# justinkay/aldi

Hardware: AMD Instinct MI355X
Metric: images/sec (student+teacher ALDI step), R50-FPN 1333x800 (higher is better)
Workload: dtype bf16

## Files before the change

aldi_amd/_lib.py:

```python
from __future__ import annotations

import ctypes as C
import os
import re

_HERE = os.path.dirname(os.path.abspath(__file__))
LIB_PATH = os.path.join(_HERE, "lib", "libaldi_hip.so")
HEADER_PATH = os.path.join(os.path.dirname(_HERE), "include", "aldi_hip.h")


class AldiHipError(RuntimeError):
    pass


if not os.path.exists(LIB_PATH):
    raise ImportError(
        f"{LIB_PATH} not found: build it with `python -c 'import __graft_entry__ as g; g.build()'` "
        "(or `make -C aldi_amd/csrc`). There is no CPU fallback for the ALDI HIP path.")

lib = C.CDLL(LIB_PATH)

F32, BF16 = 0, 1
MAX_IMAGES, MAX_LEVELS = 16, 5
c_void_p, c_int, c_float, c_long = C.c_void_p, C.c_int, C.c_float, C.c_long


def _ctype(decl: str):
    decl = decl.strip()
    if "*" in decl or decl.startswith("aldi_stream_t"):
        return C.c_void_p
    base = decl.rsplit(" ", 1)[0].replace("const", "").strip() if " " in decl else decl
    return {"int": C.c_int, "long": C.c_long, "float": C.c_float, "size_t": C.c_size_t, "unsigned": C.c_uint, "unsigned long long": C.c_ulonglong,
            "double": C.c_double}[base]


def parse_header(path: str = HEADER_PATH):
    src = open(path).read()
    src = re.sub(r"/\*.*?\*/", "", src, flags=re.S)
    protos = {}
    for m in re.finditer(r"\b(int|long|size_t|const char\*)\s+(aldi_\w+)\s*\(([^;{}]*?)\)\s*;", src, flags=re.S):
        ret, name, args = m.group(1), m.group(2), m.group(3)
        args = " ".join(args.split())
        argtypes = [] if args in ("void", "") else [_ctype(a) for a in args.split(",")]
        restype = {"int": C.c_int, "long": C.c_long, "size_t": C.c_size_t, "const char*": C.c_char_p}[ret]
        protos[name] = (restype, argtypes)
    return protos


PROTOS = parse_header()
for _name, (_res, _args) in PROTOS.items():
    _fn = getattr(lib, _name)
    _fn.restype = _res
    _fn.argtypes = _args


def check(status: int, what: str = ""):
    if status != 0:
        raise AldiHipError(f"{what}: status {status}: {lib.aldi_last_error().decode()}")


def call(name: str, *args):
    check(getattr(lib, name)(*args), name)


def set_tuning(name: str, value: int):
    call("aldi_set_tuning", name.encode(), int(value))


def get_tuning(name: str) -> int:
    v = C.c_int(0)
    call("aldi_get_tuning", name.encode(), C.byref(v))
    return v.value


def reset_tuning():
    call("aldi_reset_tuning")


def last_dispatch() -> str:
    return lib.aldi_last_dispatch().decode()


def plan_dispatch(args, n: int = 1) -> str:
    buf = C.create_string_buffer(224)
    call("aldi_conv_igemm_plan", C.byref(args) if isinstance(args, C.Structure) else args, n, buf, len(buf))
    return buf.value.decode()


def plan_wgrad_dispatch(args, n: int = 1, group: bool = False):
    buf = C.create_string_buffer(224)
    ws = C.c_long(0)
    call("aldi_conv_wgrad_plan", C.byref(args) if isinstance(args, C.Structure) else args, n, int(group), buf, len(buf), C.byref(ws))
    return buf.value.decode(), ws.value


class BoxLossChunk(C.Structure):
    _fields_ = [("r0", c_int), ("r1", c_int), ("grad_scale_cls", c_float), ("grad_scale_box", c_float), ("loss_box", c_void_p),
                ("teacher_pred", c_void_p), ("cls_temperature", c_float), ("kl", c_int), ("do_cls", c_int), ("do_reg", c_int),
                ("grad_scale_distill_cls", c_float), ("grad_scale_distill_reg", c_float), ("loss_distill", c_void_p)]


class ConvArgs(C.Structure):
    _fields_ = [
        ("x", c_void_p), ("w", c_void_p), ("y", c_void_p), ("y_f32", c_void_p),
        ("scale", c_void_p), ("shift", c_void_p), ("res", c_void_p), ("mask", c_void_p),
        ("N", c_int), ("H", c_int), ("W", c_int), ("Cin", c_int),
        ("Cout", c_int), ("KH", c_int), ("KW", c_int), ("stride", c_int), ("pad", c_int),
        ("Ho", c_int), ("Wo", c_int),
        ("relu", c_int), ("res_mode", c_int), ("out_scale", c_int), ("OH", c_int), ("OW", c_int),
        ("dtype", c_int), ("ws", c_void_p), ("ksplit", c_int), ("mask_bits", c_void_p), ("bits_out", c_void_p),
    ]


class WgradArgs(C.Structure):
    _fields_ = [
        ("x", c_void_p), ("g", c_void_p), ("dw", c_void_p), ("scale", c_void_p),
        ("N", c_int), ("H", c_int), ("W", c_int), ("Cin", c_int), ("Cout", c_int), ("KH", c_int), ("KW", c_int),
        ("stride", c_int), ("pad", c_int), ("Ho", c_int), ("Wo", c_int), ("dtype", c_int), ("db", c_void_p),
        ("ws", c_void_p), ("ws_bytes", C.c_long),
    ]


class StemArgs(C.Structure):
    _fields_ = [
        ("img", c_void_p), ("w", c_void_p), ("scale", c_void_p), ("shift", c_void_p), ("y", c_void_p),
        ("N", c_int), ("Hs", c_int), ("Ws", c_int), ("Hc", c_int), ("Wc", c_int),
        ("h", c_int * MAX_IMAGES), ("w_img", c_int * MAX_IMAGES),
        ("mean", c_float * 3), ("std", c_float * 3), ("dtype", c_int),
    ]


class RpnGeom(C.Structure):
    _fields_ = [
        ("num_levels", c_int), ("A", c_int), ("C", c_int),
        ("H", c_int * MAX_LEVELS), ("W", c_int * MAX_LEVELS), ("off", c_int * (MAX_LEVELS + 1)),
    ]


class RoiFeats(C.Structure):
    _fields_ = [
        ("feat", c_void_p * 4), ("grad", c_void_p * 4), ("H", c_int * 4), ("W", c_int * 4),
        ("scale", c_float * 4), ("C", c_int),
    ]


class DgwItem(C.Structure):
    _fields_ = [("w_master", c_void_p), ("scale", c_void_p), ("wt", c_void_p),
                ("Cout", c_int), ("KH", c_int), ("KW", c_int), ("Cin", c_int), ("tile_begin", c_int), ("reserved", c_int)]


class FoldItem(C.Structure):
    _fields_ = [("w", c_void_p), ("scale", c_void_p), ("out", c_void_p), ("rows", c_int), ("cols", c_int), ("chunk_begin", c_int), ("reserved", c_int)]


class BottleneckArgs(C.Structure):
    _fields_ = [("x", c_void_p), ("res", c_void_p), ("y", c_void_p), ("w1", c_void_p), ("w2", c_void_p), ("w3", c_void_p),
                ("b1", c_void_p), ("b2", c_void_p), ("b3", c_void_p),
                ("N", c_int), ("H", c_int), ("W", c_int), ("Cin", c_int), ("mid", c_int), ("Cout", c_int)]


class AttnArgs(C.Structure):
    _fields_ = [
        ("qkv", c_void_p), ("rel_h", c_void_p), ("rel_w", c_void_p),
        ("Qp", c_void_p), ("Kp", c_void_p), ("KpT", c_void_p), ("VT", c_void_p), ("QsT", c_void_p),
        ("O", c_void_p), ("lse", c_void_p), ("dO", c_void_p), ("dOT", c_void_p), ("dQp", c_void_p), ("delta", c_void_p),
        ("dqkv", c_void_p), ("drel_h", c_void_p), ("drel_w", c_void_p),
        ("nB", c_int), ("gh", c_int), ("gw", c_int), ("heads", c_int), ("Dq", c_int), ("scale", c_float),
    ]


PtrArray5 = c_void_p * MAX_LEVELS
```

aldi_amd/csrc/host.h:

```cpp
#pragma once
#include "../../include/aldi_hip.h"

int aldi_set_error_msg(int code, const char* msg);

typedef uint16_t bf16_t;

#define ALDI_KNOBS(X) \
    X(igemm_xcd, 1) X(igemm_tile, 0) X(igemm_dbg, 0) X(igemm_bigtile_min, 1024) X(igemm_bigtile, 64) X(igemm_bigtile_k, 768) X(igemm_lintile_min, 768) \
    X(igemm_halo, 1) X(igemm_force, 0) X(igemm_k64_min, 1024) X(igemm_group, 1) X(igemm_narrow_k, 512) X(igemm_splitk_tile, 2) X(igemm_halo_f32, 0) \
    X(igemm_f32_tile64_max, 4096) X(igemm_direct, 15) X(igemm_lean, 1) X(igemm_halo64_mid, 0) X(igemm_ws, 1) X(igemm_ws_wgs, 512) X(igemm_ws_min, 40000) \
    X(wgrad_lean, 1) X(wgrad_big_min, 28) X(wgrad_big_slots, 256) X(wgrad_slots, 384) X(wgrad_xcd, 1) \
    X(igemm_halo_ilv, 1) X(igemm_halo_small, 0) X(igemm_halo96, 0) \
    X(wgrad_dma, 0) X(wgrad_dbg, 0) X(wgrad_group_slots, 0) X(wgrad_group_epi, 24) X(wgrad_db, 0) X(wgrad_ordered, 1) X(wgrad_big_group, 1) X(wgrad_big_epi, 12) \
    X(wgrad_big_group_min, 64) X(wgrad_lds_pad_kb, 0) X(wgrad_f32_tile128, 1) X(wgrad_dma64, 3) X(wgrad_ilv, 0) \
    X(msda_gather, 7) X(msda_gather_list, 1500) X(msda_bin, 1) X(msda_bin_list, 512) X(roialign_sep, 1) X(roialign_bwd_rows, 2) \
    X(colsum_blocks, 256) X(colsum_minrows, 16) X(colsum_nt, 1024) X(colsum_block_kb, 384) \
    X(stem_mfma, 1) X(stem_pool_wgs, 0) X(sab_blocks, 512) X(ln_bwd_blocks, 512) X(ln_bwd_blocks_narrow, 1024) X(rpn_topk_fused, 1) X(ema_blocks, 2048) X(nms_mask_tri, 1) X(match_wave, 1)

struct AldiTuning {
#define ALDI_KNOB_FIELD(name, dflt) int name;
    ALDI_KNOBS(ALDI_KNOB_FIELD)
#undef ALDI_KNOB_FIELD
};
AldiTuning& aldi_tuning();
void aldi_note_dispatch(const char* kernel);

static inline int cdiv(long a, long b) { return (int)((a + b - 1) / b); }
```

aldi_amd/csrc/igemm.hip:

```cpp
#include "common.h"
#include "igemm_select.h"
#include "tile_prims.h"
#include <stdlib.h>

namespace {

template <typename T, int BM, int BN, int WM, int WN, int LDS_BYTES>
__device__ __forceinline__ void igemm_epilogue(const ConvDev& p, f32x4_t (&acc)[BM / WM / 16][BN / WN / 16], const int m0, const int n0, unsigned char* stg) {
    constexpr int NT = WM * WN * 64;
    constexpr int TM = BM / WM / 16, TN = BN / WN / 16;
    const int tid = threadIdx.x, lane = tid & 63, wave = tid >> 6;
    const int wm = wave / WN, wn = wave % WN;
    const int fr = lane & 15, fq = lane >> 4;
    if (p.dbg & 4) return;
    T* __restrict__ Y = static_cast<T*>(p.y);
    const T* __restrict__ R = static_cast<const T*>(p.res);
    const T* __restrict__ Mk = static_cast<const T*>(p.mask);
    if constexpr (sizeof(T) == 2) {
        constexpr int ROWB = BN * 2 + 16;
        constexpr bool kStageFits = BM * ROWB <= LDS_BYTES;
        if (kStageFits && Y && !p.y_f32 && (p.Cout & 7) == 0) {
            __syncthreads();
            {
                unsigned char* wr = stg + (wm * (BM / WM) + fr) * ROWB + (wn * (BN / WN) + fq * 4) * 2;
// ... 590 lines not shown
            if (wbase + it * NT < BN * KC) {
                unsigned off = b_voff[it] == OOB ? OOB : b_voff[it] + k_off;
                if (ktail && s * BK + b_kce[it] >= p.K) off = OOB;
                if (p.dbg & 16) off &= 0xfffu;
                glds16(rw, &lds[buf][BM * KC + wbase + it * NT], off);
            }
        }
        ci0 += BK;
        if (ci0 >= p.Cin) { ci0 = 0; ++tap; if (++kw == p.KW) { kw = 0; ++kh; } }
    };

    static_assert(KC == 4 || !PIPE, "the register-pipelined loop reads one k-step (4 chunks) per slab");
    constexpr int N_DMA = A_IT + (BN * KC) / NT;
    const int S_all = (p.dbg & 8) ? 1 : (p.K + BK - 1) / BK;
    const int s_first = p.ksplit > 1 ? (int)blockIdx.z * p.slabs_per_split : 0;
    const int S = p.ksplit > 1 ? min(S_all - s_first, p.slabs_per_split) : S_all;
    ci0 = s_first * BK;
    if constexpr (PIPE) pre_seen = S > 3;
    issue_slab(s_first, 0);
    if (S > 1) issue_slab(s_first + 1, 1);
    if constexpr (!PIPE) issue_pre();
    constexpr unsigned SLAB_BYTES = (BM + BN) * KC * 16;
    const int xrow = wm * (BM / WM) + fr, wrow = wn * (BN / WN) + fr;
    const unsigned x_rd0 = lds_addr(&lds[0][0]) + (unsigned)(xrow * KC + swz<KC>(xrow, fq)) * 16u;
    const unsigned w_rd0 = lds_addr(&lds[0][0]) + (unsigned)((BM + wrow) * KC + swz<KC>(wrow, fq)) * 16u;
    if constexpr (PIPE) {
    if (S > 2) issue_slab(s_first + 2, 2);
    __builtin_amdgcn_sched_barrier(0);
    issue_pre();
    __builtin_amdgcn_sched_barrier(0);
    u32x4_t xf0[TM], wf0[TN], xf1[TM], wf1[TN];
    if (S > 2) asm volatile("s_waitcnt vmcnt(%0)" ::"n"(2 * N_DMA + N_PRE) : "memory");
    else if (S > 1) asm volatile("s_waitcnt vmcnt(%0)" ::"n"(N_DMA + N_PRE) : "memory");
    else asm volatile("s_waitcnt vmcnt(%0)" ::"n"(N_PRE) : "memory");
    __builtin_amdgcn_s_barrier();
    __builtin_amdgcn_sched_barrier(0);
    frag_read_all<TM, KC * 16>(xf0, x_rd0);
    frag_read_all<TN, KC * 16>(wf0, w_rd0);
    frag_wait<TM, TN>(xf0, wf0);
    int rbuf = 1, ibuf = 0;
    auto step = [&](int s, u32x4_t* xc, u32x4_t* wc, u32x4_t* xn, u32x4_t* wn_) {
        const bool more = s + 1 < S;
        if (more) {
            if (N_PRE > 0 && s < 2) {
                if (s + 2 < S) asm volatile("s_waitcnt vmcnt(%0)" ::"n"(N_DMA + N_PRE) : "memory");
                else asm volatile("s_waitcnt vmcnt(%0)" ::"n"(N_PRE) : "memory");
            } else {
                if (s + 2 < S) asm volatile("s_waitcnt vmcnt(%0)" ::"n"(N_DMA) : "memory");
                else asm volatile("s_waitcnt vmcnt(0)" ::: "memory");
            }
            __builtin_amdgcn_s_barrier();
            __builtin_amdgcn_sched_barrier(0);
        }
        frag_read_all<TM, KC * 16>(xn, x_rd0 + (unsigned)rbuf * SLAB_BYTES);
        frag_read_all<TN, KC * 16>(wn_, w_rd0 + (unsigned)rbuf * SLAB_BYTES);
        if (more && s + 3 < S) issue_slab(s_first + s + 3, ibuf);
#pragma unroll
        for (int i = 0; i < TM; ++i)
#pragma unroll
            for (int j = 0; j < TN; ++j) acc[i][j] = Mma<T>::run(wc[j], xc[i], acc[i][j]);
        frag_wait<TM, TN>(xn, wn_);
        rbuf = rbuf == NBUF - 1 ? 0 : rbuf + 1;
        ibuf = ibuf == NBUF - 1 ? 0 : ibuf + 1;
    };
    for (int s = 0; s < S; s += 2) {
        step(s, xf0, wf0, xf1, wf1);
        if (s + 1 < S) step(s + 1, xf1, wf1, xf0, wf0);
    }
    } else {
    int buf = 0, nbuf = 2;
    for (int s = 0; s < S; ++s) {
        if (N_PRE > 0 && s == 0 && S > 1) asm volatile("s_waitcnt vmcnt(%0)" ::"n"(N_DMA + N_PRE) : "memory");
        else if (s + 1 < S) asm volatile("s_waitcnt vmcnt(%0)" ::"n"(N_DMA) : "memory");
        else asm volatile("s_waitcnt vmcnt(0)" ::: "memory");
        __builtin_amdgcn_s_barrier();
        __builtin_amdgcn_sched_barrier(0);
        if (s + 2 < S) issue_slab(s_first + s + 2, nbuf);
#pragma unroll
        for (int h = 0; h < KC / 4; ++h) {
            u32x4_t xf[TM], wf[TN];
            const unsigned xa = h == 0 ? x_rd0 : lds_addr(&lds[0][0]) + (unsigned)(xrow * KC + swz<KC>(xrow, fq + 4)) * 16u;
            const unsigned wa = h == 0 ? w_rd0 : lds_addr(&lds[0][0]) + (unsigned)((BM + wrow) * KC + swz<KC>(wrow, fq + 4)) * 16u;
            frag_read_all<TM, KC * 16>(xf, xa + (unsigned)buf * SLAB_BYTES);
            frag_read_all<TN, KC * 16>(wf, wa + (unsigned)buf * SLAB_BYTES);
            frag_wait<TM, TN>(xf, wf);
#pragma unroll
            for (int i = 0; i < TM; ++i)
#pragma unroll
                for (int j = 0; j < TN; ++j) acc[i][j] = Mma<T>::run(wf[j], xf[i], acc[i][j]);
        }
        buf = buf == NBUF - 1 ? 0 : buf + 1;
        nbuf = nbuf == NBUF - 1 ? 0 : nbuf + 1;
    }
    }

    }

    if constexpr (DIRECT) {
        if (!pre_seen) {
            asm volatile("s_waitcnt vmcnt(0)" ::: "memory");
            __builtin_amdgcn_s_barrier();
        }
        __builtin_amdgcn_sched_barrier(0);
        igemm_epilogue_direct<BM, BN, WM, WN, RESL>(p, acc, m0, n0, rres, lds_addr(aux_lds));
        return;
    }
    if (p.ksplit > 1) {
        ConvDev q = p;
        q.y_f32 = p.y_f32 + (long)blockIdx.z * p.M * p.Cout;
        igemm_epilogue<T, BM, BN, WM, WN, NSTAGE * SLOTS * 16>(q, acc, m0, n0, reinterpret_cast<unsigned char*>(&lds_all[0]));
        return;
    }
    igemm_epilogue<T, BM, BN, WM, WN, NSTAGE * SLOTS * 16>(p, acc, m0, n0, reinterpret_cast<unsigned char*>(&lds_all[0]));
}


template <typename T, int BN>
__device__ __forceinline__ void igemm_halo_rs_body(const ConvDev& p, int bid, const int nmt, const int nnt) {
    static_assert(sizeof(T) == 2, "bf16 only");
    constexpr int BM = 256, WM = 4, WN = BN / 64, NT = WM * WN * 64, KC = 4, EP = 8, BK = 32;
    static_assert(NT == 512, "eight waves: two halves of four");
    constexpr int TM = BM / WM / 16, TN = BN / WN / 16;
    constexpr int AS = ((BM + 2) * KC + 63) / 64 * 64;
    constexpr int WS = 3 * BN * KC;
    constexpr int STAGE = AS + WS, NS = 3;
    constexpr int AH_IT = (AS + NT - 1) / NT, WH_IT = WS / NT;
    static_assert(AH_IT == 3 && WH_IT == 3 && WS % NT == 0, "six DMA pieces per thread and group: two per phase");
    __shared__ __attribute__((aligned(128))) uint4 lds[NS * STAGE + 4];

    const int tid = threadIdx.x, lane = tid & 63, wave = tid >> 6;
    const int wm = wave / WN, wn = wave % WN;
    if (p.xcd) {
        const int total = nmt * nnt, q = total >> 3, r = total & 7, xcd = bid & 7, idx = bid >> 3;
        bid = (xcd < r ? xcd * (q + 1) : r * (q + 1) + (xcd - r) * q) + idx;
    }
    const int m0 = (bid / nnt) * BM, n0 = (bid % nnt) * BN;
    const T* __restrict__ X = static_cast<const T*>(p.x);
    const T* __restrict__ Wt = static_cast<const T*>(p.w);
    const __amdgpu_buffer_rsrc_t rx = __builtin_amdgcn_make_buffer_rsrc(const_cast<T*>(X), 0, p.x_bytes, 0x00020000);
    const __amdgpu_buffer_rsrc_t rw = __builtin_amdgcn_make_buffer_rsrc(const_cast<T*>(Wt), 0, p.w_bytes, 0x00020000);
    constexpr unsigned OOB = 0x80000000u;
    const int wbase = __builtin_amdgcn_readfirstlane(tid & ~63);
    const bool half_b = __builtin_amdgcn_readfirstlane(wave) >= 4;
    const bool third_pix = wbase + 2 * NT < AS;
    f32x4_t acc[TM][TN];
#pragma unroll
    for (int i = 0; i < TM; ++i)
#pragma unroll
        for (int j = 0; j < TN; ++j) acc[i][j] = f32x4_t{0.f, 0.f, 0.f, 0.f};
    const int fr = lane & 15, fq = lane >> 4;
    if (tid < 4) lds[NS * STAGE + tid] = make_uint4(0u, 0u, 0u, 0u);

    unsigned ha_voff[AH_IT], ha_mask[AH_IT];
#pragma unroll
    for (int it = 0; it < AH_IT; ++it) {
        const int c = tid + it * NT, row = c >> 2, kce = swz_halo(row, c & 3);
        const int q0 = m0 - 1 + row;
        const bool ok = row < BM + 2 && q0 >= 0 && q0 < p.M;
        const int qq = ok ? q0 : 0;
        const int h0 = (qq / p.W) % p.H;
        ha_voff[it] = ((unsigned)qq * (unsigned)p.Cin + (unsigned)(kce * EP)) * (unsigned)sizeof(T);
        ha_mask[it] = ok ? ((h0 >= 1 ? 1u : 0u) | 2u | (h0 <= p.H - 2 ? 4u : 0u)) : 0u;
    }
    unsigned hw_voff[WH_IT];
#pragma unroll
    for (int it = 0; it < WH_IT; ++it) {
        const int c = tid + it * NT, kwi = c / (BN * KC), rem = c - kwi * (BN * KC), row = rem >> 2, kce = swz_halo(row, rem & 3);
        const int co = n0 + row;
        hw_voff[it] = co < p.Cout ? ((unsigned)co * (unsigned)p.K + (unsigned)(kwi * p.Cin + kce * EP)) * (unsigned)sizeof(T) : OOB;
    }
    const int xrow = wm * (BM / WM) + fr, wrow = wn * (BN / WN) + fr;
    const unsigned lbase = lds_addr(&lds[0]);
    const unsigned zrow = lbase + (unsigned)(NS * STAGE) * 16u + (unsigned)fq * 16u;
    bool edge_l[TM], edge_r[TM];
    unsigned zaddr[TM];
#pragma unroll
    for (int i = 0; i < TM; ++i) {
        const int m = m0 + wm * (BM / WM) + i * 16 + fr;
        const int wo = m % p.W;
        edge_l[i] = wo == 0;
        edge_r[i] = wo == p.W - 1;
        zaddr[i] = zrow - (unsigned)(i * 16 * KC * 16);
    }
    unsigned x_rd[3];
#pragma unroll
    for (int kw = 0; kw < 3; ++kw) x_rd[kw] = lbase + (unsigned)((xrow + kw) * KC + swz_halo(xrow + kw, fq)) * 16u;
    const unsigned w_rd = lbase + (unsigned)((AS + wrow * KC) + swz_halo(wrow, fq)) * 16u;
    constexpr unsigned STAGE_BYTES = STAGE * 16;
    const int G = 3 * (p.Cin / BK);

    unsigned a_off = 0, w_off = 0, ikh = 0;
    int gkh = 0, gci = 0;
    auto next_group = [&]() {
        a_off = (unsigned)(((gkh - 1) * p.W * p.Cin + gci) * (int)sizeof(T));
        w_off = (unsigned)((gkh * 3 * p.Cin + gci) * (int)sizeof(T));
        ikh = (unsigned)gkh;
        gci += BK;
        if (gci >= p.Cin) { gci = 0; ++gkh; }
    };
    const unsigned dmask = (p.dbg & 16) ? 0xfffu : 0xffffffffu;
    const bool no_dma = p.dbg & 32, no_mfma = p.dbg & 64;
    auto issue_pair = [&](int pair, int st) {
        uint4* base = &lds[st * STAGE];
        if (no_dma) return;
        if (pair == 0) {
            glds16(rx, base + wbase, ((ha_mask[0] >> ikh) & 1u) ? (ha_voff[0] + a_off) & dmask : OOB);
            glds16(rx, base + wbase + NT, ((ha_mask[1] >> ikh) & 1u) ? (ha_voff[1] + a_off) & dmask : OOB);
        } else if (pair == 1) {
            glds16(rw, base + AS + wbase, hw_voff[0] == OOB ? OOB : (hw_voff[0] + w_off) & dmask);
            glds16(rw, base + AS + wbase + NT, hw_voff[1] == OOB ? OOB : (hw_voff[1] + w_off) & dmask);
        } else {
            glds16(rw, base + AS + wbase + 2 * NT, hw_voff[2] == OOB ? OOB : (hw_voff[2] + w_off) & dmask);
            if (third_pix) glds16(rx, base + wbase + 2 * NT, ((ha_mask[2] >> ikh) & 1u) ? (ha_voff[2] + a_off) & dmask : OOB);
        }
    };
    next_group();
    issue_pair(0, 0); issue_pair(1, 0); issue_pair(2, 0);
    next_group();
    issue_pair(0, 1); issue_pair(1, 1);
    asm volatile("s_waitcnt vmcnt(4)" ::: "memory");
    __builtin_amdgcn_s_barrier();
    __builtin_amdgcn_sched_barrier(0);
    if (half_b) {
        __builtin_amdgcn_s_barrier();
        __builtin_amdgcn_sched_barrier(0);
    }
    int rs = 0, s1 = 1, s2 = 2;
    for (int g = 0; g < G; ++g) {
        const unsigned gb = (unsigned)rs * STAGE_BYTES;
#pragma unroll
        for (int t = 0; t < 3; ++t) {
            u32x4_t xf[TM], wf[TN];
            if (t == 1) {
                frag_read_all<TM, KC * 16>(xf, x_rd[1] + gb);
            } else {
                unsigned xa[TM];
#pragma unroll
                for (int i = 0; i < TM; ++i) xa[i] = (t == 0 ? edge_l[i] : edge_r[i]) ? zaddr[i] : x_rd[t] + gb;
                frag_read_each<TM, KC * 16>(xf, xa);
            }
            frag_read_all<TN, KC * 16>(wf, w_rd + gb + (unsigned)(t * BN * KC * 16));
            if (t == 0) {
                if (g + 1 < G) issue_pair(2, s1);
            } else if (g + 2 < G) {
                if (t == 1) next_group();
                issue_pair(t - 1, s2);
            }
            if (t == 2 && g + 1 < G) {
                if (g + 2 < G && !no_dma) asm volatile("s_waitcnt vmcnt(4)" ::: "memory");
                else asm volatile("s_waitcnt vmcnt(0)" ::: "memory");
            }
            __builtin_amdgcn_sched_barrier(0);
            __builtin_amdgcn_s_barrier();
            __builtin_amdgcn_sched_barrier(0);
            frag_wait<TM, TN>(xf, wf);
            __builtin_amdgcn_sched_barrier(0);
            __builtin_amdgcn_s_setprio(1);
            if (!no_mfma) {
#pragma unroll
                for (int i = 0; i < TM; ++i)
#pragma unroll
                    for (int j = 0; j < TN; ++j) acc[i][j] = Mma<T>::run(wf[j], xf[i], acc[i][j]);
            }
            __builtin_amdgcn_s_setprio(0);
            __builtin_amdgcn_sched_barrier(0);
            __builtin_amdgcn_s_barrier();
            __builtin_amdgcn_sched_barrier(0);
        }
        const int o = rs; rs = s1; s1 = s2; s2 = o;
    }
    if (!half_b) {
        __builtin_amdgcn_s_barrier();
        __builtin_amdgcn_sched_barrier(0);
    }
    igemm_epilogue<T, BM, BN, WM, WN, NS * STAGE * 16>(p, acc, m0, n0, reinterpret_cast<unsigned char*>(&lds[0]));
}

template <typename T, int BN>
__global__ __launch_bounds__(512) void igemm_halo_rs_kernel(ConvDev p) {
    igemm_halo_rs_body<T, BN>(p, (int)(blockIdx.y * gridDim.x + blockIdx.x), (int)gridDim.x, (int)gridDim.y);
}

#include "igemm_halo64.h"
#include "igemm_ws.h"

template <int BM, int NT, bool HALO> constexpr int min_waves_per_simd() { return HALO && BM == 240 ? 2 * NT / 256 : 1; }
template <typename T, int BM, int BN, int WM, int WN, int KC, bool PIPE, bool HALO = false, int EPI = 0, bool LEAN = false>
__global__ __launch_bounds__(WM* WN * 64, (min_waves_per_simd<BM, WM * WN * 64, HALO>())) void igemm_kernel(ConvDev p) {
    igemm_body<T, BM, BN, WM, WN, KC, PIPE, HALO, EPI, LEAN>(p, (int)(blockIdx.y * gridDim.x + blockIdx.x), (int)gridDim.x, (int)gridDim.y);
}

template <typename T, int BM, int BN, int WM, int WN, int KC, bool PIPE, bool HALO = false>
__global__ __launch_bounds__(WM* WN * 64, (min_waves_per_simd<BM, WM * WN * 64, HALO>())) void igemm_group_kernel(ConvGroup G) {
    const int bid = (int)blockIdx.x;
    int i = 0;
    for (int k = 1; k < G.n; ++k)
        if (bid >= G.wg_begin[k]) i = k;
    i = __builtin_amdgcn_readfirstlane(i);
    const int local = bid - G.wg_begin[i];
    if (local >= G.nmt[i] * G.nnt[i]) return;
    igemm_body<T, BM, BN, WM, WN, KC, PIPE, HALO>(G.p[i], local, G.nmt[i], G.nnt[i]);
}

template <int BM, int BN, int WM, int WN, bool DIRECT, bool ILV = false>
__global__ __launch_bounds__(WM* WN * 64) void igemm_halo64_group_kernel(ConvGroup G) {
    const int bid = (int)blockIdx.x;
    int i = 0;
    for (int k = 1; k < G.n; ++k)
        if (bid >= G.wg_begin[k]) i = k;
    i = __builtin_amdgcn_readfirstlane(i);
    const int local = bid - G.wg_begin[i];
    if (local >= G.nmt[i] * G.nnt[i]) return;
    igemm_halo64_body<BM, BN, WM, WN, DIRECT, ILV>(G.p[i], local, G.nmt[i], G.nnt[i]);
}


int group_table(ConvGroup& G, const int BM, const int BN, const ConvDev& d) {
    int wg = 0;
    for (int i = 0; i < G.n; ++i) {
        G.p[i].xcd = d.xcd; G.p[i].dbg = d.dbg;
        G.nmt[i] = cdiv(G.p[i].M, BM); G.nnt[i] = cdiv(G.p[i].Cout, BN);
        G.wg_begin[i] = wg;
        wg += (G.nmt[i] * G.nnt[i] + 7) / 8 * 8;
    }
    for (int i = G.n; i <= kMaxConvGroup; ++i) G.wg_begin[i] = wg;
    return wg;
}

template <typename T, int BM, int BN, int WM, int WN, int KC, bool PIPE, bool HALO, int EPI>
int launch_tile(const Choice& c, const ConvDev& d, const ConvGroup* g, hipStream_t st) {
    constexpr int NT = WM * WN * 64;
    if constexpr (EPI != 0) {
        const dim3 grid(cdiv(d.M, BM), cdiv(d.Cout, BN));
        if constexpr (!HALO) {
            if (c.lean) hipLaunchKernelGGL((igemm_kernel<T, BM, BN, WM, WN, KC, PIPE, HALO, EPI, true>), grid, dim3(NT), 0, st, d);
        }
        if (HALO || !c.lean) hipLaunchKernelGGL((igemm_kernel<T, BM, BN, WM, WN, KC, PIPE, HALO, EPI, false>), grid, dim3(NT), 0, st, d);
    } else if (g) {
        ConvGroup G = *g;
        const int wg = group_table(G, BM, BN, d);
        hipLaunchKernelGGL((igemm_group_kernel<T, BM, BN, WM, WN, KC, PIPE, HALO>), dim3(wg), dim3(NT), 0, st, G);
    } else {
        const dim3 grid(cdiv(d.M, BM), cdiv(d.Cout, BN), d.ksplit > 1 ? d.ksplit : 1);
        hipLaunchKernelGGL((igemm_kernel<T, BM, BN, WM, WN, KC, PIPE, HALO>), grid, dim3(NT), 0, st, d);
    }
    ALDI_CHECK_LAUNCH();
    return ALDI_OK;
}
template <typename T, int BM, int BN, int WM, int WN, int KC, bool PIPE, int EPI>
int launch_TAP(const Choice& c, const ConvDev& d, const ConvGroup* g, hipStream_t st) { return launch_tile<T, BM, BN, WM, WN, KC, PIPE, false, EPI>(c, d, g, st); }
template <typename T, int BM, int BN, int WM, int WN, int KC, bool PIPE, int EPI>
int launch_HALO(const Choice& c, const ConvDev& d, const ConvGroup* g, hipStream_t st) { return launch_tile<T, BM, BN, WM, WN, KC, PIPE, true, EPI>(c, d, g, st); }

template <typename T, int BM, int BN, int WM, int WN, int KC, bool PIPE, int EPI>
int launch_ROLES(const Choice&, const ConvDev& d, const ConvGroup*, hipStream_t st) {
    static_assert(BM == 256 && WM * WN * 64 == 512, "igemm_halo_rs_body: 256 pixels on eight waves");
    const dim3 grid(cdiv(d.M, BM), cdiv(d.Cout, BN));
    hipLaunchKernelGGL((igemm_halo_rs_kernel<T, BN>), grid, dim3(512), 0, st, d);
    ALDI_CHECK_LAUNCH();
    return ALDI_OK;
}

template <typename T, int BM, int BN, int WM, int WN, int KC, bool PIPE, int EPI>
int launch_HALO64(const Choice& c, const ConvDev& d, const ConvGroup* g, hipStream_t st) {
    constexpr int NT = WM * WN * 64;
    constexpr bool HAS_ILV = BM == 256 && BN == 256 && WM == 4 && WN == 2;
    if (g) {
        ConvGroup G = *g;
        const int wg = group_table(G, BM, BN, d);
        if (c.ilv) {
            if (c.direct) hipLaunchKernelGGL((igemm_halo64_group_kernel<BM, BN, WM, WN, true, HAS_ILV>), dim3(wg), dim3(NT), 0, st, G);
            else hipLaunchKernelGGL((igemm_halo64_group_kernel<BM, BN, WM, WN, false, HAS_ILV>), dim3(wg), dim3(NT), 0, st, G);
        } else {
            if (c.direct) hipLaunchKernelGGL((igemm_halo64_group_kernel<BM, BN, WM, WN, true>), dim3(wg), dim3(NT), 0, st, G);
            else hipLaunchKernelGGL((igemm_halo64_group_kernel<BM, BN, WM, WN, false>), dim3(wg), dim3(NT), 0, st, G);
        }
    } else {
        const dim3 grid(cdiv(d.M, BM), cdiv(d.Cout, BN));
        if (c.ilv) {
            if (c.direct) hipLaunchKernelGGL((igemm_halo64_kernel<BM, BN, WM, WN, true, HAS_ILV>), grid, dim3(NT), 0, st, d);
            else hipLaunchKernelGGL((igemm_halo64_kernel<BM, BN, WM, WN, false, HAS_ILV>), grid, dim3(NT), 0, st, d);
        } else {
            if (c.direct) hipLaunchKernelGGL((igemm_halo64_kernel<BM, BN, WM, WN, true>), grid, dim3(NT), 0, st, d);
            else hipLaunchKernelGGL((igemm_halo64_kernel<BM, BN, WM, WN, false>), grid, dim3(NT), 0, st, d);
        }
    }
    ALDI_CHECK_LAUNCH();
    return ALDI_OK;
}

int launch_choice(const Choice& c, const ConvDev& d, const ConvGroup* g, hipStream_t st) {
    switch (c.tile) {
#define IGEMM_TILE_CASE(id, T, form, BM, BN, WM, WN, KC, PIPE, EPI) \
    case id: return launch_##form<T, BM, BN, WM, WN, KC, PIPE != 0, EPI>(c, d, g, st);
        IGEMM_TILES(IGEMM_TILE_CASE)
#undef IGEMM_TILE_CASE
    default: break;
    }
    return aldi_set_error_msg(ALDI_ERR_ARG, "conv_igemm: unknown tile");
}

__global__ __launch_bounds__(256) void splitk_finalize_kernel(const float* __restrict__ ws, int ks, long mc, int C, const float* __restrict__ scale,
                                                              const float* __restrict__ shift, int relu, bf16_t* __restrict__ y) {
    const long e = ((long)blockIdx.x * blockDim.x + threadIdx.x) * 4;
    if (e >= mc) return;
    float4 a = *reinterpret_cast<const float4*>(ws + e);
    for (int z = 1; z < ks; ++z) {
        const float4 b = *reinterpret_cast<const float4*>(ws + z * mc + e);
        a.x += b.x; a.y += b.y; a.z += b.z; a.w += b.w;
    }
    const int c = (int)(e % C);
    if (scale) { const float4 s4 = *reinterpret_cast<const float4*>(scale + c); a.x *= s4.x; a.y *= s4.y; a.z *= s4.z; a.w *= s4.w; }
    if (shift) { const float4 s4 = *reinterpret_cast<const float4*>(shift + c); a.x += s4.x; a.y += s4.y; a.z += s4.z; a.w += s4.w; }
    if (relu) { a.x = fmaxf(a.x, 0.f); a.y = fmaxf(a.y, 0.f); a.z = fmaxf(a.z, 0.f); a.w = fmaxf(a.w, 0.f); }
    uint2 o;
    o.x = pack2_bf16(a.x, a.y); o.y = pack2_bf16(a.z, a.w);
    *reinterpret_cast<uint2*>(y + e) = o;
}

constexpr int kNameCap = 112;

int conv_one(const aldi_conv_args* a, const bool dry, hipStream_t st, char* name) {
    ConvDev d;
    Choice c;
    if (int rc = plan_conv(a, aldi_tuning(), d, c)) return rc;
    dispatch_name(c, name, kNameCap);
    if (dry) return ALDI_OK;
    if (int rc = launch_choice(c, d, nullptr, st)) return rc;
    aldi_note_dispatch(name);
    if (c.ksplit > 1) {
        const long mc = (long)d.M * d.Cout;
        hipLaunchKernelGGL(splitk_finalize_kernel, dim3(cdiv(mc / 4, 256)), dim3(256), 0, st, static_cast<const float*>(a->ws), c.ksplit, mc, d.Cout, a->scale, a->shift,
                           a->relu, static_cast<bf16_t*>(a->y));
        ALDI_CHECK_LAUNCH();
    }
    return ALDI_OK;
}

int conv_many(const aldi_conv_args* args, const int n, const bool dry, hipStream_t st, char* name) {
    if (!args || n < 1) return aldi_set_error_msg(ALDI_ERR_ARG, "conv_igemm_group: no problems");
    if (n == 1 || !conv_group_same(args, n, aldi_tuning())) {
        for (int i = 0; i < n; ++i)
            if (int rc = conv_one(&args[i], dry, st, name)) return rc;
        return ALDI_OK;
    }
    static thread_local ConvGroup G;
    ConvDev d;
    Choice c;
    if (int rc = plan_conv_group(args, n, aldi_tuning(), G, d, c)) return rc;
    dispatch_name(c, name, kNameCap);
    if (dry) return ALDI_OK;
    if (int rc = launch_choice(c, d, &G, st)) return rc;
    aldi_note_dispatch(name);
    return ALDI_OK;
}
}

extern "C" int aldi_conv_igemm(const aldi_conv_args* a, aldi_stream_t stream) {
    char name[kNameCap];
    return conv_one(a, false, static_cast<hipStream_t>(stream), name);
}

extern "C" int aldi_conv_igemm_group(const aldi_conv_args* args, int n, aldi_stream_t stream) {
    char name[kNameCap];
    return conv_many(args, n, false, static_cast<hipStream_t>(stream), name);
}

extern "C" int aldi_conv_igemm_plan(const aldi_conv_args* args, int n, char* name, int cap) {
    char buf[kNameCap] = "";
    const int rc = n == 1 ? conv_one(args, true, nullptr, buf) : conv_many(args, n, true, nullptr, buf);
    if (rc == ALDI_OK && name && cap > 0) snprintf(name, (size_t)cap, "%s", buf);
    return rc;
}
```

aldi_amd/csrc/igemm_halo64.h:

```cpp
#pragma once

template <int N, int STRIDE, int BASE, int I = 0>
__device__ __forceinline__ void frag_read_n(u32x4_t* f, unsigned addr) {
    if constexpr (I < N) {
        f[I] = frag_read<BASE + I * STRIDE>(addr);
        frag_read_n<N, STRIDE, BASE, I + 1>(f, addr);
    }
}
template <int N>
__device__ __forceinline__ void frag_wait1(u32x4_t* a) {
    asm volatile("s_waitcnt lgkmcnt(0)" ::: "memory");
#pragma unroll
    for (int i = 0; i < N; ++i) asm volatile("" : "+v"(a[i]));
}

template <int V> struct KwTag { static constexpr int value = V; };

__device__ __forceinline__ void mma_ip(f32x4_t& c, const u32x4_t& a, const u32x4_t& b) {
    asm volatile("v_mfma_f32_16x16x32_bf16 %0, %1, %2, %0" : "+v"(c) : "v"(a), "v"(b));
}
template <int NM, int I = 0, typename FM, typename FF>
__device__ __forceinline__ void interleave(FM&& mma, FF&& fill) {
    if constexpr (I < NM) {
        mma(KwTag<I>{});
        fill(KwTag<I>{});
        interleave<NM, I + 1>(mma, fill);
    }
}

template <int BM, int BN, int WM, int WN, bool DIRECT, bool ILV = false>
__device__ __forceinline__ void igemm_halo64_body(const ConvDev& p, int bid, const int nmt, const int nnt) {
    typedef bf16_t T;
    constexpr int NT = WM * WN * 64, KC = 8, EP = 8, BK = 64;
    constexpr int TM = BM / WM / 16;
    constexpr int TN = BN / WN / 16;
    constexpr int CS = TN / 4;
    constexpr int TH = 4;
    static_assert((TM == 4 || TM == 8) && (CS == 1 || CS == 2), "64 / 128 pixels x 64 / 128 channels per wave");
    constexpr int XS = ((BM + 2) * KC + 63) / 64 * 64;
    constexpr int WS = BN * KC;
    constexpr int X_IT = (XS + NT - 1) / NT;
    constexpr int W_IT = WS / NT;
    constexpr int XQ = (X_IT - 1) / 4, WQ = W_IT / 4;
    static_assert((X_IT - 1) % 4 == 0 && W_IT % 4 == 0 && WS % NT == 0 && XS - (X_IT - 1) * NT <= 64, "piece schedule below: four quarters + one tail piece (wave 0) per slab, four quarters per tap");
    constexpr int RING = 2 * XS + 2 * WS;
    constexpr int EPI_SLOTS = BM * (BN * 2 + 16) / 16;
    constexpr int LDS_SLOTS = RING + 8 > EPI_SLOTS ? RING + 8 : EPI_SLOTS;
    constexpr int FR = 16 * KC * 16;
    __shared__ __attribute__((aligned(128))) uint4 lds_all[LDS_SLOTS];

    const int tid = threadIdx.x, lane = tid & 63, wave = tid >> 6;
    const int wm = wave / WN, wn = wave % WN;
    if (p.xcd) {
        const int total = nmt * nnt, q = total >> 3, r = total & 7, xcd = bid & 7, idx = bid >> 3;
        bid = (xcd < r ? xcd * (q + 1) : r * (q + 1) + (xcd - r) * q) + idx;
    }
    const int m0 = (bid / nnt) * BM, n0 = (bid % nnt) * BN;
    const __amdgpu_buffer_rsrc_t rx = __builtin_amdgcn_make_buffer_rsrc(const_cast<T*>(static_cast<const T*>(p.x)), 0, p.x_bytes, 0x00020000);
    const __amdgpu_buffer_rsrc_t rw = __builtin_amdgcn_make_buffer_rsrc(const_cast<T*>(static_cast<const T*>(p.w)), 0, p.w_bytes, 0x00020000);
    constexpr unsigned OOB = 0x80000000u;
    const int wbase = __builtin_amdgcn_readfirstlane(tid & ~63);
    const bool tail = wbase + (X_IT - 1) * NT < XS;
    const int fr = lane & 15, fq = lane >> 4;
    const int plev = __builtin_amdgcn_readfirstlane((p.dbg & 128) ? 0 : (p.dbg & 256) ? 1 : ((wave < WM * WN / 2) != ((p.dbg & 512) != 0)) ? 2 : 1);
    const bool prio = plev != 0, prio_hi = plev == 2;
    const bool early_w = ILV && __builtin_amdgcn_readfirstlane(p.dbg & 1024) == 0;
    const bool no_dma = p.dbg & 32, no_mfma = p.dbg & 64;

    f32x4_t acc[TM][TN];
#pragma unroll
    for (int i = 0; i < TM; ++i)
#pragma unroll
        for (int j = 0; j < TN; ++j) acc[i][j] = f32x4_t{0.f, 0.f, 0.f, 0.f};
    if (tid < 8) lds_all[RING + tid] = make_uint4(0u, 0u, 0u, 0u);

    unsigned xa_voff[X_IT], xa_ok = 0;
#pragma unroll
    for (int it = 0; it < X_IT; ++it) {
        const int c = tid + it * NT, row = c >> 3, kce = (c & 7) ^ (row & 6);
        const int q0 = m0 - 1 + row;
        const bool ok = row < BM + 2 && q0 >= 0 && q0 < p.M;
        const int qq = ok ? q0 : 0;
        const int h0 = (qq / p.W) % p.H;
        xa_voff[it] = ((unsigned)qq * (unsigned)p.Cin + (unsigned)(kce * EP)) * 2u;
        if (ok) xa_ok |= ((h0 >= 1 ? 1u : 0u) | 2u | (h0 <= p.H - 2 ? 4u : 0u)) << (3 * it);
    }
    unsigned wa_voff[W_IT];
#pragma unroll
    for (int it = 0; it < W_IT; ++it) {
        const int c = tid + it * NT, row = c >> 3, kce = (c & 7) ^ (row & 6);
        const int co = n0 + (DIRECT ? direct_perm<BN / WN>(row) : row);
        wa_voff[it] = co < p.Cout ? ((unsigned)co * (unsigned)p.K + (unsigned)(kce * EP)) * 2u : OOB;
    }
    int xkh = 0, xci = 0, tkh = 0, tci = 0, tkw = 0;
    auto issue_x = [&](int it, int st) {
        if (no_dma) return;
        const unsigned a_off = (unsigned)(((xkh - 1) * p.W * p.Cin + xci) * 2);
        glds16(rx, &lds_all[st * XS + wbase + it * NT], ((xa_ok >> (3 * it + xkh)) & 1u) ? xa_voff[it] + a_off : OOB);
    };
    auto next_x = [&]() { if (++xkh == 3) { xkh = 0; xci += BK; } };
    auto issue_w = [&](int it, int st, unsigned w_off) {
        if (no_dma) return;
        glds16(rw, &lds_all[2 * XS + st * WS + wbase + it * NT], wa_voff[it] == OOB ? OOB : wa_voff[it] + w_off);
    };
    auto tap_off = [&]() { return (unsigned)(((tkh * 3 + tkw) * p.Cin + tci) * 2); };
    auto next_tap = [&]() { if (++tkw == 3) { tkw = 0; if (++tkh == 3) { tkh = 0; tci += BK; } } };

    const int xrow = wm * (BM / WM) + fr, wrow = wn * (BN / WN) + fr;
    const unsigned lbase = lds_addr(&lds_all[0]);
    unsigned x_rd[3][2], w_rd[2];
#pragma unroll
    for (int kw = 0; kw < 3; ++kw)
#pragma unroll
        for (int h = 0; h < 2; ++h) x_rd[kw][h] = lbase + (unsigned)((xrow + kw) * KC + ((h * 4 + fq) ^ ((xrow + kw) & 6))) * 16u;
#pragma unroll
    for (int h = 0; h < 2; ++h) w_rd[h] = lbase + (unsigned)(2 * XS + wrow * KC + ((h * 4 + fq) ^ (wrow & 6))) * 16u;
    bool edge_l[TM], edge_r[TM];
    unsigned zaddr[TM];
#pragma unroll
    for (int i = 0; i < TM; ++i) {
        const int m = m0 + wm * (BM / WM) + i * 16 + fr;
        const int wo = m % p.W;
        edge_l[i] = wo == 0;
        edge_r[i] = wo == p.W - 1;
        zaddr[i] = lbase + (unsigned)(RING * 16) + (unsigned)fq * 16u - (unsigned)(i * FR);
    }
    auto read_x = [&](u32x4_t* xf, auto KW, auto H, unsigned xoff) {
        constexpr int kw = decltype(KW)::value, h = decltype(H)::value;
        if constexpr (kw == 1) {
            frag_read_n<TM, FR, 0>(xf, x_rd[1][h] + xoff);
        } else {
            const unsigned a = x_rd[kw][h] + xoff;
            unsigned xa[TM];
#pragma unroll
            for (int i = 0; i < TM; ++i) xa[i] = (kw == 0 ? edge_l[i] : edge_r[i]) ? zaddr[i] : a;
            frag_read_each<TM, KC * 16>(xf, xa);
        }
    };

    const int ngroups = 3 * (p.Cin / BK), U = 3 * ngroups;
#pragma unroll
    for (int it = 0; it < X_IT - 1; ++it) issue_x(it, 0);
    if (tail) issue_x(X_IT - 1, 0);
    next_x();
    {
        const unsigned o = tap_off();
#pragma unroll
        for (int it = 0; it < W_IT; ++it) issue_w(it, 0, o);
        next_tap();
    }
    unsigned woff_a = tap_off();
#pragma unroll
    for (int q = 0; q < 2 * WQ; ++q) issue_w(q, 1, woff_a);
    if (early_w) {
#pragma unroll
        for (int q = 2 * WQ; q < 4 * WQ; ++q) issue_w(q, 1, woff_a);
    }
    next_tap();
    __builtin_amdgcn_sched_barrier(0);
    if (early_w) asm volatile("s_waitcnt vmcnt(%0)" ::"n"(4 * WQ) : "memory");
    else asm volatile("s_waitcnt vmcnt(%0)" ::"n"(2 * WQ) : "memory");
    __builtin_amdgcn_s_barrier();
    __builtin_amdgcn_sched_barrier(0);

    u32x4_t x0[TM], x1[TM], wa[TH], wb[TH];
    read_x(x0, KwTag<0>{}, KwTag<0>{}, 0u);
    frag_read_n<TH, FR, 0>(wa, w_rd[0]);
    frag_wait<TM, TH>(x0, wa);
    __builtin_amdgcn_sched_barrier(0);

    unsigned xoff = 0, woff = 0;
    constexpr unsigned XSB = XS * 16, WSB = WS * 16;
    auto tap4 = [&](auto KW, const int g, const int u) {
        constexpr int kw = decltype(KW)::value;
        const bool more1 = u + 1 < U, more2 = u + 2 < U;
        frag_read_n<TH, FR, TH * FR>(wb, w_rd[0] + woff);
        if (more1) {
#pragma unroll
            for (int q = 0; q < WQ; ++q) issue_w(2 * WQ + q, (u + 1) & 1, woff_a);
        }
        __builtin_amdgcn_sched_barrier(0);
        if (!no_mfma) {
            if (prio) { if (prio_hi) __builtin_amdgcn_s_setprio(2); else __builtin_amdgcn_s_setprio(1); }
#pragma unroll
            for (int i = 0; i < TM; ++i)
#pragma unroll
                for (int j = 0; j < TH; ++j) acc[i][j] = Mma<T>::run(wa[j], x0[i], acc[i][j]);
            if (prio) __builtin_amdgcn_s_setprio(0);
        }
        frag_wait1<TH>(wb);
        __builtin_amdgcn_sched_barrier(0);
        read_x(x1, KW, KwTag<1>{}, xoff);
        frag_read_n<TH, FR, 0>(wa, w_rd[1] + woff);
        if (more1) {
#pragma unroll
            for (int q = 0; q < WQ; ++q) issue_w(3 * WQ + q, (u + 1) & 1, woff_a);
        }
        __builtin_amdgcn_sched_barrier(0);
        if (!no_mfma) {
            if (prio) { if (prio_hi) __builtin_amdgcn_s_setprio(2); else __builtin_amdgcn_s_setprio(1); }
#pragma unroll
            for (int i = 0; i < TM; ++i)
#pragma unroll
                for (int j = 0; j < TH; ++j) acc[i][TH + j] = Mma<T>::run(wb[j], x0[i], acc[i][TH + j]);
            if (prio) __builtin_amdgcn_s_setprio(0);
        }
        frag_wait<TM, TH>(x1, wa);
        __builtin_amdgcn_sched_barrier(0);
        frag_read_n<TH, FR, TH * FR>(wb, w_rd[1] + woff);
        int nx = 0;
        if (kw < 2 && g + 1 < ngroups) {
            const int st = (g + 1) & 1;
            if constexpr (kw == 0) {
#pragma unroll
                for (int q = 0; q < 2 * XQ; ++q) issue_x(q, st);
                nx = 2 * XQ;
            }
            if constexpr (kw == 1) {
#pragma unroll
                for (int q = 0; q < 2 * XQ; ++q) issue_x(2 * XQ + q, st);
                nx = 2 * XQ;
                if (tail) { issue_x(X_IT - 1, st); nx = 2 * XQ + 1; }
                next_x();
            }
        }
        __builtin_amdgcn_sched_barrier(0);
        if (!no_mfma) {
            if (prio) { if (prio_hi) __builtin_amdgcn_s_setprio(2); else __builtin_amdgcn_s_setprio(1); }
#pragma unroll
            for (int i = 0; i < TM; ++i)
#pragma unroll
                for (int j = 0; j < TH; ++j) acc[i][j] = Mma<T>::run(wa[j], x1[i], acc[i][j]);
            if (prio) __builtin_amdgcn_s_setprio(0);
        }
        frag_wait1<TH>(wb);
        __builtin_amdgcn_sched_barrier(0);
        if (no_dma || nx == 0) asm volatile("s_waitcnt vmcnt(0)" ::: "memory");
        else if (nx == 2 * XQ) asm volatile("s_waitcnt vmcnt(%0)" ::"n"(2 * XQ) : "memory");
        else asm volatile("s_waitcnt vmcnt(%0)" ::"n"(2 * XQ + 1) : "memory");
        __builtin_amdgcn_s_barrier();
        __builtin_amdgcn_sched_barrier(0);
        constexpr int kw_n = kw == 2 ? 0 : kw + 1;
        const unsigned xoff_n = kw == 2 ? xoff ^ XSB : xoff, woff_n = woff ^ WSB;
        read_x(x0, KwTag<kw_n>{}, KwTag<0>{}, xoff_n);
        frag_read_n<TH, FR, 0>(wa, w_rd[0] + woff_n);
        if (more2) {
            woff_a = tap_off();
#pragma unroll
            for (int q = 0; q < 2 * WQ; ++q) issue_w(q, u & 1, woff_a);
            next_tap();
        }
        __builtin_amdgcn_sched_barrier(0);
        if (!no_mfma) {
            if (prio) { if (prio_hi) __builtin_amdgcn_s_setprio(2); else __builtin_amdgcn_s_setprio(1); }
#pragma unroll
            for (int i = 0; i < TM; ++i)
#pragma unroll
                for (int j = 0; j < TH; ++j) acc[i][TH + j] = Mma<T>::run(wb[j], x1[i], acc[i][TH + j]);
            if (prio) __builtin_amdgcn_s_setprio(0);
        }
        frag_wait<TM, TH>(x0, wa);
        __builtin_amdgcn_sched_barrier(0);
        xoff = xoff_n; woff = woff_n;
    };
    auto x_addr = [&](unsigned* xa, auto KW, auto H, unsigned xo) {
        constexpr int kw = decltype(KW)::value, h = decltype(H)::value;
#pragma unroll
        for (int i = 0; i < TM; ++i) {
            if constexpr (kw == 1) xa[i] = x_rd[1][h] + xo;
            else xa[i] = (kw == 0 ? edge_l[i] : edge_r[i]) ? zaddr[i] : x_rd[kw][h] + xo;
        }
    };
    auto tap4i = [&](auto KW, const int g, const int u) {
        constexpr int kw = decltype(KW)::value;
        constexpr int NM = TM * TH;
        static_assert(TM + TH + 1 + 2 * 2 * WQ <= NM && TH + 1 + 2 * (2 * XQ + 1) <= NM && TM + TH + 2 * 2 * WQ < NM, "the fillers of a sub-phase fit between its MFMAs");
        const bool more1 = u + 1 < U, more2 = u + 2 < U;
        {
            const unsigned wr = w_rd[0] + woff;
            if (prio) { if (prio_hi) __builtin_amdgcn_s_setprio(2); else __builtin_amdgcn_s_setprio(1); }
            interleave<NM>([&](auto M) { constexpr int m = decltype(M)::value; mma_ip(acc[m / TH][m % TH], wa[m % TH], x0[m / TH]); },
                           [&](auto M) {
                               constexpr int m = decltype(M)::value;
                               if constexpr (m < TH) wb[m] = frag_read<(TH + m) * FR>(wr);
                               if constexpr (m == TH + 1) {
                                   if (more1 && !early_w) {
#pragma unroll
                                       for (int q = 0; q < WQ; ++q) issue_w(2 * WQ + q, (u + 1) & 1, woff_a);
                                   }
                               }
                           });
            if (prio) __builtin_amdgcn_s_setprio(0);
            frag_wait1<TH>(wb);
            __builtin_amdgcn_sched_barrier(0);
        }
        {
            unsigned xa[TM];
            x_addr(xa, KW, KwTag<1>{}, xoff);
            const unsigned wr = w_rd[1] + woff;
            if (prio) { if (prio_hi) __builtin_amdgcn_s_setprio(2); else __builtin_amdgcn_s_setprio(1); }
            interleave<NM>([&](auto M) { constexpr int m = decltype(M)::value; mma_ip(acc[m / TH][TH + m % TH], wb[m % TH], x0[m / TH]); },
                           [&](auto M) {
                               constexpr int m = decltype(M)::value;
                               if constexpr (m < TM) x1[m] = frag_read<m * FR>(xa[m]);
                               else if constexpr (m < TM + TH) wa[m - TM] = frag_read<(m - TM) * FR>(wr);
                               if constexpr (m == TM + TH + 1) {
                                   if (more1 && !early_w) {
#pragma unroll
                                       for (int q = 0; q < WQ; ++q) issue_w(3 * WQ + q, (u + 1) & 1, woff_a);
                                   }
                               }
                           });
            if (prio) __builtin_amdgcn_s_setprio(0);
            frag_wait<TM, TH>(x1, wa);
            __builtin_amdgcn_sched_barrier(0);
        }
        const bool slab = kw < 2 && g + 1 < ngroups;
        const int sst = (g + 1) & 1;
        int nx = 0;
        if (slab) nx = (kw == 1 && tail) ? 2 * XQ + 1 : 2 * XQ;
        {
            const unsigned wr = w_rd[1] + woff;
            if (prio) { if (prio_hi) __builtin_amdgcn_s_setprio(2); else __builtin_amdgcn_s_setprio(1); }
            interleave<NM>([&](auto M) { constexpr int m = decltype(M)::value; mma_ip(acc[m / TH][m % TH], wa[m % TH], x1[m / TH]); },
                           [&](auto M) {
                               constexpr int m = decltype(M)::value;
                               if constexpr (m < TH) wb[m] = frag_read<(TH + m) * FR>(wr);
                               if constexpr (kw < 2 && m > TH && (m - TH) % 2 == 1 && (m - TH) / 2 <= 2 * XQ) {
                                   constexpr int q = (m - TH) / 2;
                                   if (slab) {
                                       if constexpr (q < 2 * XQ) issue_x(kw * 2 * XQ + q, sst);
                                       else if constexpr (kw == 1) { if (tail) issue_x(X_IT - 1, sst); }
                                   }
                               }
                           });
            if (prio) __builtin_amdgcn_s_setprio(0);
            if constexpr (kw == 1) { if (slab) next_x(); }
            frag_wait1<TH>(wb);
            __builtin_amdgcn_sched_barrier(0);
        }
        if (no_dma || nx == 0) asm volatile("s_waitcnt vmcnt(0)" ::: "memory");
        else if (nx == 2 * XQ) asm volatile("s_waitcnt vmcnt(%0)" ::"n"(2 * XQ) : "memory");
        else asm volatile("s_waitcnt vmcnt(%0)" ::"n"(2 * XQ + 1) : "memory");
        __builtin_amdgcn_s_barrier();
        __builtin_amdgcn_sched_barrier(0);
        {
            constexpr int kw_n = kw == 2 ? 0 : kw + 1;
            const unsigned xoff_n = kw == 2 ? xoff ^ XSB : xoff, woff_n = woff ^ WSB;
            unsigned xa[TM];
            x_addr(xa, KwTag<kw_n>{}, KwTag<0>{}, xoff_n);
            const unsigned wr = w_rd[0] + woff_n;
            if (more2) woff_a = tap_off();
            if (prio) { if (prio_hi) __builtin_amdgcn_s_setprio(2); else __builtin_amdgcn_s_setprio(1); }
            interleave<NM>([&](auto M) { constexpr int m = decltype(M)::value; mma_ip(acc[m / TH][TH + m % TH], wb[m % TH], x1[m / TH]); },
                           [&](auto M) {
                               constexpr int m = decltype(M)::value;
                               if constexpr (m < TM) x0[m] = frag_read<m * FR>(xa[m]);
                               else if constexpr (m < TM + TH) wa[m - TM] = frag_read<(m - TM) * FR>(wr);
                               if constexpr (m > TM + TH && (m - TM - TH) % 2 == 1 && (m - TM - TH) / 2 < 2 * WQ) {
                                   if (more2) issue_w((m - TM - TH) / 2, u & 1, woff_a);
                               }
                               if constexpr (m > TM + TH && (m - TM - TH) % 2 == 0 && (m - TM - TH) / 2 - 1 < 2 * WQ) {
                                   if (more2 && early_w) issue_w(2 * WQ + (m - TM - TH) / 2 - 1, u & 1, woff_a);
                               }
                           });
            if (prio) __builtin_amdgcn_s_setprio(0);
            if (more2) next_tap();
            frag_wait<TM, TH>(x0, wa);
            __builtin_amdgcn_sched_barrier(0);
            xoff = xoff_n; woff = woff_n;
        }
    };
    auto tap2 = [&](auto KW, const int g, const int u) {
        constexpr int kw = decltype(KW)::value;
        const bool more1 = u + 1 < U, more2 = u + 2 < U;
        read_x(x1, KW, KwTag<1>{}, xoff);
        frag_read_n<TH, FR, 0>(wb, w_rd[1] + woff);
        if (more1) {
#pragma unroll
            for (int q = 0; q < 2 * WQ; ++q) issue_w(2 * WQ + q, (u + 1) & 1, woff_a);
        }
        int nx = 0;
        if (kw < 2 && g + 1 < ngroups) {
            const int st = (g + 1) & 1;
            if constexpr (kw == 0) {
#pragma unroll
                for (int q = 0; q < 2 * XQ; ++q) issue_x(q, st);
                nx = 2 * XQ;
            }
            if constexpr (kw == 1) {
#pragma unroll
                for (int q = 0; q < 2 * XQ; ++q) issue_x(2 * XQ + q, st);
                nx = 2 * XQ;
                if (tail) { issue_x(X_IT - 1, st); nx = 2 * XQ + 1; }
                next_x();
            }
        }
        __builtin_amdgcn_sched_barrier(0);
        if (!no_mfma) {
            if (prio) { if (prio_hi) __builtin_amdgcn_s_setprio(2); else __builtin_amdgcn_s_setprio(1); }
#pragma unroll
            for (int i = 0; i < TM; ++i)
#pragma unroll
                for (int j = 0; j < TH; ++j) acc[i][j] = Mma<T>::run(wa[j], x0[i], acc[i][j]);
            if (prio) __builtin_amdgcn_s_setprio(0);
        }
        frag_wait<TM, TH>(x1, wb);
        __builtin_amdgcn_sched_barrier(0);
        if (no_dma || nx == 0) asm volatile("s_waitcnt vmcnt(0)" ::: "memory");
        else if (nx == 2 * XQ) asm volatile("s_waitcnt vmcnt(%0)" ::"n"(2 * XQ) : "memory");
        else asm volatile("s_waitcnt vmcnt(%0)" ::"n"(2 * XQ + 1) : "memory");
        __builtin_amdgcn_s_barrier();
        __builtin_amdgcn_sched_barrier(0);
        constexpr int kw_n = kw == 2 ? 0 : kw + 1;
        const unsigned xoff_n = kw == 2 ? xoff ^ XSB : xoff, woff_n = woff ^ WSB;
        read_x(x0, KwTag<kw_n>{}, KwTag<0>{}, xoff_n);
        frag_read_n<TH, FR, 0>(wa, w_rd[0] + woff_n);
        if (more2) {
            woff_a = tap_off();
#pragma unroll
            for (int q = 0; q < 2 * WQ; ++q) issue_w(q, u & 1, woff_a);
            next_tap();
        }
        __builtin_amdgcn_sched_barrier(0);
        if (!no_mfma) {
            if (prio) { if (prio_hi) __builtin_amdgcn_s_setprio(2); else __builtin_amdgcn_s_setprio(1); }
#pragma unroll
            for (int i = 0; i < TM; ++i)
#pragma unroll
                for (int j = 0; j < TH; ++j) acc[i][j] = Mma<T>::run(wb[j], x1[i], acc[i][j]);
            if (prio) __builtin_amdgcn_s_setprio(0);
        }
        frag_wait<TM, TH>(x0, wa);
        __builtin_amdgcn_sched_barrier(0);
        xoff = xoff_n; woff = woff_n;
    };
    auto tap = [&](auto KW, const int g, const int u) {
        if constexpr (CS == 2 && ILV) tap4i(KW, g, u);
        else if constexpr (CS == 2) tap4(KW, g, u);
        else tap2(KW, g, u);
    };
    for (int g = 0; g < ngroups; ++g) {
        tap(KwTag<0>{}, g, 3 * g);
        tap(KwTag<1>{}, g, 3 * g + 1);
        tap(KwTag<2>{}, g, 3 * g + 2);
    }
    if constexpr (ILV) asm volatile("s_nop 15\n\ts_nop 15" ::: "memory");
    if constexpr (DIRECT) {
        if (p.dbg & 4) return;
        constexpr int H = TN / 2;
        float4 sc[H][2], sh[H][2];
        const bool has_sc = p.scale != nullptr, has_sh = p.shift != nullptr;
#pragma unroll
        for (int h = 0; h < H; ++h) {
            const int c = n0 + wn * (BN / WN) + h * 32 + fq * 8;
            const bool okc = c < p.Cout;
            sc[h][0] = sc[h][1] = make_float4(1.f, 1.f, 1.f, 1.f);
            sh[h][0] = sh[h][1] = make_float4(0.f, 0.f, 0.f, 0.f);
            if (has_sc && okc) { sc[h][0] = *reinterpret_cast<const float4*>(p.scale + c); sc[h][1] = *reinterpret_cast<const float4*>(p.scale + c + 4); }
            if (has_sh && okc) { sh[h][0] = *reinterpret_cast<const float4*>(p.shift + c); sh[h][1] = *reinterpret_cast<const float4*>(p.shift + c + 4); }
        }
        const __amdgpu_buffer_rsrc_t ry = make_rsrc_uniform(p.y, 0x7fffffffu);
        typedef short s16x2_t __attribute__((ext_vector_type(2)));
#pragma unroll
        for (int i = 0; i < TM; ++i) {
            const int m = m0 + wm * (BM / WM) + i * 16 + fr;
#pragma unroll
            for (int h = 0; h < H; ++h) {
                const int c = n0 + wn * (BN / WN) + h * 32 + fq * 8;
                const bool ok = m < p.M && c < p.Cout;
                float v[8];
#pragma unroll
                for (int e = 0; e < 4; ++e) { v[e] = acc[i][2 * h][e]; v[4 + e] = acc[i][2 * h + 1][e]; }
                if (has_sc) {
                    v[0] *= sc[h][0].x; v[1] *= sc[h][0].y; v[2] *= sc[h][0].z; v[3] *= sc[h][0].w;
                    v[4] *= sc[h][1].x; v[5] *= sc[h][1].y; v[6] *= sc[h][1].z; v[7] *= sc[h][1].w;
                }
                if (has_sh) {
                    v[0] += sh[h][0].x; v[1] += sh[h][0].y; v[2] += sh[h][0].z; v[3] += sh[h][0].w;
                    v[4] += sh[h][1].x; v[5] += sh[h][1].y; v[6] += sh[h][1].z; v[7] += sh[h][1].w;
                }
                uint32_t d[4];
#pragma unroll
                for (int q = 0; q < 4; ++q) d[q] = pack2_bf16(v[2 * q], v[2 * q + 1]);
                if (p.relu) {
#pragma unroll
                    for (int q = 0; q < 4; ++q) {
                        s16x2_t t = *reinterpret_cast<s16x2_t*>(&d[q]);
                        t = __builtin_elementwise_max(t, s16x2_t{0, 0});
                        d[q] = *reinterpret_cast<uint32_t*>(&t);
                    }
                }
                const u32x4_t ov = {d[0], d[1], d[2], d[3]};
                __builtin_amdgcn_raw_buffer_store_b128(ov, ry, ok ? ((unsigned)m * (unsigned)p.Cout + (unsigned)c) * 2u : 0x80000000u, 0, 0);
            }
        }
        return;
    }
    igemm_epilogue<T, BM, BN, WM, WN, LDS_SLOTS * 16>(p, acc, m0, n0, reinterpret_cast<unsigned char*>(&lds_all[0]));
}

template <int BM, int BN, int WM, int WN, bool DIRECT, bool ILV = false>
__global__ __launch_bounds__(WM* WN * 64) void igemm_halo64_kernel(ConvDev p) {
    igemm_halo64_body<BM, BN, WM, WN, DIRECT, ILV>(p, (int)(blockIdx.y * gridDim.x + blockIdx.x), (int)gridDim.x, (int)gridDim.y);
}
```

aldi_amd/csrc/igemm_select.h:

```cpp
#pragma once
#include "host.h"
#include <stdio.h>

namespace {

struct ConvDev {
    const void* x; const void* w; void* y; float* y_f32;
    const float* scale; const float* shift; const void* res; const void* mask;
    int N, H, W, Cin, Cout, KH, KW, stride, pad, Ho, Wo;
    int relu, res_mode, out_scale, OH, OW;
    int M, K, xcd, dbg;
    unsigned x_bytes, w_bytes;
    int ksplit, slabs_per_split;
    int lean;
    const unsigned char* mask_bits; unsigned char* bits_out;
};

constexpr int kMaxConvGroup = 12;
struct ConvGroup {
    int n;
    int wg_begin[kMaxConvGroup + 1];
    int nmt[kMaxConvGroup], nnt[kMaxConvGroup];
    ConvDev p[kMaxConvGroup];
};

#define IGEMM_TILES(X) \
    X(BF16_TAP_128x16,       bf16_t, TAP,    128, 16,  4, 1, 4, 1, 0) X(F32_TAP_128x16,   float, TAP,  128, 16,  4, 1, 4, 1, 0) \
    X(BF16_TAP_128x128,      bf16_t, TAP,    128, 128, 2, 2, 4, 1, 0) X(F32_TAP_128x128,  float, TAP,  128, 128, 2, 2, 4, 1, 0) \
    X(BF16_TAP_128x64,       bf16_t, TAP,    128, 64,  4, 1, 4, 1, 0) X(F32_TAP_128x64,   float, TAP,  128, 64,  4, 1, 4, 1, 0) \
    X(BF16_TAP_64x64,        bf16_t, TAP,    64,  64,  2, 2, 4, 1, 0) X(F32_TAP_64x64,    float, TAP,  64,  64,  2, 2, 4, 1, 0) \
    X(BF16_TAP_256x128,      bf16_t, TAP,    256, 128, 4, 2, 4, 0, 0) X(F32_TAP_256x128,  float, TAP,  256, 128, 4, 2, 4, 0, 0) \
    X(BF16_HALO_128x128,     bf16_t, HALO,   128, 128, 2, 2, 4, 0, 0) X(F32_HALO_128x128, float, HALO, 128, 128, 2, 2, 4, 0, 0) \
    X(BF16_HALO_128x64,      bf16_t, HALO,   128, 64,  4, 1, 4, 0, 0) X(F32_HALO_128x64,  float, HALO, 128, 64,  4, 1, 4, 0, 0) \
    X(BF16_HALO_256x128,     bf16_t, HALO,   256, 128, 4, 2, 4, 0, 0) X(F32_HALO_256x128, float, HALO, 256, 128, 4, 2, 4, 0, 0) \
    X(BF16_HALO_128x64_D,    bf16_t, HALO,   128, 64,  4, 1, 4, 0, 1) \
    X(BF16_HALO_96x64,       bf16_t, HALO,   96,  64,  3, 1, 4, 0, 0) X(BF16_HALO_96x64_D, bf16_t, HALO, 96, 64, 3, 1, 4, 0, 1) \
    X(BF16_HALO_64x64,       bf16_t, HALO,   64,  64,  2, 2, 4, 0, 0) X(BF16_HALO_64x64_D, bf16_t, HALO, 64, 64, 2, 2, 4, 0, 1) \
    X(BF16_HALO_240x128,     bf16_t, HALO,   240, 128, 3, 2, 4, 0, 0) \
    X(BF16_ROLES_256x128,    bf16_t, ROLES,  256, 128, 4, 2, 4, 0, 0) \
    X(BF16_HALO64_256x256,   bf16_t, HALO64, 256, 256, 4, 2, 8, 0, 0) \
    X(BF16_HALO64_128x128,   bf16_t, HALO64, 128, 128, 2, 2, 8, 0, 0) \
    X(BF16_HALO64_256x256_W4, bf16_t, HALO64, 256, 256, 2, 2, 8, 0, 0) \
    X(BF16_TAP_128x64_D,     bf16_t, TAP,    128, 64,  4, 1, 4, 1, 1) X(BF16_TAP_128x64_DR, bf16_t, TAP, 128, 64, 4, 1, 4, 1, 2) \
    X(BF16_TAP_128x128_K64,  bf16_t, TAP,    128, 128, 2, 2, 8, 0, 0) \
    X(BF16_TAP_128x64_K64,   bf16_t, TAP,    128, 64,  4, 1, 8, 0, 0) X(BF16_TAP_128x64_K64_D, bf16_t, TAP, 128, 64, 4, 1, 8, 0, 1) \
    X(BF16_TAP_64x64_K64,    bf16_t, TAP,    64,  64,  2, 2, 8, 0, 0) X(BF16_TAP_64x64_K64_D, bf16_t, TAP, 64, 64, 2, 2, 8, 0, 1) \
    X(BF16_TAP_256x128_K64,  bf16_t, TAP,    256, 128, 4, 2, 8, 0, 0) \
    X(BF16_WS_K64,           bf16_t, WS,     32,  256, 1, 4, 8, 0, 1) X(BF16_WS_K128,     bf16_t, WS,  32,  256, 1, 4, 16, 0, 1) \
    X(BF16_WS_K256,          bf16_t, WS,     32,  128, 1, 4, 32, 0, 1) X(BF16_WS_K512,    bf16_t, WS,  16,  128, 1, 4, 64, 0, 1)

enum TileForm { TAP, HALO, ROLES, HALO64, WS };
enum TileId {
#define IGEMM_TILE_ID(id, T, form, BM, BN, WM, WN, KC, PIPE, EPI) id,
    IGEMM_TILES(IGEMM_TILE_ID)
#undef IGEMM_TILE_ID
    kNumTiles
};
struct TileRow { const char* id; bool f32; TileForm form; int BM, BN, WM, WN, KC; bool pipe; int epi; };
constexpr TileRow kTiles[kNumTiles] = {
#define IGEMM_TILE_ROW(id, T, form, BM, BN, WM, WN, KC, PIPE, EPI) {#id, sizeof(T) == 4, form, BM, BN, WM, WN, KC, PIPE != 0, EPI},
    IGEMM_TILES(IGEMM_TILE_ROW)
#undef IGEMM_TILE_ROW
};

struct Choice {
    TileId tile;
    bool lean;
    bool direct, ilv;
    int ksplit;
    int ws_wgs;
    int group_n;
};

inline int ws_channels(int K) { return K == 64 || K == 128 ? 256 : K == 256 || K == 512 ? 128 : 0; }
inline bool ws_ok(const ConvDev& d) {
    const int bn = ws_channels(d.K);
    return d.KH * d.KW == 1 && d.stride == 1 && d.pad == 0 && d.K == d.Cin && bn && d.Cout % bn == 0 && d.y && !d.y_f32 && !d.mask && d.out_scale == 1 &&
           d.ksplit <= 1 && (long)d.M * d.Cout * 2 < (1L << 31);
}
inline bool halo64_direct_ok(const ConvDev& d) {
    return d.y && !d.y_f32 && d.out_scale == 1 && (d.Cout & 7) == 0 && !d.mask && !d.mask_bits && !d.bits_out && !d.res_mode;
}
inline bool plain_1x1(const ConvDev& d) { return d.KH * d.KW == 1 && d.stride == 1 && d.pad == 0; }

inline Choice select_tile(const ConvDev& d, const AldiTuning& tn, const bool f32, const int group_n, const ConvDev* group = nullptr) {
    Choice c = {BF16_TAP_128x128, false, false, false, d.ksplit > 1 ? d.ksplit : 0, tn.igemm_ws_wgs, group_n};
    const auto pick = [&](TileId bf16_id, TileId f32_id) {
        c.tile = f32 ? f32_id : bf16_id;
        const TileRow& r = kTiles[c.tile];
        c.lean = r.form == TAP && r.epi != 0 && tn.igemm_lean && plain_1x1(d) && d.K % 64 == 0 && !(tn.igemm_dbg & (8 | 16));
        if (r.form == HALO64) {
            c.direct = (tn.igemm_direct & 8) != 0;
            for (int i = 0; i < (group_n ? group_n : 1); ++i) c.direct = c.direct && halo64_direct_ok(group_n ? group[i] : d);
            c.ilv = c.tile == BF16_HALO64_256x256 && tn.igemm_halo_ilv != 0;
        }
        return c;
    };
#define BOTH(name) pick(BF16_##name, F32_##name)
#define BF16(name) pick(BF16_##name, BF16_##name)
    const bool bf16 = !f32;
    if (d.ksplit > 1) {
        const int tile_knob = tn.igemm_splitk_tile;
        const bool big_ok = (long)cdiv(d.M, 256) * cdiv(d.Cout, 128) * d.ksplit >= 200;
        if (tile_knob == 3 || (tile_knob == 2 && big_ok)) return BF16(TAP_256x128_K64);
        if (tile_knob == 1 || (tile_knob == 4 && big_ok)) return BF16(TAP_256x128);
        return BF16(TAP_128x128_K64);
    }
    const long big = (long)cdiv(d.M, 128) * cdiv(d.Cout, 128);
    const int force = tn.igemm_force;
    const bool direct_ok = bf16 && !group_n && d.y && !d.y_f32 && d.out_scale == 1 && (d.Cout & 7) == 0 && !d.mask && d.ksplit <= 1 &&
                           !(d.mask_bits && (d.scale || d.shift)) && d.Cout >= 64 &&
                           !(d.mask_bits && (d.Cout & 31));
    const int direct = direct_ok ? tn.igemm_direct : 0;
    {
        const bool same3 = d.KH == 3 && d.KW == 3 && d.stride == 1 && d.pad == 1 && d.Ho == d.H && d.Wo == d.W && d.Cin % 32 == 0 && d.out_scale == 1;
        const bool f32_halo = f32 && tn.igemm_halo_f32 > 0 && (long)cdiv(d.M, 128) * cdiv(d.Cout, 64) >= tn.igemm_halo_f32;
        if (tn.igemm_halo && (bf16 || f32_halo) && same3) {
            if (force == 1) return BOTH(HALO_128x128);
            if (bf16 && force == 2 && (direct & 4) && !d.res_mode) return BF16(HALO_128x64_D);
            if (force == 2) return BOTH(HALO_128x64);
            if (force == 4) return BOTH(HALO_256x128);
            if (bf16) {
                if (force == 17 && (direct & 4) && !d.res_mode) return BF16(HALO_96x64_D);
                if (force == 17) return BF16(HALO_96x64);
                if (force == 16 && (direct & 4) && !d.res_mode) return BF16(HALO_64x64_D);
                if (force == 16) return BF16(HALO_64x64);
                if (force == 9) return BF16(HALO_240x128);
                if (force == 10 && !group_n) return BF16(ROLES_256x128);
                if (force == 11 && d.Cin % 64 == 0) return BF16(HALO64_256x256);
                if (force == 13 && d.Cin % 64 == 0) return BF16(HALO64_128x128);
                if (force == 15 && d.Cin % 64 == 0) return BF16(HALO64_256x256_W4);
            }
            if (force == 0 || force == 3) {
                if (d.Cout <= 64) return BOTH(HALO_128x64);
                if (big >= tn.igemm_bigtile_min) {
                    if (bf16 && tn.igemm_bigtile == 64 && d.Cin % 64 == 0 && d.Cout % 256 == 0) return BF16(HALO64_256x256);
                    if (bf16 && tn.igemm_bigtile == 65 && d.Cin % 64 == 0 && d.Cout % 256 == 0) return BF16(HALO64_256x256_W4);
                    if (tn.igemm_bigtile == 1) return BOTH(HALO_128x128);
                    if (bf16 && tn.igemm_bigtile == 10 && !group_n) return BF16(ROLES_256x128);
                    return BOTH(HALO_256x128);
                }
                if (bf16 && tn.igemm_halo64_mid > 0 && big >= tn.igemm_halo64_mid && d.Cin % 64 == 0 && d.Cout % 128 == 0) return BF16(HALO64_128x128);
                const long t64 = (long)cdiv(d.M, 128) * cdiv(d.Cout, 64);
                if (bf16 && tn.igemm_halo96 > 0 && t64 >= 200 && t64 <= 600) {
                    if ((direct & 4) && !d.res_mode) return BF16(HALO_96x64_D);
                    return BF16(HALO_96x64);
                }
                if (bf16 && tn.igemm_halo_small > 0 && t64 <= tn.igemm_halo_small && d.Cin >= 512) {
                    if ((direct & 4) && !d.res_mode) return BF16(HALO_64x64_D);
                    return BF16(HALO_64x64);
                }
                if (bf16 && (direct & 4) && !d.res_mode) return BF16(HALO_128x64_D);
                return BOTH(HALO_128x64);
            }
        }
    }
    if (bf16 && !group_n && ws_ok(d) && (force == 14 || (force == 0 && tn.igemm_ws && (tn.igemm_direct & 1) && d.M >= (d.res_mode == 2 ? 4L : 1L) * tn.igemm_ws_min)))
        return d.K == 64 ? BF16(WS_K64) : d.K == 128 ? BF16(WS_K128) : d.K == 256 ? BF16(WS_K256) : BF16(WS_K512);
    if (force == 5 || (force == 0 && d.Cout <= 16)) return BOTH(TAP_128x16);
    if (force == 1) return BOTH(TAP_128x128);
    if (bf16 && force == 2 && (direct & 1)) return d.res_mode ? BF16(TAP_128x64_DR) : BF16(TAP_128x64_D);
    if (force == 2) return BOTH(TAP_128x64);
    if (force == 3) return BOTH(TAP_64x64);
    if (force == 4) return BOTH(TAP_256x128);
    if (bf16) {
        const bool plain = plain_1x1(d);
        if (plain && force == 6) return BF16(TAP_128x128_K64);
        if (plain && force == 7) return BF16(TAP_128x64_K64);
        if (plain && force == 12 && (direct & 1) && !d.res_mode && d.K % 64 == 0) return BF16(TAP_128x64_K64_D);
        const bool lin256 = tn.igemm_tile != 9 && big >= tn.igemm_lintile_min && d.K >= tn.igemm_bigtile_k;
        if (plain && (force == 8 || (force == 0 && !lin256 && d.Cout > 64 && d.K % 64 == 0 && d.K >= tn.igemm_k64_min))) {
            if ((direct & 2) && !d.res_mode) return BF16(TAP_64x64_K64_D);
            return BF16(TAP_64x64_K64);
        }
    }
    if (f32 && force == 0 && big < tn.igemm_f32_tile64_max) return BOTH(TAP_64x64);
    if (d.Cout <= 64) return BOTH(TAP_128x64);
    if (tn.igemm_tile != 9 && big >= tn.igemm_lintile_min && d.K >= tn.igemm_bigtile_k) {
        if (bf16 && tn.igemm_tile != 7 && plain_1x1(d) && d.K % 64 == 0) return BF16(TAP_256x128_K64);
        return BOTH(TAP_256x128);
    }
    if (big < 200) return BOTH(TAP_64x64);
    if (bf16 && d.K <= tn.igemm_narrow_k && (direct & 1)) return d.res_mode ? BF16(TAP_128x64_DR) : BF16(TAP_128x64_D);
    if (bf16 && d.K <= tn.igemm_narrow_k) return BOTH(TAP_128x64);
    return BOTH(TAP_128x128);
#undef BOTH
#undef BF16
}

inline int dispatch_name(const Choice& c, char* name, int cap) {
    const TileRow& r = kTiles[c.tile];
    const char* elem = r.f32 ? "f32" : "bf16";
    const char* grp = c.group_n ? "_group" : "";
    switch (r.form) {
    case WS: return snprintf(name, cap, "igemm_ws<%s,%d,%d,k%d>", elem, r.BM, r.BN, r.KC * 8);
    case HALO64:
        return snprintf(name, cap, "igemm%s%.0d<%s,%d,%d,%d,%d,halo64%s%s>", grp, c.group_n, elem, r.BM, r.BN, r.WM, r.WN, c.direct ? ",direct" : "",
                        (c.tile == BF16_HALO64_256x256 && !c.ilv) ? ",lockstep" : "");
    case ROLES: return snprintf(name, cap, "igemm<%s,%d,%d,%d,%d,roles,halo>", elem, r.BM, r.BN, r.WM, r.WN);
    default:
        return snprintf(name, cap, "igemm%s%.0d<%s,%d,%d,%d,%d,%s,%s%s%s>%s", grp, c.group_n, elem, r.BM, r.BN, r.WM, r.WN, r.pipe ? "pipe" : "flat", r.form == HALO ? "halo" : "tap",
                        r.KC == 8 ? ",k64" : "", r.epi == 2 ? ",direct+res" : r.epi == 1 ? ",direct" : "", c.ksplit > 1 ? " splitk" : "");
    }
}

inline int fill_convdev(const aldi_conv_args* a, ConvDev& d) {
    if (!a || !a->x || !a->w || (!a->y && !a->y_f32)) return aldi_set_error_msg(ALDI_ERR_ARG, "conv_igemm: null pointer");
    const int bk = a->dtype == ALDI_BF16 ? 32 : 16;
    const int ep = a->dtype == ALDI_BF16 ? 8 : 4;
    if (a->dtype != ALDI_BF16 && a->dtype != ALDI_F32) return aldi_set_error_msg(ALDI_ERR_ARG, "conv_igemm: bad dtype");
    if (a->KH * a->KW == 1 ? (a->Cin % ep != 0) : (a->Cin % bk != 0))
        return aldi_set_error_msg(ALDI_ERR_ARG, "conv_igemm: Cin must be a multiple of 32 (bf16) / 16 (f32) for KxK convs; of a 16-B chunk for 1x1");
    if (a->Cout % 4 != 0) return aldi_set_error_msg(ALDI_ERR_ARG, "conv_igemm: Cout must be a multiple of 4");
    if (a->res_mode == 2 && ((a->Ho & 1) || (a->Wo & 1))) return aldi_set_error_msg(ALDI_ERR_ARG, "conv_igemm: upsample residual needs even Ho,Wo");
    if (a->res_mode && !a->res) return aldi_set_error_msg(ALDI_ERR_ARG, "conv_igemm: res_mode set without res");
    d.x = a->x; d.w = a->w; d.y = a->y; d.y_f32 = a->y_f32; d.scale = a->scale; d.shift = a->shift;
    d.res = a->res; d.mask = a->mask;
    d.N = a->N; d.H = a->H; d.W = a->W; d.Cin = a->Cin; d.Cout = a->Cout; d.KH = a->KH; d.KW = a->KW;
    d.stride = a->stride; d.pad = a->pad; d.Ho = a->Ho; d.Wo = a->Wo;
    d.relu = a->relu; d.res_mode = a->res_mode; d.out_scale = a->out_scale < 1 ? 1 : a->out_scale;
    d.OH = a->OH; d.OW = a->OW;
    long M = (long)a->N * a->Ho * a->Wo;
    if (M <= 0 || M > 0x7fffffffL) return aldi_set_error_msg(ALDI_ERR_ARG, "conv_igemm: bad M");
    d.M = (int)M;
    d.K = a->KH * a->KW * a->Cin;
    const size_t esz = a->dtype == ALDI_BF16 ? 2 : 4;
    const size_t xb = (size_t)a->N * a->H * a->W * a->Cin * esz, wb = (size_t)a->Cout * d.K * esz;
    const size_t yb = (size_t)a->N * (d.out_scale > 1 ? (size_t)a->OH * a->OW : (size_t)a->Ho * a->Wo) * a->Cout * esz;
    if (xb >= 0x80000000ull || wb >= 0x80000000ull || yb >= 0x80000000ull)
        return aldi_set_error_msg(ALDI_ERR_ARG, "conv_igemm: operand larger than 2 GiB (32-bit buffer offsets)");
    if (a->KH * a->KW > 16) return aldi_set_error_msg(ALDI_ERR_ARG, "conv_igemm: at most 16 taps");
    d.x_bytes = (unsigned)xb;
    d.w_bytes = (unsigned)wb;
    d.xcd = 0; d.dbg = 0;
    d.ksplit = 0; d.slabs_per_split = 0; d.lean = 0;
    d.mask_bits = static_cast<const unsigned char*>(a->mask_bits);
    d.bits_out = static_cast<unsigned char*>(a->bits_out);
    if ((a->mask_bits || a->bits_out) && (a->dtype != ALDI_BF16 || (a->Cout & 7) || d.out_scale != 1 || a->res_mode == 2 || !a->y || a->y_f32 || a->ksplit > 1))
        return aldi_set_error_msg(ALDI_ERR_ARG, "conv_igemm: bit masks take bf16 outputs with Cout % 8 == 0 in the plain layout (no fp32 output, scatter, upsampled residual or split-K)");
    if (a->mask_bits && a->mask) return aldi_set_error_msg(ALDI_ERR_ARG, "conv_igemm: mask and mask_bits are alternatives");
    return ALDI_OK;
}

inline int plan_conv(const aldi_conv_args* a, const AldiTuning& tn, ConvDev& d, Choice& c) {
    if (int rc = fill_convdev(a, d)) return rc;
    if (a->ksplit > 1) {
        const int ks = a->ksplit;
        if (a->dtype != ALDI_BF16 || a->KH * a->KW != 1 || a->stride != 1 || a->pad != 0 || a->res_mode || a->mask || a->y_f32 || !a->y || !a->ws ||
            (a->out_scale > 1) || d.K % (64 * ks) != 0 || ks > 64)
            return aldi_set_error_msg(ALDI_ERR_ARG, "conv_igemm: split-K takes bf16 plain 1x1 / linear layers with K % (64 * ksplit) == 0, a workspace, no res / mask / fp32 output");
        d.y = nullptr; d.y_f32 = static_cast<float*>(a->ws); d.scale = nullptr; d.shift = nullptr; d.relu = 0;
        d.ksplit = ks;
    }
    c = select_tile(d, tn, a->dtype != ALDI_BF16, 0);
    d.xcd = tn.igemm_xcd; d.dbg = tn.igemm_dbg;
    if (c.ksplit > 1) d.slabs_per_split = d.K / (kTiles[c.tile].KC * 8) / c.ksplit;
    return ALDI_OK;
}

inline bool conv_group_same(const aldi_conv_args* args, int n, const AldiTuning& tn) {
    bool same = n <= kMaxConvGroup && tn.igemm_group;
    for (int i = 1; i < n && same; ++i) {
        const aldi_conv_args &a = args[0], &b = args[i];
        same = a.dtype == b.dtype && a.Cin == b.Cin && a.Cout == b.Cout && a.KH == b.KH && a.KW == b.KW &&
               a.stride == b.stride && a.pad == b.pad && (a.Ho == a.H) == (b.Ho == b.H) && (a.Wo == a.W) == (b.Wo == b.W) && a.out_scale == b.out_scale &&
               (a.y != nullptr) == (b.y != nullptr) && (a.y_f32 != nullptr) == (b.y_f32 != nullptr);
    }
    return same;
}

inline int plan_conv_group(const aldi_conv_args* args, int n, const AldiTuning& tn, ConvGroup& G, ConvDev& d, Choice& c) {
    G.n = n;
    long Msum = 0;
    for (int i = 0; i < n; ++i) {
        if (int rc = fill_convdev(&args[i], G.p[i])) return rc;
        Msum += G.p[i].M;
    }
    for (int i = 1; i < n; ++i)
        for (int j = i; j > 0 && G.p[j].M > G.p[j - 1].M; --j) { const ConvDev t_ = G.p[j]; G.p[j] = G.p[j - 1]; G.p[j - 1] = t_; }
    d = G.p[0];
    d.M = (int)(Msum > 0x7fffffffL ? 0x7fffffffL : Msum);
    c = select_tile(d, tn, args[0].dtype != ALDI_BF16, n, G.p);
    d.xcd = tn.igemm_xcd; d.dbg = tn.igemm_dbg;
    return ALDI_OK;
}

}
```

aldi_amd/engine.py:

```python
from __future__ import annotations

import contextlib
import dataclasses
import inspect
import math
import os
from collections import OrderedDict
from typing import Dict, List, Optional, Sequence, Tuple

import torch

from . import ops
from .arch import FC_DIM, FPN_C, NUM_ANCHORS, POOL, STAGE_BLOCKS, Packed, ParamLayout, pad_to

PIXEL_MEAN = (103.530, 116.280, 123.675)
PIXEL_STD = (1.0, 1.0, 1.0)
ANCHOR_SIZES = (32, 64, 128, 256, 512)
ANCHOR_RATIOS = (0.5, 1.0, 2.0)
STRIDES = (4, 8, 16, 32, 64)
GMAX = 128
RPN_BATCH, RPN_POS_FRAC = 256, 0.5
ROI_BATCH, ROI_POS_FRAC = 512, 0.25
RPN_PRE = (2000, 1000)
RPN_POST = (1000, 1000)
# ... 116 lines not shown
    def folded(self, names: Sequence[str]) -> List[torch.Tensor]:
        if self._fold_plan is None:
            self._fold_names = list(names) if not self._fold_names else self._fold_names
            self._fold_plan = ops.FoldWeightsPlan([(self.w_master(n), self.scale(n)) for n in self._fold_names])
            self._fold_plan.run()
        idx = [self._fold_names.index(n) for n in names]
        return [self._fold_plan.out[i] for i in idx]

    def stem_packed(self, name: str) -> torch.Tensor:
        if self._stem_pk is None:
            self._stem_pk = ops.stem_pack_weights(self.w_master(name))
            self._stem_name = name
        return self._stem_pk

    def _wt_source(self, key: str):
        neg = key.endswith("-")
        key = key[:-1] if neg else key
        flat = key.endswith("@flat")
        name = key[:-len("@flat")] if flat else key
        w = self.w_master(name)
        if flat:
            w = w.view(w.shape[0], 1, 1, -1)
        return w, self._wt_scale(name, neg)

    def _wt_scale(self, name: str, negate: bool):
        if not negate:
            return self.scale(name)
        rows = self.layout.t[name].rows
        if rows not in self._neg1:
            self._neg1[rows] = torch.full((rows,), -1.0, dtype=torch.float32, device=self.device)
        return self._neg1[rows]

    def _refresh_wt(self):
        self._wt_dirty = False
        self._wt.clear()
        if not self._wt_keys:
            return
        if self._wt_plan is None:
            self._wt_plan = ops.DgradWeightsPlan([self._wt_source(key) for key in self._wt_keys], self.dtype)
        self._wt_plan.run()
        for key, o in zip(self._wt_keys, self._wt_plan.out):
            self._wt[key] = o

    def load_state_dict(self, sd: Dict[str, torch.Tensor]):
        missing = [k for k in self.layout.state_dict_keys() if k not in sd]
        if missing:
            raise KeyError(f"missing keys in state_dict: {missing[:5]}{'...' if len(missing) > 5 else ''}")
        self.master.copy_(self.layout.pack(sd).to(self.device))
        self.refresh()

    def state_dict(self) -> "OrderedDict[str, torch.Tensor]":
        return self.layout.unpack(self.master)

    def refresh(self, cast: bool = True):
        L = self.layout
        if L.bn_channels:
            b = L.bn_base
            c = L.bn_channels
            ops.bn_fold(self.master[b:b + c], self.master[b + c:b + 2 * c], self.master[b + 2 * c:b + 3 * c],
                        self.master[b + 3 * c:b + 4 * c], self.bn_scale, self.bn_shift, c)
        if self.dtype != torch.float32 and cast:
            ops.cast_from_f32(self.master[:L.n_weights], self.dtype, out=self.compute)
        if self._stem_pk is not None:
            ops.stem_pack_weights(self.w_master(self._stem_name), out=self._stem_pk)
        if self._fold_plan is not None:
            self._fold_plan.run()
        self._refresh_wt()

    def zero_grad(self):
        self.grad.zero_()
        self._gscale = 1.0

    def scale_grad(self, f: float):
        self._gscale = getattr(self, "_gscale", 1.0) * f

    def sgd_step(self, lr: float, momentum: float = 0.9, weight_decay: float = 1e-4, grad_scale: float = 1.0):
        n = self.layout.n_train
        ops.sgd_step(self.master, self.grad, self.mom, self.compute if self.dtype != torch.float32 else None, n, lr, momentum,
                     weight_decay, grad_scale * getattr(self, "_gscale", 1.0), self.first_step, self.dtype)
        self._after_sgd()

    def _after_sgd(self):
        self.first_step = False
        if self.lazy_wt:
            self._wt_dirty = True
        else:
            self._refresh_wt()

    def sgd_range_dev(self, lo: int, hi: int, hyper: torch.Tensor):
        hi = min(hi, self.layout.n_train)
        if hi > lo:
            ops.sgd_step_dev(self.master, self.grad, self.mom, self.compute if self.dtype != torch.float32 else None, lo, hi, hyper, self.dtype)

    def ema_from(self, student: "Weights", alpha: float, copy_only: bool):
        n = self.layout.n_total
        if self.dtype == torch.bfloat16:
            ops.ema_update(self.master, student.master, self.compute, n, alpha, copy_only, self.dtype, n_compute=self.layout.n_weights)
            self.refresh(cast=False)
        else:
            ops.ema_update(self.master, student.master, None, n, alpha, copy_only, torch.float32)
            self.refresh()


def make_anchors(shapes: Sequence[Tuple[int, int]], device, sizes: Sequence[float] = ANCHOR_SIZES) -> torch.Tensor:
    out = []
    for (h, w), size, stride in zip(shapes, sizes, STRIDES):
        cell = []
        for r in ANCHOR_RATIOS:
            area = size ** 2.0
            aw = math.sqrt(area / r)
            ah = r * aw
            cell.append([-aw / 2.0, -ah / 2.0, aw / 2.0, ah / 2.0])
        cell = torch.tensor(cell, dtype=torch.float32)
        sx = torch.arange(0, w * stride, step=stride, dtype=torch.float32)
        sy = torch.arange(0, h * stride, step=stride, dtype=torch.float32)
        yy, xx = torch.meshgrid(sy, sx, indexing="ij")
        shifts = torch.stack((xx.reshape(-1), yy.reshape(-1), xx.reshape(-1), yy.reshape(-1)), dim=1)
        out.append((shifts.view(-1, 1, 4) + cell.view(1, -1, 4)).reshape(-1, 4))
    return torch.cat(out).contiguous().to(device)


@dataclasses.dataclass(frozen=True)
class D2Params:
    pixel_mean: Tuple[float, ...] = PIXEL_MEAN
    pixel_std: Tuple[float, ...] = PIXEL_STD
    anchor_sizes: Tuple[float, ...] = ANCHOR_SIZES
    rpn_batch: int = RPN_BATCH
    rpn_pos_frac: float = RPN_POS_FRAC
    rpn_iou: Tuple[float, float] = (0.3, 0.7)
    rpn_pre: Tuple[int, int] = RPN_PRE
    rpn_post: Tuple[int, int] = RPN_POST
    rpn_nms: float = RPN_NMS
    roi_batch: int = ROI_BATCH
    roi_pos_frac: float = ROI_POS_FRAC
    roi_iou: float = 0.5
    roi_weights: Tuple[float, float, float, float] = ROI_WEIGHTS
    score_thresh: float = SCORE_THRESH
    nms_test: float = NMS_TEST
    dets: int = DETS

    @classmethod
    def from_cfg(cls, cfg) -> "D2Params":
        M = cfg.MODEL

        def get(node, key, default):
            return node.get(key, default) if hasattr(node, "get") else getattr(node, key, default)

        def need(cond, what):
            if not cond:
                raise ValueError(f"aldi_amd R50-FPN engine: unsupported config value: {what}")
        rpn, roi, box, ag = M.RPN, M.ROI_HEADS, get(M, "ROI_BOX_HEAD", {}), M.ANCHOR_GENERATOR
        sizes = [list(s_) for s_ in ag.SIZES]
        need(len(sizes) == 5 and all(len(s_) == 1 for s_ in sizes), f"ANCHOR_GENERATOR.SIZES {sizes} (one size per level p2..p6)")
        ratios = [list(r_) for r_ in ag.ASPECT_RATIOS]
        need(all(tuple(float(v) for v in r_) == ANCHOR_RATIOS for r_ in ratios), f"ANCHOR_GENERATOR.ASPECT_RATIOS {ratios} (kernels: {ANCHOR_RATIOS})")
        need(len(M.PIXEL_MEAN) == 3 and len(M.PIXEL_STD) == 3, "PIXEL_MEAN / PIXEL_STD must have 3 entries")
        need(list(get(rpn, "IN_FEATURES", ["p2", "p3", "p4", "p5", "p6"])) == ["p2", "p3", "p4", "p5", "p6"], "RPN.IN_FEATURES")
        need(list(get(roi, "IN_FEATURES", ["p2", "p3", "p4", "p5"])) == ["p2", "p3", "p4", "p5"], "ROI_HEADS.IN_FEATURES")
        need(tuple(get(rpn, "BBOX_REG_WEIGHTS", (1.0, 1.0, 1.0, 1.0))) == (1.0, 1.0, 1.0, 1.0), "RPN.BBOX_REG_WEIGHTS != (1, 1, 1, 1)")
        need(float(get(rpn, "SMOOTH_L1_BETA", 0.0)) == 0.0 and float(get(box, "SMOOTH_L1_BETA", 0.0)) == 0.0, "SMOOTH_L1_BETA != 0 (the losses are pure L1)")
        need(get(rpn, "BBOX_REG_LOSS_TYPE", "smooth_l1") == "smooth_l1" and get(box, "BBOX_REG_LOSS_TYPE", "smooth_l1") == "smooth_l1", "BBOX_REG_LOSS_TYPE")
        need(float(get(rpn, "LOSS_WEIGHT", 1.0)) == 1.0 and float(get(rpn, "BBOX_REG_LOSS_WEIGHT", 1.0)) == 1.0, "RPN loss weights != 1")
        need(int(get(box, "POOLER_RESOLUTION", POOL)) == POOL and int(get(box, "POOLER_SAMPLING_RATIO", 0)) == 0 and
             get(box, "POOLER_TYPE", "ROIAlignV2") == "ROIAlignV2", "ROI_BOX_HEAD pooler (kernels: ROIAlignV2, 7x7, adaptive sampling)")
        need(not get(box, "CLS_AGNOSTIC_BBOX_REG", False), "CLS_AGNOSTIC_BBOX_REG")
        need(get(roi, "PROPOSAL_APPEND_GT", True), "ROI_HEADS.PROPOSAL_APPEND_GT False")
        need(len(rpn.IOU_THRESHOLDS) == 2 and len(roi.IOU_THRESHOLDS) == 1, "IOU_THRESHOLDS (RPN: two, ROI heads: one)")
        pre = (int(rpn.PRE_NMS_TOPK_TRAIN), int(rpn.PRE_NMS_TOPK_TEST))
        post = (int(rpn.POST_NMS_TOPK_TRAIN), int(rpn.POST_NMS_TOPK_TEST))
        need(max(pre) <= 2048 and min(pre + post) >= 1, f"RPN.PRE_NMS_TOPK {pre} (the NMS workspace holds 2048 boxes per level and image)")
        dets = int(get(get(cfg, "TEST", {}), "DETECTIONS_PER_IMAGE", DETS))
        need(1 <= dets <= GMAX, f"TEST.DETECTIONS_PER_IMAGE {dets} (<= {GMAX}: pseudo-label rows)")
        need(int(rpn.BATCH_SIZE_PER_IMAGE) >= 1 and int(roi.BATCH_SIZE_PER_IMAGE) >= 1, "BATCH_SIZE_PER_IMAGE")
        return cls(pixel_mean=tuple(float(v) for v in M.PIXEL_MEAN), pixel_std=tuple(float(v) for v in M.PIXEL_STD),
                   anchor_sizes=tuple(float(s_[0]) for s_ in sizes), rpn_batch=int(rpn.BATCH_SIZE_PER_IMAGE), rpn_pos_frac=float(rpn.POSITIVE_FRACTION),
                   rpn_iou=(float(rpn.IOU_THRESHOLDS[0]), float(rpn.IOU_THRESHOLDS[1])), rpn_pre=pre, rpn_post=post, rpn_nms=float(rpn.NMS_THRESH),
                   roi_batch=int(roi.BATCH_SIZE_PER_IMAGE), roi_pos_frac=float(roi.POSITIVE_FRACTION), roi_iou=float(roi.IOU_THRESHOLDS[0]),
                   roi_weights=tuple(float(v) for v in get(box, "BBOX_REG_WEIGHTS", ROI_WEIGHTS)), score_thresh=float(roi.SCORE_THRESH_TEST),
                   nms_test=float(roi.NMS_THRESH_TEST), dets=dets)


def raise_on_error(code: int, who: str = "engine"):
    if code & 1:
        raise FloatingPointError(f"{who}: predicted boxes or scores contain Inf/NaN. Training has diverged.")
    if code & 2:
        raise RuntimeError(f"{who}: sparse RPN-head backward: more active pixels than (2 * BATCH_SIZE_PER_IMAGE + 4 * positives) per image; "
                           "the excess was dropped, gradients of this step are wrong -- or, from the detection post-processing: a row of class "
                           "scores contains Inf/NaN; the row was dropped")
    if code & 4:
        raise RuntimeError(f"{who}: detection post-processing: more than 8192 candidates above SCORE_THRESH_TEST in one image; the excess was dropped")
    if code & 8:
        raise RuntimeError(f"{who}: RPN top-k: the group barrier of `topk_fused_kernel` timed out (its workgroups were not co-resident); the candidates "
                           "of this step are wrong.  Set ALDI_RPN_TOPK_FUSED=0 for the five-launch path")
    if code:
        raise RuntimeError(f"{who}: device error word {code}")


class Ctx(dict):
    __getattr__ = dict.__getitem__
    __setattr__ = dict.__setitem__


class RCNN:
    p = D2Params()

    def __init__(self, weights: Weights, num_classes: int, params: Optional[D2Params] = None):
        self.wts = weights
        if params is not None:
            self.p = params
        self.K = num_classes
        self.device, self.dtype = weights.device, weights.dtype
        self.Cp = weights.layout.t["box_pred"].rows
        self.Ch = weights.layout.t["rpn_head_out"].rows
        self._anchor_cache: Dict[tuple, tuple] = {}
        self._ws: Dict[str, torch.Tensor] = {}
        self.err = torch.zeros(1, dtype=torch.int32, device=self.device)
        torch.set_num_threads(1)
        idx = lambda n: int(n.rsplit(".", 1)[1])
        names = list(getattr(weights.layout, "t", {}))
        self.img_da_layers = sorted((n for n in names if n.startswith("img_align.model.")), key=idx)
        self.ins_da_layers = sorted((n for n in names if n.startswith("ins_align.model.")), key=idx)
        self.has_img_da, self.has_ins_da = bool(self.img_da_layers), bool(self.ins_da_layers)
        self.fused_stem = os.environ.get("ALDI_FUSED_STEM", "1") == "1"
        self.wgrad_tail_split = int(os.environ.get("ALDI_WGRAD_TAIL_SPLIT", "2"))
        self.group_wgrad = os.environ.get("ALDI_WGRAD_GROUP", "1") == "1"
        self.mask_bits = os.environ.get("ALDI_MASK_BITS", "1") == "1"
        self.mask_bits_inner = os.environ.get("ALDI_MASK_BITS_INNER", "1") == "1"
        self.level_groups = os.environ.get("ALDI_LEVEL_GROUPS", "1") == "1"
        self.fused_res2 = os.environ.get("ALDI_FUSED_RES2", "1") == "1"
        self.fused_res2_shortcut = os.environ.get("ALDI_FUSED_RES2_SHORTCUT", "1") == "1"
        self._wg_queue: list = []
        self.sparse_rpn_backward = os.environ.get("ALDI_RPN_SPARSE_BWD", "1") == "1"
        spec = getattr(weights.layout, "img_da", None)
        self.img_da_level = ("p2", "p3", "p4", "p5", "p6").index(spec["layer"]) if spec else 0

    def stage_images(self, images: Sequence[torch.Tensor]):
        sizes = [(int(im.shape[1]), int(im.shape[2])) for im in images]
        Hs = pad_to(max(s[0] for s in sizes), 32)
        Ws = pad_to(max(s[1] for s in sizes), 32)
        N = len(images)
        if all(im.is_cuda for im in images):
            st = torch.zeros((N, 3, Hs, Ws), dtype=torch.uint8, device=self.device)
            for i, im in enumerate(images):
                st[i, :, : sizes[i][0], : sizes[i][1]] = im
        else:
            host = torch.zeros((N, 3, Hs, Ws), dtype=torch.uint8).pin_memory()
            for i, im in enumerate(images):
                host[i, :, : sizes[i][0], : sizes[i][1]] = im
            st = host.to(self.device, non_blocking=True)
        hw = torch.tensor(sizes, dtype=torch.int32).to(self.device)
        return st, sizes, hw

    def stage_gt(self, instances: Sequence[dict]):
        N = len(instances)
        gb = torch.zeros((N, GMAX, 4), dtype=torch.float32)
        gc = torch.zeros((N, GMAX), dtype=torch.int32)
        cnt = torch.zeros((N,), dtype=torch.int32)
        on_dev = []
        for i, inst in enumerate(instances):
            b = inst["gt_boxes"]
            b = b.tensor if hasattr(b, "tensor") else b
            g = int(b.shape[0])
            if g > GMAX:
                raise ValueError(f"more than {GMAX} GT boxes in one image")
            if g:
                if b.is_cuda:
                    on_dev.append((i, g, b, inst["gt_classes"]))
                else:
                    gb[i, :g] = b.reshape(-1, 4).to(torch.float32)
                    gc[i, :g] = inst["gt_classes"].to(torch.int32)
            cnt[i] = g
        gbd, gcd, cntd = ops.upload_packed([gb, gc, cnt], self.device)
        for i, g, b, cl in on_dev:
            gbd[i, :g] = b.reshape(-1, 4).to(torch.float32)
            gcd[i, :g] = cl.to(torch.int32)
        return {"boxes": gbd, "classes": gcd, "count": cntd, "host_count": cnt.tolist()}

    def geometry(self, Hs: int, Ws: int):
        key = (Hs, Ws)
        if key not in self._anchor_cache:
            shapes = []
            h, w = Hs // 4, Ws // 4
            for l in range(4):
                shapes.append((h, w))
                if l < 3:
                    h, w = h // 2, w // 2
            shapes.append(((shapes[3][0] - 1) // 2 + 1, (shapes[3][1] - 1) // 2 + 1))
            geom = ops.make_geom(shapes, NUM_ANCHORS, self.Ch)
            anchors = make_anchors(shapes, self.device, getattr(self, "anchor_sizes", self.p.anchor_sizes))
            self._anchor_cache[key] = (shapes, geom, anchors)
            while len(self._anchor_cache) > 16:
                self._anchor_cache.pop(next(iter(self._anchor_cache)))
        else:
            self._anchor_cache[key] = self._anchor_cache.pop(key)
        return self._anchor_cache[key]

    def workspace(self, name: str, nbytes: int) -> torch.Tensor:
        t = self._ws.get(name)
        if t is None or t.numel() < nbytes:
            t = torch.empty(nbytes, dtype=torch.uint8, device=self.device)
            self._ws[name] = t
        return t

    def _conv_call(self, x, name, *, relu=False, res=None, res_mode=0, want_f32=False, out=None, bits_out=None):
        W = self.wts
        p = W.layout.t[name]
        return x, W.w(name), dict(stride=p.stride, pad=p.pad, scale=W.scale(name), shift=W.shift(name), res=res, res_mode=res_mode, relu=relu,
                                  want_f32=want_f32, out=out, bits_out=bits_out)

    def conv(self, x, name, **kw):
        x, w, kw = self._conv_call(x, name, **kw)
        return ops.conv2d(x, w, **kw)

    def _serve(self, req):
        if isinstance(req, list):
            return ops.conv2d_group([self._conv_call(r[0], r[1], **r[2]) for r in req])
        return self.conv(req[0], req[1], **req[2])

    def _drive(self, gen):
        try:
            req = next(gen)
            while True:
                req = gen.send(self._serve(req))
        except StopIteration as e:
            return e.value

    @staticmethod
    def drive_pair(eng_a, gen_a, eng_b, gen_b, streams=None):
        res = [None, None]
        ctx_a = torch.cuda.stream(streams[0]) if streams else contextlib.nullcontext()
        ctx_b = torch.cuda.stream(streams[1]) if streams else contextlib.nullcontext()
        try:
            with ctx_a:
                ra = next(gen_a)
        except StopIteration as e:
            ra, res[0] = None, e.value
        try:
            with ctx_b:
                rb = next(gen_b)
        except StopIteration as e:
            rb, res[1] = None, e.value
        while ra is not None or rb is not None:
            if streams:
                if ra is not None:
                    with ctx_a:
                        ya = eng_a._serve(ra)
                        try:
                            ra = gen_a.send(ya)
                        except StopIteration as e:
                            ra, res[0] = None, e.value
                if rb is not None:
                    with ctx_b:
                        yb = eng_b._serve(rb)
                        try:
                            rb = gen_b.send(yb)
                        except StopIteration as e:
                            rb, res[1] = None, e.value
                continue
            if ra is not None and rb is not None:
                la, lb = (ra if isinstance(ra, list) else [ra]), (rb if isinstance(rb, list) else [rb])
                ys = ops.conv2d_group([eng_a._conv_call(r[0], r[1], **r[2]) for r in la] + [eng_b._conv_call(r[0], r[1], **r[2]) for r in lb])
                ya = ys[:len(la)] if isinstance(ra, list) else ys[0]
                yb = ys[len(la):] if isinstance(rb, list) else ys[len(la)]
            elif ra is not None:
                ya = eng_a._serve(ra)
            else:
                yb = eng_b._serve(rb)
            if ra is not None:
                try:
                    ra = gen_a.send(ya)
                except StopIteration as e:
                    ra, res[0] = None, e.value
            if rb is not None:
                try:
                    rb = gen_b.send(yb)
                except StopIteration as e:
                    rb, res[1] = None, e.value
        return res[0], res[1]

    def trunk(self, st_u8: torch.Tensor, sizes, save: bool) -> Ctx:
        return self._drive(self.trunk_steps(st_u8, sizes, save))

    def prefix_pipelinable(self) -> bool:
        return type(self) is RCNN and self.dtype == torch.bfloat16 and self.fused_stem and self.fused_res2

    def trunk_steps(self, st_u8: torch.Tensor, sizes, save: bool, fpn: bool = True, pre: Optional[torch.Tensor] = None,
                    prefix_out: Optional[torch.Tensor] = None):
        W = self.wts
        c = Ctx()
        bu = "backbone.bottom_up."
        if pre is not None:
            x = pre
        elif self.dtype == torch.bfloat16 and self.fused_stem:
            x = ops.stem_pool_forward(st_u8, sizes, W.stem_packed(bu + "stem.conv1"), W.scale(bu + "stem.conv1"), W.shift(bu + "stem.conv1"),
                                      self.p.pixel_mean, self.p.pixel_std)
        else:
            stem = ops.stem_forward(st_u8, sizes, W.w_master(bu + "stem.conv1"), W.scale(bu + "stem.conv1"), W.shift(bu + "stem.conv1"),
                                    self.p.pixel_mean, self.p.pixel_std, self.dtype)
            x = ops.maxpool3s2(stem)
            del stem
        blocks = []
        cs = []
        out_bits = {}
        fuse2 = self.dtype == torch.bfloat16 and self.fused_res2
        if fuse2:
            res2 = [f"{bu}res2.{b}.conv{k}" for b in range(STAGE_BLOCKS[0]) for k in (1, 2, 3)]
            fw = dict(zip(res2, W.folded(res2)))
        assert prefix_out is None or (fuse2 and pre is None)
        for si, nb in enumerate(STAGE_BLOCKS):
            if si == 0 and pre is not None:
                cs.append(x)
                continue
            for b in range(nb):
                p = f"{bu}res{si + 2}.{b}."
                if si == 0 and fuse2:
                    fold_sc = b == 0 and self.fused_res2_shortcut
                    sc = (yield x, p + "shortcut", {}) if b == 0 and not fold_sc else x
                    x = ops.bottleneck_fused(x, sc, fw[p + "conv1"], fw[p + "conv2"], fw[p + "conv3"], W.shift(p + "conv1"), W.shift(p + "conv2"),
                                             W.shift(p + "conv3"), out=prefix_out if (prefix_out is not None and b == nb - 1) else None,
                                             shortcut=(W.w(p + "shortcut"), W.scale(p + "shortcut"), W.shift(p + "shortcut")) if fold_sc else None)
                    continue
                sc = (yield x, p + "shortcut", {}) if b == 0 else x
                want_bits = save and si > 0 and self.mask_bits and self.dtype == torch.bfloat16

                def bits_for(inp, name):
                    if not want_bits:
                        return None
                    lt = W.layout.t[name]
                    ho = (inp.shape[1] + 2 * lt.pad - lt.kk) // lt.stride + 1
                    wo = (inp.shape[2] + 2 * lt.pad - lt.kk) // lt.stride + 1
                    return torch.empty(inp.shape[0] * ho * wo * (lt.wshape[0] // 8), dtype=torch.uint8, device=self.device)
                b1 = bits_for(x, p + "conv1") if self.mask_bits_inner else None
                h1 = yield x, p + "conv1", dict(relu=True, bits_out=b1)
                b2 = bits_for(h1, p + "conv2") if self.mask_bits_inner else None
                h2 = yield h1, p + "conv2", dict(relu=True, bits_out=b2)
                bits = bits_for(h2, p + "conv3")
                out = yield h2, p + "conv3", dict(relu=True, res=sc, res_mode=1, bits_out=bits)
                if save and si > 0:
                    blocks.append((p, x, h1, h2, out, b == 0))
                    if bits is not None:
                        out_bits[out.data_ptr()] = bits
                        if b1 is not None:
                            out_bits[h1.data_ptr()], out_bits[h2.data_ptr()] = b1, b2
                x = out
            cs.append(x)
            if prefix_out is not None:
                return x
        if not fpn:
            if save:
                c.blocks, c.cs, c.out_bits = blocks, cs, out_bits
            else:
                c.cs = cs
            return c
        prev = {}
        P = {}
        prev[5] = yield cs[3], "backbone.fpn_lateral5", {}
        if self.level_groups:
            for lvl in (4, 3, 2):
                prev[lvl] = yield cs[lvl - 2], f"backbone.fpn_lateral{lvl}", dict(res=prev[lvl + 1], res_mode=2)
            outs = yield [(prev[lvl], f"backbone.fpn_output{lvl}", {}) for lvl in (2, 3, 4, 5)]
            P.update(zip((2, 3, 4, 5), outs))
        else:
            P[5] = yield prev[5], "backbone.fpn_output5", {}
            for lvl in (4, 3, 2):
                prev[lvl] = yield cs[lvl - 2], f"backbone.fpn_lateral{lvl}", dict(res=prev[lvl + 1], res_mode=2)
                P[lvl] = yield prev[lvl], f"backbone.fpn_output{lvl}", {}
        P[6] = ops.subsample2(P[5])
        c.P = [P[2], P[3], P[4], P[5], P[6]]
        if save:
            c.blocks, c.cs, c.prev, c.out_bits = blocks, cs, prev, out_bits
        return c

    def rpn_head(self, c: Ctx, save: bool):
        self._drive(self.rpn_head_steps(c, save))

    def rpn_head_steps(self, c: Ctx, save: bool):
        px = [f.shape[0] * f.shape[1] * f.shape[2] for f in c.P]
        flat = torch.empty((1, sum(px), 1, FPN_C), dtype=self.dtype, device=self.device)
        ts, o, reqs = [], 0, []
        for f, n in zip(c.P, px):
            view = flat[0, o:o + n, 0].view(f.shape[0], f.shape[1], f.shape[2], FPN_C)
            reqs.append((f, "proposal_generator.rpn_head.conv", dict(relu=True, out=view)))
            o += n
        if self.level_groups:
            ts = yield reqs
        else:
            for r in reqs:
                ts.append((yield r))
        hf = yield flat, "rpn_head_out", dict(want_f32=True)
        heads, o = [], 0
        for f, n in zip(c.P, px):
            heads.append(hf[0, o:o + n, 0].view(f.shape[0], f.shape[1], f.shape[2], hf.shape[3]))
            o += n
        c.head, c.head_flat = heads, hf
        if save:
            c.rpn_t = ts

    def box_head(self, pooled: torch.Tensor, c: Optional[Ctx] = None):
        R = pooled.shape[0]
        x = pooled.view(R, 1, 1, POOL * POOL * FPN_C)
        fc1 = self.conv(x, "roi_heads.box_head.fc1", relu=True)
        bits2 = None
        if c is not None and self.mask_bits and self.dtype == torch.bfloat16 and R > 0 and os.environ.get("ALDI_MASK_BITS_FC", "1") == "1":
            bits2 = torch.empty(R * (FC_DIM // 8), dtype=torch.uint8, device=self.device)
        fc2 = self.conv(fc1, "roi_heads.box_head.fc2", relu=True, bits_out=bits2)
        pred = self.conv(fc2, "box_pred", want_f32=True).view(R, self.Cp)
        if c is not None:
            c.pooled, c.fc1, c.fc2 = pooled, fc1, fc2
            if bits2 is not None:
                if c.get("out_bits") is None:
                    c.out_bits = {}
                c.out_bits[fc2.data_ptr()] = bits2
        return pred, fc2

    def roi_feats(self, c: Ctx, grads=None):
        return ops.make_roi_feats(c.P[:4], grads, [1.0 / s for s in STRIDES[:4]])

    def _sample_host(self, counts: List[List[int]], batch: int, frac: float):
        N = len(counts)
        S = batch
        sel = torch.zeros((N, 2, S), dtype=torch.int32)
        nsel = torch.zeros((N, 2), dtype=torch.int32)
        for n, (npos, nneg) in enumerate(counts):
            num_pos = min(npos, int(batch * frac))
            num_neg = min(nneg, batch - num_pos)
            perm1 = randperm_prefix(npos, num_pos)
            perm2 = randperm_prefix(nneg, num_neg)
            sel[n, 0, :num_pos] = perm1.to(torch.int32)
            sel[n, 1, :num_neg] = perm2.to(torch.int32)
            nsel[n, 0], nsel[n, 1] = num_pos, num_neg
        return sel, nsel, nsel.tolist()

    def _sample(self, counts: List[List[int]], batch: int, frac: float):
        sel, nsel, h = self._sample_host(counts, batch, frac)
        sel_d, nsel_d = ops.upload_packed([sel, nsel], self.device)
        return sel_d, nsel_d, h

    def rpn_match(self, geom, anchors, gt, N):
        sumA = anchors.shape[0]
        dev = self.device
        best_iou = torch.empty((N, sumA), dtype=torch.float32, device=dev)
        best_idx = torch.empty((N, sumA), dtype=torch.int32, device=dev)
        labels = torch.empty((N, sumA), dtype=torch.int32, device=dev)
        scratch = ops.box_match_scratch(N, GMAX, dev)
        ops.box_match(anchors, 0, None, sumA, gt["boxes"], gt["count"], GMAX, N, self.p.rpn_iou[0], self.p.rpn_iou[1], True, best_iou, best_idx, scratch, labels)
        lists = torch.empty((N, 2, sumA), dtype=torch.int32, device=dev)
        counts = torch.empty((N, 2), dtype=torch.int32, device=dev)
        ops.compact_labels(labels, sumA, N, 0, lists, counts)
        return labels, best_idx, lists, counts

    def rpn_sample(self, lists, counts, N, host_counts=None):
        if host_counts is None:
            both = torch.cat([counts.view(-1), self.err.view(-1)]).cpu().tolist()
            raise_on_error(both[-1])
            host_counts = [both[2 * i: 2 * i + 2] for i in range(N)]
        lists = lists.contiguous()
        sel, nsel, nsel_h = self._sample(host_counts, self.p.rpn_batch, self.p.rpn_pos_frac)
        L_ = lists.shape[2]
        labels = torch.empty((N, L_), dtype=torch.int32, device=self.device)
        ops.rpn_apply_sample(labels, L_, N, lists, sel, nsel, self.p.rpn_batch)
        n_fg = sum(a for a, _ in nsel_h)
        n_valid = sum(a + b for a, b in nsel_h)
        return labels, n_valid, n_fg, host_counts

    def proposals(self, c: Ctx, geom, anchors, hw, N, training: bool):
        nl = 5
        ws = self.workspace("rpn", ops.rpn_proposals_workspace(N, nl))
        post = self.p.rpn_post[0 if training else 1]
        boxes = torch.empty((N, post, 4), dtype=torch.float32, device=self.device)
        scores = torch.empty((N, post), dtype=torch.float32, device=self.device)
        count = torch.empty((N,), dtype=torch.int32, device=self.device)
        ops.rpn_proposals(geom, c.head, anchors, hw, N, self.p.rpn_pre[0 if training else 1], post, self.p.rpn_nms, ws, boxes, scores, count, self.err)
        return boxes, scores, count

    def forward_train(self, images, instances, *, roi_seed: Optional[int] = None, pre_roi_hook=None,
                      gt_dev: Optional[dict] = None, do_align: bool = False, labeled: bool = True,
                      da_weights: Tuple[float, float] = (0.0, 0.0)) -> Ctx:
        N = len(images)
        st, sizes, hw = self.stage_images(images)
        shapes, geom, anchors = self.geometry(st.shape[2], st.shape[3])
        gt = gt_dev if gt_dev is not None else self.stage_gt(instances)
        c = self.trunk(st, sizes, save=True)
        c.N, c.sizes, c.hw, c.geom, c.anchors, c.gt, c.shapes = N, sizes, hw, geom, anchors, gt, shapes
        self.rpn_head(c, save=True)
        dev = self.device
        _, matched, lists, counts = self.rpn_match(geom, anchors, gt, N)
        labels, _, _, c.rpn_host_counts = self.rpn_sample(lists, counts, N)
        c.rpn_labels, c.rpn_matched, c.rpn_lists, c.rpn_counts = labels, matched, lists, counts
        c.loss_rpn = torch.zeros(2, dtype=torch.float32, device=dev)
        ops.rpn_loss(geom, c.head, None, anchors, labels, matched, gt["boxes"], gt["count"], GMAX, N, 1.0 / (self.p.rpn_batch * N), 0.0, 0.0, c.loss_rpn)
        c.props, c.prop_scores, c.prop_count = self.proposals(c, geom, anchors, hw, N, training=True)
        if pre_roi_hook is not None:
            pre_roi_hook()
        if roi_seed is not None:
            torch.manual_seed(roi_seed)
        self.roi_sample(c, c.props, c.prop_count, gt, N)
        self.roi_forward(c)
        c.loss_box = torch.zeros(2, dtype=torch.float32, device=dev)
        ops.box_loss(c.pred, self.Cp, self.K, c.R, c.rois, c.r_cls, c.r_gt, self.p.roi_weights, 0.0, 0.0, None, c.loss_box)
        c.align = {}
        c.distill = None
        c.labeled, c.da_weights = labeled, da_weights
        if do_align:
            self.align_forward(c, labeled, da_weights)
        return c

    def forward_train_fused(self, specs: List[dict]) -> Ctx:
        dev = self.device
        images = [im for sp in specs for im in sp["images"]]
        N = len(images)
        st, sizes, hw = self.stage_images(images)
        shapes, geom, anchors = self.geometry(st.shape[2], st.shape[3])
        c = self.trunk(st, sizes, save=True)
        c.N, c.sizes, c.hw, c.geom, c.anchors, c.shapes = N, sizes, hw, geom, anchors, shapes
        self.rpn_head(c, save=True)
        side = self._wgrad_stream()
        if side is not None:
            side.wait_stream(torch.cuda.current_stream())
            with torch.cuda.stream(side):
                c.props, c.prop_scores, c.prop_count = self.proposals(c, geom, anchors, hw, N, training=True)
        else:
            c.props, c.prop_scores, c.prop_count = self.proposals(c, geom, anchors, hw, N, training=True)
        for sp in specs:
            if sp.get("gt_lazy") is not None:
                sp["gt_dev"] = sp["gt_lazy"]()
        for sp in specs:
            if sp.get("gt_wait") is not None:
                sp["gt_wait"]()
        gts = [sp["gt_dev"] if sp.get("gt_dev") is not None else self.stage_gt(sp["instances"]) for sp in specs]
        gt = {k: torch.cat([g[k] for g in gts]) for k in ("boxes", "classes", "count")}
        c.gt = gt
        _, matched, lists, counts = self.rpn_match(geom, anchors, gt, N)
        if side is not None:
            torch.cuda.current_stream().wait_stream(side)
        prep = self._roi_prepare(c.props, c.prop_count, gt, N)
        both = torch.cat([counts.view(-1), prep["counts"].view(-1), self.err.view(-1)]).cpu().tolist()
        raise_on_error(both[-1], "student")
        rpn_counts = [both[2 * i: 2 * i + 2] for i in range(N)]
        roi_counts = [both[2 * N + 2 * i: 2 * N + 2 * i + 2] for i in range(N)]
        rsel, rnsel, rh, osel, onsel, oh = [], [], [], [], [], []
        n0 = 0
        chunks = []
        for sp in specs:
            n1 = n0 + len(sp["images"])
            if sp.get("pre_rpn"):
                sp["pre_rpn"]()
            a, b, h_ = self._sample_host(rpn_counts[n0:n1], self.p.rpn_batch, self.p.rpn_pos_frac)
            rsel.append(a); rnsel.append(b); rh += h_
            if sp.get("pre_roi"):
                sp["pre_roi"]()
            a, b, h2 = self._sample_host(roi_counts[n0:n1], self.p.roi_batch, self.p.roi_pos_frac)
            osel.append(a); onsel.append(b); oh += h2
            chunks.append(dict(n0=n0, n1=n1, labeled=sp.get("labeled", True), do_align=sp.get("do_align", False),
                               da_weights=sp.get("da_weights", (0.0, 0.0)), rpn_counts=rpn_counts[n0:n1], roi_counts=roi_counts[n0:n1]))
            n0 = n1
        labels = torch.empty((N, anchors.shape[0]), dtype=torch.int32, device=dev)
        rsel_d, rnsel_d, osel_d, onsel_d = ops.upload_packed([torch.cat(rsel), torch.cat(rnsel), torch.cat(osel), torch.cat(onsel)], dev)
        ops.rpn_apply_sample(labels, anchors.shape[0], N, lists, rsel_d, rnsel_d, self.p.rpn_batch)
        c.rpn_labels, c.rpn_matched, c.rpn_lists, c.rpn_counts = labels, matched, lists, counts
        self._roi_gather(c, prep, osel_d, onsel_d, oh, gt, N)
        r0 = 0
        for ch, sp in zip(chunks, specs):
            r1 = r0 + sum(c.rows[ch["n0"]:ch["n1"]])
            if sp.get("post_rois") is not None:
                sp["post_rois"](c, ch["n0"], r0, r1)
            r0 = r1
        self.roi_forward(c)
        r0 = 0
        for ch in chunks:
            n0, n1 = ch["n0"], ch["n1"]
            r1 = r0 + sum(c.rows[n0:n1])
            ch["r0"], ch["r1"] = r0, r1
            ch["loss_rpn"] = torch.zeros(2, dtype=torch.float32, device=dev)
            ch["loss_box"] = torch.zeros(2, dtype=torch.float32, device=dev)
            nc = n1 - n0
            ops.rpn_loss(geom, [h[n0:n1] for h in c.head], None, anchors, labels[n0:n1], matched[n0:n1], gt["boxes"][n0:n1], gt["count"][n0:n1],
                         GMAX, nc, 1.0 / (self.p.rpn_batch * nc), 0.0, 0.0, ch["loss_rpn"])
            ops.box_loss(c.pred[r0:r1], self.Cp, self.K, r1 - r0, c.rois[r0:r1], c.r_cls[r0:r1], c.r_gt[r0:r1], self.p.roi_weights, 0.0, 0.0, None, ch["loss_box"])
            ch["align"] = {}
            ch["distill"] = None
            if ch["do_align"]:
                self._align_forward_chunk(c, ch)
            r0 = r1
        c.chunks = chunks
        c.align = {}
        c.distill = None
        return c

    def _align_forward_chunk(self, c: Ctx, ch: dict):
        dev = self.device
        label = 1.0 if ch["labeled"] else 0.0
        n0, n1, r0, r1 = ch["n0"], ch["n1"], ch["r0"], ch["r1"]
        if self.has_img_da:
            acts, pooled, logit = self._img_disc_forward(c.P[self.img_da_level][n0:n1])
            ch["loss_da_img"] = torch.zeros(1, dtype=torch.float32, device=dev)
            ops.domain_bce(logit, logit.shape[-1], n1 - n0, label, ch["da_weights"][0], 0.0, None, ch["loss_da_img"])
            ch["align"]["img"] = (acts, pooled, logit)
        if self.has_ins_da and r1 > r0:
            acts, logit = self._ins_disc_forward(c.fc2[r0:r1])
            ch["loss_da_ins"] = torch.zeros(1, dtype=torch.float32, device=dev)
            ops.domain_bce(logit, logit.shape[-1], r1 - r0, label, ch["da_weights"][1], 0.0, None, ch["loss_da_ins"])
            ch["align"]["ins"] = (acts, logit)

    def _img_disc_forward(self, feat: torch.Tensor):
        acts = [feat]
        for name in self.img_da_layers[:-1]:
            acts.append(self.conv(acts[-1], name, relu=True))
        pooled = ops.avgpool(acts[-1])
        return acts, pooled, self.conv(pooled, self.img_da_layers[-1], want_f32=True)

    def _ins_disc_forward(self, feat: torch.Tensor):
        acts = [feat]
        for name in self.ins_da_layers[:-1]:
            acts.append(self.conv(acts[-1], name, relu=True))
        return acts, self.conv(acts[-1], self.ins_da_layers[-1], want_f32=True)

    def distill_forward_chunk(self, c: Ctx, ch: dict, teacher_head, teacher_pred, labels, n_valid, n_fg, values=True, **kw):
        dev = self.device
        n0, n1, r0, r1 = ch["n0"], ch["n1"], ch["r0"], ch["r1"]
        ch["distill"] = dict(t_head=teacher_head, t_pred=teacher_pred, labels=labels, n_valid=n_valid, n_fg=n_fg, **kw)
        if not values:
            return
        ch["loss_dist_rpn"] = torch.zeros(2, dtype=torch.float32, device=dev)
        ch["loss_dist_roi"] = torch.zeros(2, dtype=torch.float32, device=dev)
        ops.rpn_distill_loss(c.geom, [h[n0:n1] for h in c.head], teacher_head, None, labels, n1 - n0, kw["obj_T"], n_valid, n_fg,
                             kw["do_obj"], kw["do_rpn_reg"], 0.0, ch["loss_dist_rpn"], counts_dev=kw.get("counts_dev"))
        ops.roih_distill_loss(c.pred[r0:r1], teacher_pred, self.Cp, self.K, r1 - r0, kw["cls_T"], kw["kl"], kw["do_cls"], kw["do_roih_reg"],
                              0.0, None, ch["loss_dist_roi"])

    def chunk_loss_dict(self, ch: dict) -> "OrderedDict[str, torch.Tensor]":
        d = OrderedDict()
        d["loss_cls"], d["loss_box_reg"] = ch["loss_box"][0], ch["loss_box"][1]
        d["loss_rpn_cls"], d["loss_rpn_loc"] = ch["loss_rpn"][0], ch["loss_rpn"][1]
        if "img" in ch["align"]:
            d["loss_da_img"] = ch["loss_da_img"][0]
        if "ins" in ch["align"]:
            d["loss_da_ins"] = ch["loss_da_ins"][0]
        return d

    def chunk_distill_loss_dict(self, ch: dict) -> "OrderedDict[str, torch.Tensor]":
        d = OrderedDict()
        k = ch["distill"]
        if k["do_obj"]:
            d["loss_obj_bce"] = ch["loss_dist_rpn"][0]
        if k["do_rpn_reg"]:
            d["loss_rpn_l1"] = ch["loss_dist_rpn"][1]
        if k["do_cls"]:
            d["loss_cls_ce"] = ch["loss_dist_roi"][0]
        if k["do_roih_reg"]:
            d["loss_roih_l1"] = ch["loss_dist_roi"][1]
        return d

    def backward_fused(self, c: Ctx, scales: List[Dict[str, float]], after_losses=None):
        T, dev = self.dtype, self.device
        early = c.get("rpn_early")
        if early is not None and early.get("arena_box") is not None and self._aux_stream() is not None:
            arena, c.gpred = early["arena_box"], early["gpred"]
            torch.cuda.current_stream().wait_event(early["ev_zero"])
        else:
            arena = torch.zeros(2 + 8 * len(c.chunks), dtype=torch.float32, device=dev)
            c.gpred = torch.zeros((max(c.R, 1), self.Cp), dtype=torch.float32, device=dev)
        scratch = arena[:2]
        aux0 = self._aux_stream() if early is not None else None
        if aux0 is None:
            early = None
        rpn_ctx = (lambda: torch.cuda.stream(aux0)) if early is not None else contextlib.nullcontext
        if early is not None and early.get("ev") is not None:
            aux0.wait_event(early["ev"])
        hf = c.get("head_flat")
        with rpn_ctx():
            rpn_arena = arena
            if early is not None:
                rpn_arena = early["arena"]
                rpn_arena.zero_()
            if hf is not None:
                gf, o = (early["gf"].zero_() if early is not None else torch.zeros_like(hf)), 0
                c.ghead = []
                for h in c.head:
                    n = h.shape[0] * h.shape[1] * h.shape[2]
                    c.ghead.append(gf[0, o:o + n, 0].view(h.shape))
                    o += n
            else:
                c.ghead = [torch.zeros_like(h) for h in c.head]
        gt = c.gt
        align_list = []
        box_fused = [] if (c.R > 0 and len(c.chunks) <= 8 and self.Cp % 2 == 0 and os.environ.get("ALDI_BOX_LOSS_FUSED", "1") == "1") else None
        c.gpred_lo = None
        for ci, (ch, sc_) in enumerate(zip(c.chunks, scales)):
            sc = lambda k: float(sc_.get(k, 0.0))
            n0, n1, r0, r1 = ch["n0"], ch["n1"], ch["r0"], ch["r1"]
            nc = n1 - n0
            heads = [h[n0:n1] for h in c.head]
# ... 609 lines not shown
```

aldi_amd/ops.py:

```python
from __future__ import annotations

import ctypes as C
import os
from typing import List, Optional, Sequence

import torch

from . import _lib as L


def dtype_code(t: torch.dtype) -> int:
    if t == torch.float32:
        return L.F32
    if t == torch.bfloat16:
        return L.BF16
    raise TypeError(f"unsupported dtype {t}")


def _p(t: Optional[torch.Tensor]):
    return None if t is None else t.data_ptr()


_RAW_STREAM = getattr(torch._C, "_cuda_getCurrentRawStream", None)


def stream_ptr() -> int:
    if _RAW_STREAM is not None:
        return _RAW_STREAM(torch.cuda.current_device())
    return torch.cuda.current_stream().cuda_stream


def upload_packed(tensors, device):
    metas, off = [], 0
    for t in tensors:
        nb = t.numel() * t.element_size()
        metas.append((off, nb))
        off += (nb + 15) // 16 * 16
    host = torch.empty(max(off, 16), dtype=torch.uint8).pin_memory()
    for t, (o, nb) in zip(tensors, metas):
        if nb:
            host[o:o + nb] = t.contiguous().view(-1).view(torch.uint8)
    dev = host.to(device, non_blocking=True)
    return [dev[o:o + nb].view(t.dtype).view(t.shape) for t, (o, nb) in zip(tensors, metas)]


def conv2d(x: torch.Tensor, w: torch.Tensor, *, stride: int = 1, pad: int = 0,
           scale: Optional[torch.Tensor] = None, shift: Optional[torch.Tensor] = None,
           res: Optional[torch.Tensor] = None, res_mode: int = 0, relu: bool = False,
           mask: Optional[torch.Tensor] = None, out: Optional[torch.Tensor] = None,
           out_f32: Optional[torch.Tensor] = None, want_f32: bool = False,
           out_scale: int = 1, out_hw=None, ksplit: Optional[int] = None, mask_bits: Optional[torch.Tensor] = None,
           bits_out: Optional[torch.Tensor] = None) -> torch.Tensor:
    N, H, W_, Cin = x.shape
    Cout, KH, KW, Cin2 = w.shape
    assert Cin == Cin2 and x.is_contiguous() and w.is_contiguous() and x.dtype == w.dtype, (x.shape, w.shape, x.dtype, w.dtype)
    Ho = (H + 2 * pad - KH) // stride + 1
    Wo = (W_ + 2 * pad - KW) // stride + 1
    if out_scale > 1:
        OH, OW = out_hw
        shape = (N, OH, OW, Cout)
    else:
        OH = OW = 0
        shape = (N, Ho, Wo, Cout)
    if out is None and not want_f32:
        out = torch.empty(shape, dtype=x.dtype, device=x.device)
    if want_f32 and out_f32 is None:
        out_f32 = torch.empty(shape, dtype=torch.float32, device=x.device)
    ws = None
    if ksplit is None:
        ksplit = _auto_ksplit(x, N * Ho * Wo, Cout, KH * KW * Cin, KH * KW == 1 and stride == 1 and pad == 0 and res is None and mask is None
                              and not want_f32 and out_f32 is None and out_scale == 1 and mask_bits is None and bits_out is None)
    if ksplit and ksplit > 1:
        ws = torch.empty(ksplit * N * Ho * Wo * Cout, dtype=torch.float32, device=x.device)
    a = L.ConvArgs(_p(x), _p(w), _p(out), _p(out_f32), _p(scale), _p(shift), _p(res), _p(mask),
                   N, H, W_, Cin, Cout, KH, KW, stride, pad, Ho, Wo,
                   int(relu), res_mode, out_scale, OH, OW, dtype_code(x.dtype), _p(ws), int(ksplit or 0), _p(mask_bits), _p(bits_out))
    L.call("aldi_conv_igemm", C.byref(a), stream_ptr())
    return out_f32 if want_f32 and out is None else out


def _auto_ksplit(x, M, Cout, K, plain: bool) -> int:
    if not plain or x.dtype != torch.bfloat16 or K < 4096 or K % 256 or os.environ.get("ALDI_SPLITK", "1") != "1":
        return 0
    tiles = ((M + 127) // 128) * ((Cout + 127) // 128)
    if not (16 <= tiles <= 160) or Cout % 4:
        return 0
    tiles256 = ((M + 255) // 256) * ((Cout + 127) // 128)
    for ks in (2, 4, 7, 8, 14, 16):
        if K % (64 * ks) == 0 and tiles256 * ks >= 216:
            return ks
    return 4 if K % 256 == 0 else 0


def _conv_args(x, w, *, stride=1, pad=0, scale=None, shift=None, res=None, res_mode=0, relu=False, mask=None, out=None, out_f32=None,
               want_f32=False, out_scale=1, out_hw=None, mask_bits=None, bits_out=None):
    N, H, W_, Cin = x.shape
    Cout, KH, KW, Cin2 = w.shape
    assert Cin == Cin2 and x.is_contiguous() and w.is_contiguous() and x.dtype == w.dtype, (x.shape, w.shape, x.dtype, w.dtype)
    Ho = (H + 2 * pad - KH) // stride + 1
    Wo = (W_ + 2 * pad - KW) // stride + 1
    if out_scale > 1:
        OH, OW = out_hw
        shape = (N, OH, OW, Cout)
    else:
        OH = OW = 0
        shape = (N, Ho, Wo, Cout)
    if out is None and not want_f32:
        out = torch.empty(shape, dtype=x.dtype, device=x.device)
    if want_f32 and out_f32 is None:
        out_f32 = torch.empty(shape, dtype=torch.float32, device=x.device)
    a = L.ConvArgs(_p(x), _p(w), _p(out), _p(out_f32), _p(scale), _p(shift), _p(res), _p(mask),
                   N, H, W_, Cin, Cout, KH, KW, stride, pad, Ho, Wo,
                   int(relu), res_mode, out_scale, OH, OW, dtype_code(x.dtype), None, 0, _p(mask_bits), _p(bits_out))
    return a, (out_f32 if want_f32 and out is None else out)


def conv2d_group(calls) -> List[torch.Tensor]:
    arr = (L.ConvArgs * len(calls))()
    outs = []
    for i, (x, w, kw) in enumerate(calls):
        arr[i], y = _conv_args(x, w, **kw)
        outs.append(y)
    L.call("aldi_conv_igemm_group", arr, len(calls), stream_ptr())
    return outs


_WGRAD_WS = {}
WGRAD_WS_EPOCH = 0
WGRAD_ORDERED = os.environ.get("ALDI_WGRAD_ORDERED", "1") != "0"


def _wgrad_workspace(arr, n: int, device) -> None:
    if not WGRAD_ORDERED:
        return
    need = L.lib.aldi_conv_wgrad_group_workspace(arr, n)
    if need < 0:
        raise RuntimeError("aldi_conv_wgrad_group_workspace: " + L.lib.aldi_last_error().decode())
    if need == 0:
        need = 256
    key = (device, stream_ptr())
    buf = _WGRAD_WS.get(key)
    if buf is None or buf.numel() * 4 < need:
        global WGRAD_WS_EPOCH
        if buf is not None:
            WGRAD_WS_EPOCH += 1
            if torch.cuda.is_current_stream_capturing():
                raise RuntimeError("the weight-gradient workspace has to grow during a hipGraph capture: run the new shapes eagerly once first")
        else:
            need = max([need] + [b.numel() * 4 for (d_, _), b in _WGRAD_WS.items() if d_ == device])
        buf = torch.empty((need + (need >> 2) + 3) // 4, dtype=torch.float32, device=device)
        _WGRAD_WS[key] = buf
    arr[0].ws = buf.data_ptr()
    arr[0].ws_bytes = buf.numel() * 4


def conv_wgrad(x: torch.Tensor, g: torch.Tensor, dw: torch.Tensor, *, KH: int, KW: int, stride: int = 1, pad: int = 0,
               scale: Optional[torch.Tensor] = None, db: Optional[torch.Tensor] = None) -> None:
    N, H, W_, Cin = x.shape
    _, Ho, Wo, Cout = g.shape
    assert dw.dtype == torch.float32 and dw.numel() == Cout * KH * KW * Cin and x.dtype == g.dtype, (dw.shape, x.shape, g.shape)
    arr = (L.WgradArgs * 1)()
    arr[0] = L.WgradArgs(_p(x), _p(g), _p(dw), _p(scale), N, H, W_, Cin, Cout, KH, KW, stride, pad, Ho, Wo, dtype_code(x.dtype), _p(db), None, 0)
    if x.dtype == torch.bfloat16:
        _wgrad_workspace(arr, 1, x.device)
    L.call("aldi_conv_wgrad", arr, stream_ptr())


def conv_wgrad_group(problems) -> None:
    arr = (L.WgradArgs * len(problems))()
    for i, (x, g, dw, kw) in enumerate(problems):
        N, H, W_, Cin = x.shape
        _, Ho, Wo, Cout = g.shape
        KH, KW = kw["KH"], kw["KW"]
        assert dw.dtype == torch.float32 and dw.numel() == Cout * KH * KW * Cin and x.dtype == g.dtype, (dw.shape, x.shape, g.shape)
        arr[i] = L.WgradArgs(_p(x), _p(g), _p(dw), _p(kw.get("scale")), N, H, W_, Cin, Cout, KH, KW, kw.get("stride", 1), kw.get("pad", 0), Ho, Wo,
                             dtype_code(x.dtype), _p(kw.get("db")), None, 0)
    _wgrad_workspace(arr, len(problems), problems[0][0].device)
    L.call("aldi_conv_wgrad_group", arr, len(problems), stream_ptr())


def noop() -> None:
    L.call("aldi_noop", stream_ptr())


def bias_grad(g: torch.Tensor, db: torch.Tensor) -> None:
    Cc = g.shape[-1]
    L.call("aldi_bias_grad", _p(g), _p(db), g.numel() // Cc, Cc, dtype_code(g.dtype), stream_ptr())


def dgrad_weights(w_master: torch.Tensor, scale: Optional[torch.Tensor], dtype: torch.dtype,
                  out: Optional[torch.Tensor] = None) -> torch.Tensor:
    Cout, KH, KW, Cin = w_master.shape
    if out is None:
        out = torch.empty((Cin, KH, KW, Cout), dtype=dtype, device=w_master.device)
    L.call("aldi_dgrad_weights", _p(w_master), _p(scale), _p(out), Cout, KH, KW, Cin, dtype_code(dtype), stream_ptr())
    return out


class DgradWeightsPlan:

    def __init__(self, entries, dtype: torch.dtype):
        dev = entries[0][0].device
        self.dtype = dtype
        self.keep = list(entries)
        sizes = [w.numel() for w, _ in entries]
        offs, tot = [], 0
        for n in sizes:
            offs.append(tot)
            tot += (n + 63) // 64 * 64
        self.buf = torch.empty(tot, dtype=dtype, device=dev)
        self.out = []
        items = (L.DgwItem * len(entries))()
        tile = 0
        for i, (w, sc) in enumerate(entries):
            Cout, KH, KW, Cin = w.shape
            o = self.buf[offs[i]:offs[i] + sizes[i]].view(Cin, KH, KW, Cout)
            self.out.append(o)
            it = items[i]
            it.w_master, it.scale, it.wt = w.data_ptr(), (sc.data_ptr() if sc is not None else None), o.data_ptr()
            it.Cout, it.KH, it.KW, it.Cin, it.tile_begin, it.reserved = Cout, KH, KW, Cin, tile, 0
            tile += KH * KW * ((Cout + 31) // 32) * ((Cin + 31) // 32)
        self.total_tiles = tile
        self.n = len(entries)
        raw = torch.frombuffer(bytearray(bytes(items)), dtype=torch.uint8)
        self.items = raw.to(dev)

    def run(self):
        L.call("aldi_dgrad_weights_batch", _p(self.items), self.n, self.total_tiles, dtype_code(self.dtype), stream_ptr())


class FoldWeightsPlan:

    def __init__(self, entries):
        dev = entries[0][0].device
        self.keep = list(entries)
        sizes = [w.numel() for w, _ in entries]
        offs, tot = [], 0
        for n in sizes:
            assert n % 8 == 0
            offs.append(tot)
            tot += (n + 63) // 64 * 64
        self.buf = torch.empty(tot, dtype=torch.bfloat16, device=dev)
        self.out = []
        items = (L.FoldItem * len(entries))()
        chunk = 0
        for i, (w, sc) in enumerate(entries):
            assert w.dtype == torch.float32 and w.is_contiguous() and w.data_ptr() % 16 == 0, "fold_weights: fp32, contiguous, 16-byte aligned"
            o = self.buf[offs[i]:offs[i] + sizes[i]].view(w.shape)
            self.out.append(o)
            it = items[i]
            it.w, it.scale, it.out = w.data_ptr(), (sc.data_ptr() if sc is not None else None), o.data_ptr()
            it.rows, it.cols, it.chunk_begin, it.reserved = w.shape[0], sizes[i] // w.shape[0], chunk, 0
            chunk += sizes[i] // 8
        self.total_chunks, self.n = chunk, len(entries)
        self.items = torch.frombuffer(bytearray(bytes(items)), dtype=torch.uint8).to(dev)

    def run(self):
        L.call("aldi_fold_weights_batch", _p(self.items), self.n, self.total_chunks, stream_ptr())


def bottleneck_fused(x: torch.Tensor, res: torch.Tensor, w1, w2, w3, b1, b2, b3, out: Optional[torch.Tensor] = None, *,
                     shortcut=None) -> torch.Tensor:
    N, H, W_, Cin = x.shape
    mid, Cout = w1.shape[0], w3.shape[0]
    assert x.dtype == torch.bfloat16 and x.is_contiguous()
    assert w1.numel() == mid * Cin and w2.numel() == mid * 9 * mid and w3.numel() == Cout * mid and w1.dtype == torch.bfloat16
    if out is None:
        out = torch.empty((N, H, W_, Cout), dtype=x.dtype, device=x.device)
    if shortcut is not None:
        wsc, ssc, bsc = shortcut
        assert wsc.dtype == torch.bfloat16 and wsc.is_contiguous() and wsc.numel() == Cout * Cin, wsc.shape
        assert ssc.dtype == bsc.dtype == torch.float32 and ssc.numel() == bsc.numel() == Cout
        a = L.BottleneckArgs(_p(x), None, _p(out), _p(w1), _p(w2), _p(w3), _p(b1), _p(b2), _p(b3), N, H, W_, Cin, mid, Cout)
        L.call("aldi_bottleneck_fused_sc", C.byref(a), _p(wsc), _p(ssc), _p(bsc), stream_ptr())
        return out
    assert res.is_contiguous() and res.shape == (N, H, W_, Cout), (x.shape, res.shape)
    a = L.BottleneckArgs(_p(x), _p(res), _p(out), _p(w1), _p(w2), _p(w3), _p(b1), _p(b2), _p(b3), N, H, W_, Cin, mid, Cout)
    L.call("aldi_bottleneck_fused", C.byref(a), stream_ptr())
    return out


def stem_forward(img_u8: torch.Tensor, sizes: Sequence[Sequence[int]], w: torch.Tensor, scale: torch.Tensor, shift: torch.Tensor,
                 mean: Sequence[float], std: Sequence[float], dtype: torch.dtype) -> torch.Tensor:
    N, _, Hs, Ws = img_u8.shape
    Hc, Wc = Hs // 2, Ws // 2
    y = torch.empty((N, Hc, Wc, 64), dtype=dtype, device=img_u8.device)
    a = L.StemArgs()
    a.img, a.w, a.scale, a.shift, a.y = _p(img_u8), _p(w), _p(scale), _p(shift), _p(y)
    a.N, a.Hs, a.Ws, a.Hc, a.Wc = N, Hs, Ws, Hc, Wc
    for i, (h, w_) in enumerate(sizes):
        a.h[i], a.w_img[i] = int(h), int(w_)
    for c in range(3):
        a.mean[c], a.std[c] = float(mean[c]), float(std[c])
    a.dtype = dtype_code(dtype)
    L.call("aldi_stem_forward", C.byref(a), stream_ptr())
    return y


def stem_pack_weights(w: torch.Tensor, out: Optional[torch.Tensor] = None) -> torch.Tensor:
    if out is None:
        out = torch.empty((64, 200), dtype=torch.bfloat16, device=w.device)
    L.call("aldi_stem_pack_weights", _p(w), _p(out), stream_ptr())
    return out


def stem_pool_forward(img_u8: torch.Tensor, sizes: Sequence[Sequence[int]], w_packed: torch.Tensor, scale: torch.Tensor, shift: torch.Tensor,
                      mean: Sequence[float], std: Sequence[float]) -> torch.Tensor:
    N, _, Hs, Ws = img_u8.shape
    Hc, Wc = Hs // 2, Ws // 2
    y = torch.empty((N, (Hc - 1) // 2 + 1, (Wc - 1) // 2 + 1, 64), dtype=torch.bfloat16, device=img_u8.device)
    a = L.StemArgs()
    a.img, a.w, a.scale, a.shift, a.y = _p(img_u8), None, _p(scale), _p(shift), None
    a.N, a.Hs, a.Ws, a.Hc, a.Wc = N, Hs, Ws, Hc, Wc
    for i, (h, w_) in enumerate(sizes):
        a.h[i], a.w_img[i] = int(h), int(w_)
    for c in range(3):
        a.mean[c], a.std[c] = float(mean[c]), float(std[c])
    a.dtype = L.BF16
    L.call("aldi_stem_pool_forward", C.byref(a), _p(w_packed), _p(y), stream_ptr())
    return y


def maxpool3s2(x: torch.Tensor) -> torch.Tensor:
    N, H, W_, Cc = x.shape
    y = torch.empty((N, (H - 1) // 2 + 1, (W_ - 1) // 2 + 1, Cc), dtype=x.dtype, device=x.device)
    L.call("aldi_maxpool3s2", _p(x), _p(y), N, H, W_, Cc, dtype_code(x.dtype), stream_ptr())
    return y


def subsample2(x: torch.Tensor) -> torch.Tensor:
    N, H, W_, Cc = x.shape
    y = torch.empty((N, (H - 1) // 2 + 1, (W_ - 1) // 2 + 1, Cc), dtype=x.dtype, device=x.device)
    L.call("aldi_subsample2", _p(x), _p(y), N, H, W_, Cc, 0, dtype_code(x.dtype), stream_ptr())
    return y


def subsample2_bwd(g_small: torch.Tensor, g_big: torch.Tensor) -> None:
    N, H, W_, Cc = g_big.shape
    L.call("aldi_subsample2", _p(g_small), _p(g_big), N, H, W_, Cc, 1, dtype_code(g_big.dtype), stream_ptr())


def upsample2_bwd(g: torch.Tensor, out: torch.Tensor, accumulate: bool) -> None:
    N, Hc, Wc, Cc = out.shape
    assert g.shape == (N, Hc * 2, Wc * 2, Cc)
    L.call("aldi_upsample2_bwd", _p(g), _p(out), N, Hc, Wc, Cc, int(accumulate), dtype_code(g.dtype), stream_ptr())


def upsample2_bwd_chain(g2: torch.Tensor, o3: torch.Tensor, o4: torch.Tensor, o5: torch.Tensor) -> None:
    N, H5, W5, Cc = o5.shape
    assert o4.shape == (N, H5 * 2, W5 * 2, Cc) and o3.shape == (N, H5 * 4, W5 * 4, Cc) and g2.shape == (N, H5 * 8, W5 * 8, Cc)
    L.call("aldi_upsample2_bwd_chain", _p(g2), _p(o3), _p(o4), _p(o5), N, H5, W5, Cc, dtype_code(g2.dtype), stream_ptr())


def add_f32(a: Optional[torch.Tensor], b: Optional[torch.Tensor], out: torch.Tensor, relu_src: Optional[torch.Tensor] = None) -> torch.Tensor:
    L.call("aldi_add_f32", _p(a), _p(b), _p(relu_src), _p(out), out.numel(), dtype_code(out.dtype), stream_ptr())
    return out


def cast_from_f32(src: torch.Tensor, dtype: torch.dtype, out: Optional[torch.Tensor] = None) -> torch.Tensor:
    if out is None:
        out = torch.empty(src.shape, dtype=dtype, device=src.device)
    L.call("aldi_cast_from_f32", _p(src), _p(out), src.numel(), dtype_code(dtype), stream_ptr())
    return out


def sgd_step(p, g, buf, p_compute, n, lr, momentum, weight_decay, grad_scale, first_step, dtype) -> None:
    L.call("aldi_sgd_step", _p(p), _p(g), _p(buf), _p(p_compute), n, lr, momentum, weight_decay, grad_scale, int(first_step),
           dtype_code(dtype), stream_ptr())


def sgd_step_dev(p, g, buf, p_compute, lo: int, hi: int, hyper: torch.Tensor, dtype) -> None:
    pc = None if p_compute is None else p_compute.data_ptr() + lo * p_compute.element_size()
    L.call("aldi_sgd_step_dev", p.data_ptr() + 4 * lo, g.data_ptr() + 4 * lo, buf.data_ptr() + 4 * lo, pc, hi - lo, _p(hyper), dtype_code(dtype), stream_ptr())


def ema_update(teacher, student, teacher_compute, n, alpha, copy_only, dtype, n_compute=None) -> None:
    nc = 0 if teacher_compute is None else (teacher_compute.numel() if n_compute is None else n_compute)
    L.call("aldi_ema_update", _p(teacher), _p(student), _p(teacher_compute), n, nc, alpha, int(copy_only), dtype_code(dtype), stream_ptr())


def bn_fold(w, b, mean, var, scale, shift, Cc) -> None:
    L.call("aldi_bn_fold", _p(w), _p(b), _p(mean), _p(var), _p(scale), _p(shift), Cc, stream_ptr())


def make_geom(shapes: Sequence[Sequence[int]], A: int, Cc: int) -> L.RpnGeom:
    g = L.RpnGeom()
    g.num_levels, g.A, g.C = len(shapes), A, Cc
    off = 0
    for i, (h, w) in enumerate(shapes):
        g.H[i], g.W[i], g.off[i] = h, w, off
        off += h * w * A
    for i in range(len(shapes), L.MAX_LEVELS + 1):
        g.off[i] = off
    return g


def ptrs(ts: Optional[Sequence[Optional[torch.Tensor]]]):
    if ts is None:
        return None
    arr = L.PtrArray5()
    for i, t in enumerate(ts):
        arr[i] = _p(t)
    return arr


def box_match(boxes, box_stride_n, box_count, Lb, gt_boxes, gt_count, Gmax, N, lo, hi, lowq, best_iou, best_idx, scratch, labels):
    L.call("aldi_box_match", _p(boxes), box_stride_n, _p(box_count), Lb, _p(gt_boxes), _p(gt_count), Gmax, N, lo, hi, int(lowq),
           _p(best_iou), _p(best_idx), _p(scratch), scratch.numel() * scratch.element_size(), _p(labels), stream_ptr())


def box_match_scratch(N: int, Gmax: int, device) -> torch.Tensor:
    return torch.empty((N, Gmax * 32), dtype=torch.int32, device=device)


def stage_images(images, batch: torch.Tensor) -> None:
    n = len(images)
    ptr = (C.c_void_p * n)(*[_p(im) for im in images])
    hs = (C.c_int * n)(*[int(im.shape[1]) for im in images])
    ws = (C.c_int * n)(*[int(im.shape[2]) for im in images])
    L.call("aldi_stage_images", ptr, hs, ws, n, batch.shape[1], batch.shape[2], batch.shape[3], _p(batch), stream_ptr())


def compact_labels(labels, Lb, N, bg, lists, counts):
    ws = torch.empty(max(int(L.lib.aldi_compact_labels_workspace(Lb, N)), 16), dtype=torch.uint8, device=labels.device)
    L.call("aldi_compact_labels", _p(labels), Lb, N, bg, _p(lists), _p(counts), _p(ws), stream_ptr())


# ... 186 lines not shown
```

include/aldi_hip.h:

```cpp
#ifndef ALDI_HIP_H
#define ALDI_HIP_H
#include <stddef.h>
#include <stdint.h>

#ifdef __cplusplus
extern "C" {
#endif

typedef void* aldi_stream_t;

enum { ALDI_F32 = 0, ALDI_BF16 = 1 };
enum { ALDI_OK = 0, ALDI_ERR_HIP = -1, ALDI_ERR_ARG = -2 };

const char* aldi_last_error(void);
int aldi_version(void);
int aldi_noop(aldi_stream_t stream);

int aldi_set_tuning(const char* name, int value);
int aldi_get_tuning(const char* name, int* value);
int aldi_reset_tuning(void);
const char* aldi_last_dispatch(void);

typedef struct {
    const void* x;
    const void* w;
    void* y;
    float* y_f32;
    const float* scale;
    const float* shift;
    const void* res;
    const void* mask;
    int N, H, W, Cin;
    int Cout, KH, KW, stride, pad;
    int Ho, Wo;
    int relu;
    int res_mode;
    int out_scale;
    int OH, OW;
    int dtype;
    void* ws;
    int ksplit;
    const void* mask_bits;
    void* bits_out;
} aldi_conv_args;

int aldi_conv_igemm(const aldi_conv_args* a, aldi_stream_t stream);
int aldi_conv_igemm_group(const aldi_conv_args* args, int n, aldi_stream_t stream);
int aldi_conv_igemm_plan(const aldi_conv_args* args, int n, char* name, int cap);

typedef struct {
    const void* x;
    const void* g;
    float* dw;
    const float* scale;
    int N, H, W, Cin, Cout, KH, KW, stride, pad, Ho, Wo;
    int dtype;
    float* db;
    void* ws;
    long ws_bytes;
} aldi_wgrad_args;
int aldi_conv_wgrad(const aldi_wgrad_args* a, aldi_stream_t stream);

int aldi_conv_wgrad_group(const aldi_wgrad_args* args, int n, aldi_stream_t stream);
long aldi_conv_wgrad_group_workspace(const aldi_wgrad_args* args, int n);
int aldi_conv_wgrad_plan(const aldi_wgrad_args* args, int n, int group, char* name, int cap, long* ws_bytes);

int aldi_bias_grad(const void* g, float* db, int M, int C, int dtype, aldi_stream_t stream);

int aldi_dgrad_weights(const float* w_master, const float* scale, void* wt, int Cout, int KH, int KW, int Cin,
                       int dtype, aldi_stream_t stream);

typedef struct aldi_dgw_item {
    const float* w_master;
    const float* scale;
    void* wt;
    int Cout, KH, KW, Cin;
    int tile_begin, reserved;
} aldi_dgw_item;
int aldi_dgrad_weights_batch(const aldi_dgw_item* items, int n_items, int total_tiles, int dtype, aldi_stream_t stream);

typedef struct aldi_bottleneck_args {
    const void* x;
    const void* res;
    void* y;
    const void* w1; const void* w2; const void* w3;
    const float* b1; const float* b2; const float* b3;
    int N, H, W, Cin, mid, Cout;
} aldi_bottleneck_args;
int aldi_bottleneck_fused(const aldi_bottleneck_args* a, aldi_stream_t stream);
int aldi_bottleneck_fused_sc(const aldi_bottleneck_args* a, const void* wsc, const float* sc_scale, const float* sc_shift, aldi_stream_t stream);
typedef struct aldi_fold_item {
    const float* w; const float* scale; void* out;
    int rows, cols, chunk_begin, reserved;
} aldi_fold_item;
int aldi_fold_weights_batch(const aldi_fold_item* items, int n_items, int total_chunks, aldi_stream_t stream);

#define ALDI_MAX_IMAGES 16

typedef struct {
    const uint8_t* img;
    const float* w;
    const float* scale; const float* shift;
    void* y;
    int N, Hs, Ws, Hc, Wc;
    int h[ALDI_MAX_IMAGES], w_img[ALDI_MAX_IMAGES];
    float mean[3], std[3];
    int dtype;
} aldi_stem_args;
int aldi_stem_forward(const aldi_stem_args* a, aldi_stream_t stream);
int aldi_stem_pack_weights(const float* w, void* w_packed, aldi_stream_t stream);
int aldi_stem_pool_forward(const aldi_stem_args* a, const void* w_packed, void* y_pool, aldi_stream_t stream);

int aldi_maxpool3s2(const void* x, void* y, int N, int H, int W, int C, int dtype, aldi_stream_t stream);
int aldi_stage_images(const void* const* images, const int* heights, const int* widths, int n, int C, int Hs, int Ws, void* batch,
                      aldi_stream_t stream);
int aldi_subsample2(const void* x, void* y, int N, int H, int W, int C, int backward, int dtype, aldi_stream_t stream);
int aldi_upsample2_bwd(const void* g, void* out, int N, int Hc, int Wc, int C, int accumulate, int dtype, aldi_stream_t stream);
int aldi_upsample2_bwd_chain(const void* g2, void* o3, void* o4, void* o5, int N, int H5, int W5, int C, int dtype, aldi_stream_t stream);
int aldi_add_f32(const void* a, const float* b, const void* relu_src, void* out, long n, int dtype, aldi_stream_t stream);
int aldi_cast_from_f32(const float* src, void* dst, long n, int dtype, aldi_stream_t stream);

int aldi_sgd_step(float* p, const float* g, float* buf, void* p_compute, long n, float lr, float momentum, float weight_decay,
                  float grad_scale, int first_step, int dtype, aldi_stream_t stream);
int aldi_sgd_step_dev(float* p, const float* g, float* buf, void* p_compute, long n, const float* hyper, int dtype, aldi_stream_t stream);
int aldi_ema_update(float* teacher, const float* student, void* teacher_compute, long n, long n_compute, double alpha, int copy_only, int dtype,
                    aldi_stream_t stream);
int aldi_bn_fold(const float* w, const float* b, const float* mean, const float* var, float* scale, float* shift, int C, aldi_stream_t stream);

#define ALDI_MAX_LEVELS 5
typedef struct {
    int num_levels;
    int A;
    int C;
    int H[ALDI_MAX_LEVELS], W[ALDI_MAX_LEVELS];
    int off[ALDI_MAX_LEVELS + 1];
} aldi_rpn_geom;

int aldi_box_match(const float* boxes, long box_stride_n, const int* box_count, int L,
                   const float* gt_boxes, const int* gt_count, int Gmax, int N,
                   float lo, float hi, int allow_low_quality,
                   float* best_iou, int* best_idx, unsigned* gt_best_scratch, size_t gt_best_bytes, int* labels, aldi_stream_t stream);
size_t aldi_compact_labels_workspace(int L, int N);
int aldi_compact_labels(const int* labels, int L, int N, int bg_label, int* lists, int* counts, void* workspace, aldi_stream_t stream);
int aldi_rpn_apply_sample(int* labels, int L, int N, const int* lists, const int* sel, const int* nsel, int S, aldi_stream_t stream);
int aldi_rpn_loss(const aldi_rpn_geom* gm, float* const* head, float* const* grad, const float* anchors, const int* labels, const int* matched,
                  const float* gt_boxes, const int* gt_count, int Gmax, int N, float inv_norm, float grad_scale_cls, float grad_scale_loc,
                  float* loss2, aldi_stream_t stream);
size_t aldi_rpn_proposals_workspace(int N, int num_levels);
int aldi_rpn_proposals(const aldi_rpn_geom* gm, float* const* head, const float* anchors, const int* img_hw, int N,
                       int pre_nms_topk, int post_nms_topk, float nms_thresh, void* workspace,
                       float* out_boxes, float* out_scores, int* out_count, int* err_flag, aldi_stream_t stream);

size_t aldi_rpn_active_pixels_workspace(const aldi_rpn_geom* gm, int N);
int aldi_rpn_active_pixels(const aldi_rpn_geom* gm, float* const* grad_head, int N, int cap, int* idx, int* count, void* workspace,
                           int* err_flag, aldi_stream_t stream);
int aldi_rpn_sparse_gather(const aldi_rpn_geom* gm, float* const* grad_head, const void* const* hidden, const void* const* feat, int N, int Cf,
                           int cap, const int* idx, const int* count, void* G, void* Tm, void* X9, int dtype, aldi_stream_t stream);
int aldi_rpn_sparse_scatter(const aldi_rpn_geom* gm, void* const* gfeat, const void* Y, int N, int Cf, int cap, const int* idx,
                            const int* count, int dtype, int grad_dtype, aldi_stream_t stream);

typedef struct {
    const void* feat[4];
    float* grad[4];
    int H[4], W[4];
    float scale[4];
    int C;
} aldi_roi_feats;

int aldi_roi_prepare(const float* props, const int* pcount, int P, const float* gt_boxes, const int* gt_classes, const int* gt_count,
                     int Gmax, int N, int K, float iou_thresh, float* cand, int* ccount, float* best_iou, int* best_idx,
                     unsigned* gt_best_scratch, int* labels, int* cls, aldi_stream_t stream);
int aldi_roi_prepare_lists(const float* props, const int* pcount, int P, const float* gt_boxes, const int* gt_classes, const int* gt_count,
                           int Gmax, int N, int K, float iou_thresh, float* cand, int* ccount, float* best_iou, int* best_idx, int* labels,
                           int* cls, int* lists, int* counts, unsigned* tickets, const int* tail_a, const int* tail_b, aldi_stream_t stream);
int aldi_roi_gather(const float* cand, const int* cls, const int* best_idx, int L, const int* lists, const int* sel, const int* nsel, int S,
                    const int* row_off, const float* gt_boxes, const int* gt_count, int Gmax, int N,
                    float* rois, int* r_cls, float* r_gt, int* r_idx, aldi_stream_t stream);
int aldi_rois_from_proposals(const float* props, const int* pcount, int P, int N, float* rois, aldi_stream_t stream);
int aldi_roialign(const aldi_roi_feats* f, const float* rois, int R, int P, void* pooled, int backward, int dtype, aldi_stream_t stream);
int aldi_roialign_backward(const aldi_roi_feats* f, const float* rois, int R, int P, const void* g_pooled, int N, int rois_sorted, int dtype,
                           int grad_dtype, aldi_stream_t stream);

int aldi_box_loss(const float* pred, int Cp, int K, int R, const float* rois, const int* cls, const float* gt_boxes,
                  const float* weights4, float grad_scale_cls, float grad_scale_box, float* grad, float* loss2, aldi_stream_t stream);
typedef struct {
    int r0, r1;
    float grad_scale_cls, grad_scale_box;
    float* loss_box;
    const float* teacher_pred;
    float cls_temperature;
    int kl, do_cls, do_reg;
    float grad_scale_distill_cls, grad_scale_distill_reg;
    float* loss_distill;
} aldi_box_loss_chunk;
int aldi_box_losses_fused(const float* pred, int Cp, int K, const float* rois, const int* cls, const float* gt_boxes, const float* weights4,
                          const aldi_box_loss_chunk* chunks, int nchunks, float* grad, void* grad_lo, aldi_stream_t stream);
size_t aldi_detections_workspace(int N);
int aldi_detections(const float* pred, int Cp, int K, const float* props, const int* pcount, int P, int N, const int* img_hw,
                    const float* weights4, float score_thresh, float nms_thresh, int topk, float pl_thresh, void* workspace,
                    float* det_boxes, float* det_scores, int* det_cls, int* det_count,
                    float* pl_boxes, int* pl_cls, float* pl_scores, int* pl_count, int pl_rows, int* err_flag, aldi_stream_t stream);

int aldi_rpn_distill_loss(const aldi_rpn_geom* gm, float* const* student_head, float* const* teacher_head, float* const* grad,
                          const int* labels, int N, float obj_temperature, int n_valid, int n_fg, const int* n_valid_fg_dev,
                          int do_obj, int do_reg, float grad_scale, float* loss2, aldi_stream_t stream);
int aldi_roih_distill_loss(const float* student_pred, const float* teacher_pred, int Cp, int K, int R, float cls_temperature,
                           int kl, int do_cls, int do_reg, float grad_scale, float* grad, float* loss2, aldi_stream_t stream);
int aldi_domain_bce(const float* pred, int ld, int R, float label, float weight, float grad_scale, void* grad, float* loss,
                    int dtype, aldi_stream_t stream);
size_t aldi_avgpool_workspace(int N, int C);
int aldi_avgpool(const void* x, void* y, int N, int HW, int C, int dtype, void* workspace, aldi_stream_t stream);
int aldi_avgpool_bwd(const void* gy, const void* act, void* gx, int N, int HW, int C, int dtype, aldi_stream_t stream);

int aldi_torch_randperm_prefix(unsigned char* state, long n, long k, long* out);
int aldi_torch_rng_script(unsigned char* state, const long* script, int nops, int* out, int threads);
int aldi_step_draws(unsigned char* state, const int* counts, int N, const int* chunks, int nch, const long* seeds, int nseeds,
                    int rpn_batch, int rpn_pos_cap, int roi_batch, int roi_pos_cap, int* words, const int* word0, int* rows_out, int threads);
int aldi_torch_rng_prefetch(const unsigned char* state, const long* seeds, int nseeds, long max_draws);
int aldi_torch_rng_prefetch_hits(void);
int aldi_torch_rng_prefetch_wait(void);

int aldi_aug_sum_u8(const unsigned char* img, long n, unsigned long long* sum, aldi_stream_t stream);
int aldi_aug_blend(unsigned char* img, int H, int W, int mode, double w, const unsigned long long* sum, aldi_stream_t stream);
int aldi_aug_blur(const unsigned char* img, unsigned char* out, float* tmp0, float* tmp1, int H, int W, const double* weights, int radius,
                  aldi_stream_t stream);
int aldi_aug_erase(unsigned char* img, int H, int W, int h0, int w0, int h, int w, const float* fill, aldi_stream_t stream);
int aldi_aug_mic(unsigned char* img, int H, int W, const unsigned char* mask, int mh, int mw, aldi_stream_t stream);
int aldi_aug_hwc_to_chw(const unsigned char* in, unsigned char* out, int H, int W, aldi_stream_t stream);

enum { ALDI_AUG_COLOUR = 1, ALDI_AUG_GRAY = 2, ALDI_AUG_BLUR = 4, ALDI_AUG_CHW_IN = 8, ALDI_AUG_CHW_OUT = 16 };
enum { ALDI_AUG_HALO = 8 };
typedef struct aldi_aug_desc {
    const unsigned char* src;
    unsigned char* dst;
    const unsigned char* mask;
    unsigned long long sum;
    double wc, wb, ws, wg;
    double taps[ALDI_AUG_HALO + 1];
    long fill_off[3];
    int H, W, flags, radius;
    int rect[3][4];
    int nerase, mh, mw;
    int tile_begin;
    int sum_begin, sum_blocks;
} aldi_aug_desc;
typedef struct aldi_aug_fill_job {
    const unsigned int* snap;
    long out_off;
    int pos, ndoubles;
} aldi_aug_fill_job;
int aldi_aug_batch_sums(aldi_aug_desc* desc, int n, int nblocks, aldi_stream_t stream);
int aldi_aug_batch_fills(const aldi_aug_fill_job* jobs, int njobs, unsigned char* arena, aldi_stream_t stream);
int aldi_aug_batch_view(const aldi_aug_desc* desc, int n, int ntiles, const unsigned char* arena, aldi_stream_t stream);
int aldi_np_mt_advance(unsigned int* key, int* pos, long n, long seg, unsigned int* snaps, int* snap_pos, long max_snaps);

enum { ALDI_COCO_AREAS = 4, ALDI_COCO_THRS = 10, ALDI_COCO_RECS = 101 };
int aldi_coco_postprocess(const float* boxes, const float* scores, const long* classes, const int* entry, const double* meta, long n,
                          int num_classes, double* out_boxes, double* out_scores, unsigned char* out_valid, aldi_stream_t stream);
size_t aldi_coco_match_workspace(long num_gt);
int aldi_coco_match(const double* det_boxes, const int* det_off, const double* gt_boxes, const double* gt_area, const unsigned char* gt_flags,
                    const int* gt_off, int num_segments, long num_gt, const double* area_rng, const double* iou_thrs, int max_det,
                    void* workspace, unsigned long long* matched, unsigned long long* dt_ignore, int* num_gt_out, aldi_stream_t stream);
int aldi_coco_accumulate(const long* perm, const int* cat_off, const unsigned long long* matched, const unsigned long long* dt_ignore,
                         const int* num_gt, int num_images, int num_classes, const double* rec_thrs, double* precision, double* recall,
                         int* valid, aldi_stream_t stream);


int aldi_layernorm_forward(const void* x, const int* map, const float* gamma, const float* beta, void* y, float* mean,
                           float* rstd, int rows, int C, float eps, int relu, int dtype, aldi_stream_t stream);
int aldi_layernorm_backward(const void* g, const void* x, const int* map, const float* gamma, const float* mean, const float* rstd,
                            const void* res, const void* mask, void* dx, float* dgamma, float* dbeta, int rows, int C, int dtype,
                            aldi_stream_t stream);
int aldi_gelu(const void* x, const void* g, void* out, long n, int dtype, aldi_stream_t stream);
int aldi_rows_add(const void* a, const void* b, const int* map, const float* scale, void* out, int rows, int C,
                  int rows_per_sample, int dtype, aldi_stream_t stream);
int aldi_patchify(const uint8_t* img, void* out, int N, int Hs, int Ws, int P, const int* hw, const float* mean, const float* std,
                  int dtype, aldi_stream_t stream);
int aldi_linear_resize(const float* in, float* out, int L0, int L1, int C, int backward, aldi_stream_t stream);
int aldi_bicubic_resize(const float* in, float* out, int S0h, int S0w, int gh, int gw, int C, int backward, aldi_stream_t stream);
int aldi_add_pos(const void* x, const float* pos, void* y, int N, long TC, int dtype, aldi_stream_t stream);
int aldi_sum_batch(const void* g, float* out, int N, long TC, int dtype, aldi_stream_t stream);
int aldi_maxpool2(const void* x, void* y, unsigned char* idx, int N, int H, int W, int C, int backward, int dtype, aldi_stream_t stream);
int aldi_adamw_step(float* p, const float* g, float* m, float* v, void* p_compute, long n, float lr, float beta1, float beta2,
                    float eps, float weight_decay, int step, float grad_scale, int dtype, aldi_stream_t stream);

typedef struct {
    const void* qkv;
    const float* rel_h;
    const float* rel_w;
    void *Qp, *Kp, *KpT, *VT, *QsT;
    void* O;
    float* lse;
    const void* dO;
    void *dOT, *dQp;
    float* delta;
    void* dqkv;
    float *drel_h, *drel_w;
    int nB, gh, gw, heads, Dq;
    float scale;
} aldi_attn_args;
int aldi_attn_layout(int gh, int gw, int rel, int* Dq, int* tiled, long* vt_cols);
int aldi_attn_prepare(const aldi_attn_args* a, aldi_stream_t stream);
int aldi_attn_forward(const aldi_attn_args* a, aldi_stream_t stream);
int aldi_attn_backward(const aldi_attn_args* a, aldi_stream_t stream);

int aldi_ms_deform_attn_forward(const float* value, const int* spatial_shapes, const int* level_start_index, const float* sampling_loc,
                                const float* attn_weight, float* out, int N, int S, int M, int D, int Lq, int L, int P, aldi_stream_t stream);
int aldi_ms_deform_attn_backward(const float* value, const int* spatial_shapes, const int* level_start_index, const float* sampling_loc,
                                 const float* attn_weight, const float* grad_out, float* grad_value, float* grad_sampling_loc,
                                 float* grad_attn_weight, int N, int S, int M, int D, int Lq, int L, int P, aldi_stream_t stream);

int aldi_ms_deform_attn_backward_self(const float* value, const int* spatial_shapes, const int* level_start_index, const int* spatial_shapes_host,
                                      const float* sampling_loc, const float* attn_weight, const float* grad_out, float* grad_value,
                                      float* grad_sampling_loc, float* grad_attn_weight, void* workspace, size_t workspace_bytes,
                                      int N, int S, int M, int D, int L, int P, aldi_stream_t stream);
size_t aldi_ms_deform_attn_backward_self_workspace(const int* spatial_shapes_host, int N, int S, int M, int L, int P);

size_t aldi_group_norm_workspace(int N, int HW, int G);
int aldi_group_norm_forward(const float* x, const float* gamma, const float* beta, float* y, float* mean, float* rstd, void* workspace, int N, int HW,
                            int C, int G, float eps, aldi_stream_t stream);
int aldi_msda_prepare(const float* raw, const float* ref, const int* spatial_shapes, float* sampling_loc, float* attn_weight, long T, int M, int L, int P,
                      aldi_stream_t stream);
int aldi_mha_small_forward(const float* q, const float* k, const float* v, float* out, float* lse, int B, int Q, int H, int D, int ldq, int ldk, int ldv,
                           float scale, float drop_p, unsigned long long seed, aldi_stream_t stream);
int aldi_dropout_add(const float* x, const float* res, float* out, long n, float p, unsigned long long seed, aldi_stream_t stream);
int aldi_msda_prepare_backward(const float* g_loc, const float* g_aw, const float* attn_weight, const int* spatial_shapes, float* g_raw, float* g_ref, long T,
                               int M, int L, int P, aldi_stream_t stream);
int aldi_mha_small_backward(const float* q, const float* k, const float* v, const float* out, const float* d_out, const float* lse, float* dq, float* dk,
                            float* dv, float* delta, int B, int Q, int H, int D, int ldq, int ldk, int ldv, int lddq, int lddk, int lddv, float scale,
                            float drop_p, unsigned long long seed, aldi_stream_t stream);
size_t aldi_group_norm_backward_workspace(int N, int HW, int C, int G);
int aldi_group_norm_backward(const float* g, const float* x, const float* gamma, const float* mean, const float* rstd, float* dx, float* dgamma,
                             float* dbeta, void* workspace, int N, int HW, int C, int G, aldi_stream_t stream);
int aldi_detr_box_finish_backward(const float* g_boxes, const float* boxes, const float* ref, float* g_t, float* g_ref, long R, long refs,
                                  aldi_stream_t stream);
int aldi_detr_match_cost(const float* logits, const float* boxes, const int* t_labels, const float* t_boxes, const int* t_count, float* cost, int LB, int B,
                         int Nq, int K, int Gmax, float w_class, float w_bbox, float w_giou, float alpha, aldi_stream_t stream);
int aldi_detr_set_loss(const float* logits, const float* boxes, const int* match, const int* t_labels, const float* t_boxes, float* rows, float* losses,
                       float* g_logits, float* g_boxes, int LB, int B, int Nq, int K, int Gmax, float alpha, float c_ce, float c_bbox, float c_giou,
                       float num_boxes, aldi_stream_t stream);
int aldi_mask_rows(float* x, const unsigned char* keep, long T, int C, aldi_stream_t stream);
int aldi_detr_box_finish(const float* t, const float* ref, float* boxes, long R, long refs, aldi_stream_t stream);

int aldi_dwconv7(const void* x, const void* wt, const float* bias, void* y, int N, int H, int W, int C, int flip, int dtype, aldi_stream_t stream);
int aldi_dwconv7_wgrad(const void* x, const void* g, float* dw, int N, int H, int W, int C, int dtype, aldi_stream_t stream);
int aldi_scale_add(const void* x, const void* y, const float* gamma, const float* scale, void* out, long rows, int C, int rows_per_sample,
// ... 18 lines not shown
```

Before: 501.2.

## Fuse RPN 1x1 head conv into the 3x3 RPN conv epilogue

Adds an optional head to the bf16 256x256 halo64 direct-epilogue conv kernel. The kernel multiplies the freshly computed ReLU tile by the small 1x1 RPN head weights with MFMA and reduces the two wave columns through LDS. It then writes the fp32 head output directly, so the separate head conv launch and its re-read of the 256-channel feature map go away. When gradients are not saved, the bf16 conv output is not written at all. In exchange it costs extra registers in the epilogue, an extra barrier, and a plan probe per step.

```diff
diff --git a/aldi_amd/_lib.py b/aldi_amd/_lib.py
--- a/aldi_amd/_lib.py
+++ b/aldi_amd/_lib.py
@@ -109,6 +109,7 @@
         ("Ho", c_int), ("Wo", c_int),
         ("relu", c_int), ("res_mode", c_int), ("out_scale", c_int), ("OH", c_int), ("OW", c_int),
         ("dtype", c_int), ("ws", c_void_p), ("ksplit", c_int), ("mask_bits", c_void_p), ("bits_out", c_void_p),
+        ("head_w", c_void_p), ("head_shift", c_void_p), ("head_out", c_void_p), ("head_cout", c_int),
     ]
 
 
diff --git a/aldi_amd/csrc/host.h b/aldi_amd/csrc/host.h
--- a/aldi_amd/csrc/host.h
+++ b/aldi_amd/csrc/host.h
@@ -10,7 +10,7 @@
     X(igemm_halo, 1) X(igemm_force, 0) X(igemm_k64_min, 1024) X(igemm_group, 1) X(igemm_narrow_k, 512) X(igemm_splitk_tile, 2) X(igemm_halo_f32, 0) \
     X(igemm_f32_tile64_max, 4096) X(igemm_direct, 15) X(igemm_lean, 1) X(igemm_halo64_mid, 0) X(igemm_ws, 1) X(igemm_ws_wgs, 512) X(igemm_ws_min, 40000) \
     X(wgrad_lean, 1) X(wgrad_big_min, 28) X(wgrad_big_slots, 256) X(wgrad_slots, 384) X(wgrad_xcd, 1) \
-    X(igemm_halo_ilv, 1) X(igemm_halo_small, 0) X(igemm_halo96, 0) \
+    X(igemm_halo_ilv, 1) X(igemm_halo_small, 0) X(igemm_halo96, 0) X(rpn_head_fuse, 1) \
     X(wgrad_dma, 0) X(wgrad_dbg, 0) X(wgrad_group_slots, 0) X(wgrad_group_epi, 24) X(wgrad_db, 0) X(wgrad_ordered, 1) X(wgrad_big_group, 1) X(wgrad_big_epi, 12) \
     X(wgrad_big_group_min, 64) X(wgrad_lds_pad_kb, 0) X(wgrad_f32_tile128, 1) X(wgrad_dma64, 3) X(wgrad_ilv, 0) \
     X(msda_gather, 7) X(msda_gather_list, 1500) X(msda_bin, 1) X(msda_bin_list, 512) X(roialign_sep, 1) X(roialign_bwd_rows, 2) \
diff --git a/aldi_amd/csrc/igemm.hip b/aldi_amd/csrc/igemm.hip
--- a/aldi_amd/csrc/igemm.hip
+++ b/aldi_amd/csrc/igemm.hip
@@ -916,7 +916,8 @@
     igemm_body<T, BM, BN, WM, WN, KC, PIPE, HALO>(G.p[i], local, G.nmt[i], G.nnt[i]);
 }
 
-template <int BM, int BN, int WM, int WN, bool DIRECT, bool ILV = false>
+static_assert(sizeof(ConvGroup) <= 4096, "a ConvGroup travels as the kernel argument (4 KB limit)");
+template <int BM, int BN, int WM, int WN, bool DIRECT, bool ILV = false, bool HEAD = false>
 __global__ __launch_bounds__(WM* WN * 64) void igemm_halo64_group_kernel(ConvGroup G) {
     const int bid = (int)blockIdx.x;
     int i = 0;
@@ -925,7 +926,7 @@
     i = __builtin_amdgcn_readfirstlane(i);
     const int local = bid - G.wg_begin[i];
     if (local >= G.nmt[i] * G.nnt[i]) return;
-    igemm_halo64_body<BM, BN, WM, WN, DIRECT, ILV>(G.p[i], local, G.nmt[i], G.nnt[i]);
+    igemm_halo64_body<BM, BN, WM, WN, DIRECT, ILV, HEAD>(G.p[i], local, G.nmt[i], G.nnt[i]);
 }
 
 
@@ -979,6 +980,22 @@
 int launch_HALO64(const Choice& c, const ConvDev& d, const ConvGroup* g, hipStream_t st) {
     constexpr int NT = WM * WN * 64;
     constexpr bool HAS_ILV = BM == 256 && BN == 256 && WM == 4 && WN == 2;
+    if constexpr (HAS_ILV) {
+        if (c.head) {
+            if (g) {
+                ConvGroup G = *g;
+                const int wg = group_table(G, BM, BN, d);
+                if (c.ilv) hipLaunchKernelGGL((igemm_halo64_group_kernel<BM, BN, WM, WN, true, true, true>), dim3(wg), dim3(NT), 0, st, G);
+                else hipLaunchKernelGGL((igemm_halo64_group_kernel<BM, BN, WM, WN, true, false, true>), dim3(wg), dim3(NT), 0, st, G);
+            } else {
+                const dim3 grid(cdiv(d.M, BM), cdiv(d.Cout, BN));
+                if (c.ilv) hipLaunchKernelGGL((igemm_halo64_kernel<BM, BN, WM, WN, true, true, true>), grid, dim3(NT), 0, st, d);
+                else hipLaunchKernelGGL((igemm_halo64_kernel<BM, BN, WM, WN, true, false, true>), grid, dim3(NT), 0, st, d);
+            }
+            ALDI_CHECK_LAUNCH();
+            return ALDI_OK;
+        }
+    }
     if (g) {
         ConvGroup G = *g;
         const int wg = group_table(G, BM, BN, d);
@@ -1034,14 +1051,30 @@
 
 constexpr int kNameCap = 112;
 
+aldi_conv_args head_conv_args(const aldi_conv_args& a) {
+    aldi_conv_args h = {};
+    h.x = a.y; h.w = a.head_w; h.y_f32 = a.head_out; h.shift = a.head_shift;
+    h.N = a.N; h.H = a.Ho; h.W = a.Wo; h.Cin = a.Cout; h.Cout = a.head_cout; h.KH = h.KW = 1; h.stride = 1; h.pad = 0; h.Ho = a.Ho; h.Wo = a.Wo;
+    h.out_scale = 1; h.dtype = a.dtype;
+    return h;
+}
+
+int conv_many(const aldi_conv_args* args, const int n, const bool dry, hipStream_t st, char* name);
+
 int conv_one(const aldi_conv_args* a, const bool dry, hipStream_t st, char* name) {
     ConvDev d;
     Choice c;
     if (int rc = plan_conv(a, aldi_tuning(), d, c)) return rc;
     dispatch_name(c, name, kNameCap);
+    if (!dry) {
+        if (int rc = launch_choice(c, d, nullptr, st)) return rc;
+        aldi_note_dispatch(name);
+    }
+    if (a->head_out && !c.head) {
+        const aldi_conv_args h = head_conv_args(*a);
+        return conv_many(&h, 1, dry, st, name);
+    }
     if (dry) return ALDI_OK;
-    if (int rc = launch_choice(c, d, nullptr, st)) return rc;
-    aldi_note_dispatch(name);
     if (c.ksplit > 1) {
         const long mc = (long)d.M * d.Cout;
         hipLaunchKernelGGL(splitk_finalize_kernel, dim3(cdiv(mc / 4, 256)), dim3(256), 0, st, static_cast<const float*>(a->ws), c.ksplit, mc, d.Cout, a->scale, a->shift,
@@ -1063,9 +1096,15 @@
     Choice c;
     if (int rc = plan_conv_group(args, n, aldi_tuning(), G, d, c)) return rc;
     dispatch_name(c, name, kNameCap);
-    if (dry) return ALDI_OK;
-    if (int rc = launch_choice(c, d, &G, st)) return rc;
-    aldi_note_dispatch(name);
+    if (!dry) {
+        if (int rc = launch_choice(c, d, &G, st)) return rc;
+        aldi_note_dispatch(name);
+    }
+    if (args[0].head_out && !c.head) {
+        aldi_conv_args h[kMaxConvGroup];
+        for (int i = 0; i < n; ++i) h[i] = head_conv_args(args[i]);
+        return conv_many(h, n, dry, st, name);
+    }
     return ALDI_OK;
 }
 }
diff --git a/aldi_amd/csrc/igemm_halo64.h b/aldi_amd/csrc/igemm_halo64.h
--- a/aldi_amd/csrc/igemm_halo64.h
+++ b/aldi_amd/csrc/igemm_halo64.h
@@ -28,9 +28,10 @@
     }
 }
 
-template <int BM, int BN, int WM, int WN, bool DIRECT, bool ILV = false>
+template <int BM, int BN, int WM, int WN, bool DIRECT, bool ILV = false, bool HEAD = false>
 __device__ __forceinline__ void igemm_halo64_body(const ConvDev& p, int bid, const int nmt, const int nnt) {
     typedef bf16_t T;
+    static_assert(!HEAD || (DIRECT && BM == 256 && BN == 256 && WM == 4 && WN == 2), "HEAD: the 8-wave 256 x 256 direct tile");
     constexpr int NT = WM * WN * 64, KC = 8, EP = 8, BK = 64;
     constexpr int TM = BM / WM / 16;
     constexpr int TN = BN / WN / 16;
@@ -449,6 +450,18 @@
     if constexpr (DIRECT) {
         if (p.dbg & 4) return;
         constexpr int H = TN / 2;
+        u32x4_t hw[HEAD ? H : 1];
+        f32x4_t pacc[HEAD ? TM : 1];
+        if constexpr (HEAD) {
+            asm volatile("s_waitcnt lgkmcnt(0)" ::: "memory");
+            __builtin_amdgcn_s_barrier();
+            const __amdgpu_buffer_rsrc_t rhw = make_rsrc_uniform(p.head_w, (unsigned)(p.head_cout * BN * 2));
+#pragma unroll
+            for (int h = 0; h < H; ++h) hw[h] = __builtin_amdgcn_raw_buffer_load_b128(rhw, (unsigned)((fr * BN + wn * (BN / WN) + h * 32 + fq * 8) * 2), 0, 0);
+#pragma unroll
+            for (int i = 0; i < TM; ++i) pacc[i] = f32x4_t{0.f, 0.f, 0.f, 0.f};
+        }
+        u32x4_t ovs[HEAD ? TM : 1][HEAD ? H : 1];
         float4 sc[H][2], sh[H][2];
         const bool has_sc = p.scale != nullptr, has_sh = p.shift != nullptr;
 #pragma unroll
@@ -468,7 +481,7 @@
 #pragma unroll
             for (int h = 0; h < H; ++h) {
                 const int c = n0 + wn * (BN / WN) + h * 32 + fq * 8;
-                const bool ok = m < p.M && c < p.Cout;
+                const bool ok = m < p.M && c < p.Cout && (!HEAD || p.y != nullptr);
                 float v[8];
 #pragma unroll
                 for (int e = 0; e < 4; ++e) { v[e] = acc[i][2 * h][e]; v[4 + e] = acc[i][2 * h + 1][e]; }
@@ -493,6 +506,42 @@
                 }
                 const u32x4_t ov = {d[0], d[1], d[2], d[3]};
                 __builtin_amdgcn_raw_buffer_store_b128(ov, ry, ok ? ((unsigned)m * (unsigned)p.Cout + (unsigned)c) * 2u : 0x80000000u, 0, 0);
+                if constexpr (HEAD) ovs[i][h] = ov;
+            }
+        }
+        if constexpr (HEAD) {
+            const unsigned ho = lbase + (unsigned)((wm * TM * 64 + lane) * 16);
+            if (wn == 0) {
+#pragma unroll
+                for (int h = 0; h < H; ++h)
+#pragma unroll
+                    for (int i = 0; i < TM; ++i) pacc[i] = Mma<T>::run(hw[h], ovs[i][h], pacc[i]);
+                asm volatile("s_nop 15\n\ts_nop 15" : "+v"(pacc[0]), "+v"(pacc[1]), "+v"(pacc[2]), "+v"(pacc[3]));
+#pragma unroll
+                for (int i = 0; i < TM; ++i) asm volatile("ds_write_b128 %0, %1 offset:%2" ::"v"(ho), "v"(pacc[i]), "n"(i * 64 * 16) : "memory");
+            }
+            asm volatile("s_waitcnt lgkmcnt(0)" ::: "memory");
+            __builtin_amdgcn_s_barrier();
+            if (wn == 1) {
+                u32x4_t rcv[TM];
+                frag_read_n<TM, 64 * 16, 0>(rcv, ho);
+                frag_wait1<TM>(rcv);
+#pragma unroll
+                for (int i = 0; i < TM; ++i) pacc[i] = __builtin_bit_cast(f32x4_t, rcv[i]);
+#pragma unroll
+                for (int h = 0; h < H; ++h)
+#pragma unroll
+                    for (int i = 0; i < TM; ++i) pacc[i] = Mma<T>::run(hw[h], ovs[i][h], pacc[i]);
+                float4 hs = make_float4(0.f, 0.f, 0.f, 0.f);
+                const bool okc = fq * 4 < p.head_cout;
+                if (p.head_shift != nullptr && okc) hs = *reinterpret_cast<const float4*>(p.head_shift + fq * 4);
+                const __amdgpu_buffer_rsrc_t rho = make_rsrc_uniform(p.head_out, (unsigned)p.M * (unsigned)p.head_cout * 4u);
+#pragma unroll
+                for (int i = 0; i < TM; ++i) {
+                    const int m = m0 + wm * (BM / WM) + i * 16 + fr;
+                    const f32x4_t o = {pacc[i][0] + hs.x, pacc[i][1] + hs.y, pacc[i][2] + hs.z, pacc[i][3] + hs.w};
+                    __builtin_amdgcn_raw_buffer_store_b128(__builtin_bit_cast(u32x4_t, o), rho, m < p.M && okc ? ((unsigned)m * (unsigned)p.head_cout + (unsigned)(fq * 4)) * 4u : 0x80000000u, 0, 0);
+                }
             }
         }
         return;
@@ -500,7 +549,7 @@
     igemm_epilogue<T, BM, BN, WM, WN, LDS_SLOTS * 16>(p, acc, m0, n0, reinterpret_cast<unsigned char*>(&lds_all[0]));
 }
 
-template <int BM, int BN, int WM, int WN, bool DIRECT, bool ILV = false>
+template <int BM, int BN, int WM, int WN, bool DIRECT, bool ILV = false, bool HEAD = false>
 __global__ __launch_bounds__(WM* WN * 64) void igemm_halo64_kernel(ConvDev p) {
-    igemm_halo64_body<BM, BN, WM, WN, DIRECT, ILV>(p, (int)(blockIdx.y * gridDim.x + blockIdx.x), (int)gridDim.x, (int)gridDim.y);
+    igemm_halo64_body<BM, BN, WM, WN, DIRECT, ILV, HEAD>(p, (int)(blockIdx.y * gridDim.x + blockIdx.x), (int)gridDim.x, (int)gridDim.y);
 }
diff --git a/aldi_amd/csrc/igemm_select.h b/aldi_amd/csrc/igemm_select.h
--- a/aldi_amd/csrc/igemm_select.h
+++ b/aldi_amd/csrc/igemm_select.h
@@ -14,6 +14,7 @@
     int ksplit, slabs_per_split;
     int lean;
     const unsigned char* mask_bits; unsigned char* bits_out;
+    const void* head_w; const float* head_shift; float* head_out; int head_cout;
 };
 
 constexpr int kMaxConvGroup = 12;
@@ -70,6 +71,7 @@
     int ksplit;
     int ws_wgs;
     int group_n;
+    bool head;
 };
 
 inline int ws_channels(int K) { return K == 64 || K == 128 ? 256 : K == 256 || K == 512 ? 128 : 0; }
@@ -79,7 +81,10 @@
            d.ksplit <= 1 && (long)d.M * d.Cout * 2 < (1L << 31);
 }
 inline bool halo64_direct_ok(const ConvDev& d) {
-    return d.y && !d.y_f32 && d.out_scale == 1 && (d.Cout & 7) == 0 && !d.mask && !d.mask_bits && !d.bits_out && !d.res_mode;
+    return (d.y || d.head_out) && !d.y_f32 && d.out_scale == 1 && (d.Cout & 7) == 0 && !d.mask && !d.mask_bits && !d.bits_out && !d.res_mode;
+}
+inline bool head_fuse_ok(const ConvDev& d) {
+    return d.head_out && d.Cout == 256 && d.head_cout % 4 == 0 && d.head_cout <= 16 && (long)d.M * d.head_cout * 4 < (1L << 31);
 }
 inline bool plain_1x1(const ConvDev& d) { return d.KH * d.KW == 1 && d.stride == 1 && d.pad == 0; }
 
@@ -93,6 +98,8 @@
             c.direct = (tn.igemm_direct & 8) != 0;
             for (int i = 0; i < (group_n ? group_n : 1); ++i) c.direct = c.direct && halo64_direct_ok(group_n ? group[i] : d);
             c.ilv = c.tile == BF16_HALO64_256x256 && tn.igemm_halo_ilv != 0;
+            c.head = c.tile == BF16_HALO64_256x256 && c.direct && tn.rpn_head_fuse != 0;
+            for (int i = 0; i < (group_n ? group_n : 1); ++i) c.head = c.head && head_fuse_ok(group_n ? group[i] : d);
         }
         return c;
     };
@@ -195,8 +202,8 @@
     switch (r.form) {
     case WS: return snprintf(name, cap, "igemm_ws<%s,%d,%d,k%d>", elem, r.BM, r.BN, r.KC * 8);
     case HALO64:
-        return snprintf(name, cap, "igemm%s%.0d<%s,%d,%d,%d,%d,halo64%s%s>", grp, c.group_n, elem, r.BM, r.BN, r.WM, r.WN, c.direct ? ",direct" : "",
-                        (c.tile == BF16_HALO64_256x256 && !c.ilv) ? ",lockstep" : "");
+        return snprintf(name, cap, "igemm%s%.0d<%s,%d,%d,%d,%d,halo64%s%s%s>", grp, c.group_n, elem, r.BM, r.BN, r.WM, r.WN, c.direct ? ",direct" : "",
+                        c.head ? ",head" : "", (c.tile == BF16_HALO64_256x256 && !c.ilv) ? ",lockstep" : "");
     case ROLES: return snprintf(name, cap, "igemm<%s,%d,%d,%d,%d,roles,halo>", elem, r.BM, r.BN, r.WM, r.WN);
     default:
         return snprintf(name, cap, "igemm%s%.0d<%s,%d,%d,%d,%d,%s,%s%s%s>%s", grp, c.group_n, elem, r.BM, r.BN, r.WM, r.WN, r.pipe ? "pipe" : "flat", r.form == HALO ? "halo" : "tap",
@@ -205,7 +212,7 @@
 }
 
 inline int fill_convdev(const aldi_conv_args* a, ConvDev& d) {
-    if (!a || !a->x || !a->w || (!a->y && !a->y_f32)) return aldi_set_error_msg(ALDI_ERR_ARG, "conv_igemm: null pointer");
+    if (!a || !a->x || !a->w || (!a->y && !a->y_f32 && !a->head_out)) return aldi_set_error_msg(ALDI_ERR_ARG, "conv_igemm: null pointer");
     const int bk = a->dtype == ALDI_BF16 ? 32 : 16;
     const int ep = a->dtype == ALDI_BF16 ? 8 : 4;
     if (a->dtype != ALDI_BF16 && a->dtype != ALDI_F32) return aldi_set_error_msg(ALDI_ERR_ARG, "conv_igemm: bad dtype");
@@ -239,6 +246,19 @@
     if ((a->mask_bits || a->bits_out) && (a->dtype != ALDI_BF16 || (a->Cout & 7) || d.out_scale != 1 || a->res_mode == 2 || !a->y || a->y_f32 || a->ksplit > 1))
         return aldi_set_error_msg(ALDI_ERR_ARG, "conv_igemm: bit masks take bf16 outputs with Cout % 8 == 0 in the plain layout (no fp32 output, scatter, upsampled residual or split-K)");
     if (a->mask_bits && a->mask) return aldi_set_error_msg(ALDI_ERR_ARG, "conv_igemm: mask and mask_bits are alternatives");
+    d.head_w = a->head_w; d.head_shift = a->head_shift; d.head_out = a->head_out; d.head_cout = a->head_out ? a->head_cout : 0;
+    if (a->head_out && (!a->head_w || a->head_cout < 4 || a->head_cout % 4 != 0))
+        return aldi_set_error_msg(ALDI_ERR_ARG, "conv_igemm: head_out needs head_w and a head_cout that is a positive multiple of 4");
+    if (a->head_out && (a->ksplit > 1 || d.out_scale != 1 || a->y_f32))
+        return aldi_set_error_msg(ALDI_ERR_ARG, "conv_igemm: a head reads the plain `dtype` output y (no split-K, scatter or fp32 output)");
+    return ALDI_OK;
+}
+
+inline int head_needs_y(const Choice& c, const ConvDev* p, int n) {
+    for (int i = 0; i < n && !c.head; ++i)
+        if (p[i].head_out && !p[i].y)
+            return aldi_set_error_msg(ALDI_ERR_ARG, "conv_igemm: y is null but the head does not fuse into this launch (it takes bf16, the 256x256 halo64 tile with the direct "
+                                                    "epilogue, Cout = 256, head_cout <= 16 and rpn_head_fuse = 1): pass y for the two-launch path");
     return ALDI_OK;
 }
 
@@ -253,6 +273,7 @@
         d.ksplit = ks;
     }
     c = select_tile(d, tn, a->dtype != ALDI_BF16, 0);
+    if (int rc = head_needs_y(c, &d, 1)) return rc;
     d.xcd = tn.igemm_xcd; d.dbg = tn.igemm_dbg;
     if (c.ksplit > 1) d.slabs_per_split = d.K / (kTiles[c.tile].KC * 8) / c.ksplit;
     return ALDI_OK;
@@ -264,7 +285,8 @@
         const aldi_conv_args &a = args[0], &b = args[i];
         same = a.dtype == b.dtype && a.Cin == b.Cin && a.Cout == b.Cout && a.KH == b.KH && a.KW == b.KW &&
                a.stride == b.stride && a.pad == b.pad && (a.Ho == a.H) == (b.Ho == b.H) && (a.Wo == a.W) == (b.Wo == b.W) && a.out_scale == b.out_scale &&
-               (a.y != nullptr) == (b.y != nullptr) && (a.y_f32 != nullptr) == (b.y_f32 != nullptr);
+               (a.y != nullptr || a.head_out != nullptr) == (b.y != nullptr || b.head_out != nullptr) && (a.y_f32 != nullptr) == (b.y_f32 != nullptr) &&
+               (a.head_out != nullptr) == (b.head_out != nullptr) && (!a.head_out || a.head_cout == b.head_cout);
     }
     return same;
 }
@@ -281,6 +303,7 @@
     d = G.p[0];
     d.M = (int)(Msum > 0x7fffffffL ? 0x7fffffffL : Msum);
     c = select_tile(d, tn, args[0].dtype != ALDI_BF16, n, G.p);
+    if (int rc = head_needs_y(c, G.p, n)) return rc;
     d.xcd = tn.igemm_xcd; d.dbg = tn.igemm_dbg;
     return ALDI_OK;
 }
diff --git a/aldi_amd/engine.py b/aldi_amd/engine.py
--- a/aldi_amd/engine.py
+++ b/aldi_amd/engine.py
@@ -442,11 +442,14 @@
             self._ws[name] = t
         return t
 
-    def _conv_call(self, x, name, *, relu=False, res=None, res_mode=0, want_f32=False, out=None, bits_out=None):
+    def _conv_call(self, x, name, *, relu=False, res=None, res_mode=0, want_f32=False, out=None, bits_out=None, head=None, head_out=None, no_out=False):
         W = self.wts
         p = W.layout.t[name]
-        return x, W.w(name), dict(stride=p.stride, pad=p.pad, scale=W.scale(name), shift=W.shift(name), res=res, res_mode=res_mode, relu=relu,
-                                  want_f32=want_f32, out=out, bits_out=bits_out)
+        kw = dict(stride=p.stride, pad=p.pad, scale=W.scale(name), shift=W.shift(name), res=res, res_mode=res_mode, relu=relu,
+                  want_f32=want_f32, out=out, bits_out=bits_out)
+        if head is not None:
+            kw.update(head=(W.w(head), W.shift(head), head_out), no_out=no_out)
+        return x, W.w(name), kw
 
     def conv(self, x, name, **kw):
         x, w, kw = self._conv_call(x, name, **kw)
@@ -616,18 +619,32 @@
 
     def rpn_head_steps(self, c: Ctx, save: bool):
         px = [f.shape[0] * f.shape[1] * f.shape[2] for f in c.P]
-        flat = torch.empty((1, sum(px), 1, FPN_C), dtype=self.dtype, device=self.device)
+        conv, head = "proposal_generator.rpn_head.conv", "rpn_head_out"
+        fuse, hf = False, None
+        if self.dtype == torch.bfloat16 and self.level_groups and self.Ch <= 16 and self.wts.scale(head) is None:
+            hf = torch.empty((1, sum(px), 1, self.Ch), dtype=torch.float32, device=self.device)
+            probe, o = [], 0
+            for f, n in zip(c.P, px):
+                probe.append(self._conv_call(f, conv, relu=True, head=head, head_out=hf[0, o:o + n, 0], out=f))
+                o += n
+            fuse = ",head" in ops.conv2d_group_plan(probe)
+        flat = None if (fuse and not save) else torch.empty((1, sum(px), 1, FPN_C), dtype=self.dtype, device=self.device)
         ts, o, reqs = [], 0, []
         for f, n in zip(c.P, px):
-            view = flat[0, o:o + n, 0].view(f.shape[0], f.shape[1], f.shape[2], FPN_C)
-            reqs.append((f, "proposal_generator.rpn_head.conv", dict(relu=True, out=view)))
+            kw = dict(relu=True)
+            if flat is not None:
+                kw["out"] = flat[0, o:o + n, 0].view(f.shape[0], f.shape[1], f.shape[2], FPN_C)
+            if fuse:
+                kw.update(head=head, head_out=hf[0, o:o + n, 0], no_out=flat is None)
+            reqs.append((f, conv, kw))
             o += n
         if self.level_groups:
             ts = yield reqs
         else:
             for r in reqs:
                 ts.append((yield r))
-        hf = yield flat, "rpn_head_out", dict(want_f32=True)
+        if not fuse:
+            hf = yield flat, head, dict(want_f32=True)
         heads, o = [], 0
         for f, n in zip(c.P, px):
             heads.append(hf[0, o:o + n, 0].view(f.shape[0], f.shape[1], f.shape[2], hf.shape[3]))
diff --git a/aldi_amd/ops.py b/aldi_amd/ops.py
--- a/aldi_amd/ops.py
+++ b/aldi_amd/ops.py
@@ -50,7 +50,7 @@
            mask: Optional[torch.Tensor] = None, out: Optional[torch.Tensor] = None,
            out_f32: Optional[torch.Tensor] = None, want_f32: bool = False,
            out_scale: int = 1, out_hw=None, ksplit: Optional[int] = None, mask_bits: Optional[torch.Tensor] = None,
-           bits_out: Optional[torch.Tensor] = None) -> torch.Tensor:
+           bits_out: Optional[torch.Tensor] = None, head=None, no_out: bool = False) -> torch.Tensor:
     N, H, W_, Cin = x.shape
     Cout, KH, KW, Cin2 = w.shape
     assert Cin == Cin2 and x.is_contiguous() and w.is_contiguous() and x.dtype == w.dtype, (x.shape, w.shape, x.dtype, w.dtype)
@@ -62,21 +62,32 @@
     else:
         OH = OW = 0
         shape = (N, Ho, Wo, Cout)
-    if out is None and not want_f32:
+    if out is None and not want_f32 and not no_out:
         out = torch.empty(shape, dtype=x.dtype, device=x.device)
     if want_f32 and out_f32 is None:
         out_f32 = torch.empty(shape, dtype=torch.float32, device=x.device)
     ws = None
     if ksplit is None:
         ksplit = _auto_ksplit(x, N * Ho * Wo, Cout, KH * KW * Cin, KH * KW == 1 and stride == 1 and pad == 0 and res is None and mask is None
-                              and not want_f32 and out_f32 is None and out_scale == 1 and mask_bits is None and bits_out is None)
+                              and head is None and not want_f32 and out_f32 is None and out_scale == 1 and mask_bits is None and bits_out is None)
     if ksplit and ksplit > 1:
         ws = torch.empty(ksplit * N * Ho * Wo * Cout, dtype=torch.float32, device=x.device)
     a = L.ConvArgs(_p(x), _p(w), _p(out), _p(out_f32), _p(scale), _p(shift), _p(res), _p(mask),
                    N, H, W_, Cin, Cout, KH, KW, stride, pad, Ho, Wo,
-                   int(relu), res_mode, out_scale, OH, OW, dtype_code(x.dtype), _p(ws), int(ksplit or 0), _p(mask_bits), _p(bits_out))
+                   int(relu), res_mode, out_scale, OH, OW, dtype_code(x.dtype), _p(ws), int(ksplit or 0), _p(mask_bits), _p(bits_out), *_head_fields(head, N * Ho * Wo, Cout, x))
     L.call("aldi_conv_igemm", C.byref(a), stream_ptr())
     return out_f32 if want_f32 and out is None else out
+
+
+def _head_fields(head, M: int, Cout: int, x: torch.Tensor):
+    if head is None:
+        return None, None, None, 0
+    hw, hshift, hout = head
+    ch = hw.shape[0]
+    assert hw.is_contiguous() and hw.numel() == ch * Cout and hw.dtype == x.dtype, (hw.shape, hw.dtype, Cout)
+    assert hout.is_contiguous() and hout.dtype == torch.float32 and hout.numel() == M * ch, (hout.shape, M, ch)
+    assert hshift is None or (hshift.dtype == torch.float32 and hshift.numel() == ch)
+    return _p(hw), _p(hshift), _p(hout), ch
 
 
 def _auto_ksplit(x, M, Cout, K, plain: bool) -> int:
@@ -93,7 +104,7 @@
 
 
 def _conv_args(x, w, *, stride=1, pad=0, scale=None, shift=None, res=None, res_mode=0, relu=False, mask=None, out=None, out_f32=None,
-               want_f32=False, out_scale=1, out_hw=None, mask_bits=None, bits_out=None):
+               want_f32=False, out_scale=1, out_hw=None, mask_bits=None, bits_out=None, head=None, no_out=False):
     N, H, W_, Cin = x.shape
     Cout, KH, KW, Cin2 = w.shape
     assert Cin == Cin2 and x.is_contiguous() and w.is_contiguous() and x.dtype == w.dtype, (x.shape, w.shape, x.dtype, w.dtype)
@@ -105,13 +116,13 @@
     else:
         OH = OW = 0
         shape = (N, Ho, Wo, Cout)
-    if out is None and not want_f32:
+    if out is None and not want_f32 and not no_out:
         out = torch.empty(shape, dtype=x.dtype, device=x.device)
     if want_f32 and out_f32 is None:
         out_f32 = torch.empty(shape, dtype=torch.float32, device=x.device)
     a = L.ConvArgs(_p(x), _p(w), _p(out), _p(out_f32), _p(scale), _p(shift), _p(res), _p(mask),
                    N, H, W_, Cin, Cout, KH, KW, stride, pad, Ho, Wo,
-                   int(relu), res_mode, out_scale, OH, OW, dtype_code(x.dtype), None, 0, _p(mask_bits), _p(bits_out))
+                   int(relu), res_mode, out_scale, OH, OW, dtype_code(x.dtype), None, 0, _p(mask_bits), _p(bits_out), *_head_fields(head, N * Ho * Wo, Cout, x))
     return a, (out_f32 if want_f32 and out is None else out)
 
 
@@ -123,6 +134,13 @@
         outs.append(y)
     L.call("aldi_conv_igemm_group", arr, len(calls), stream_ptr())
     return outs
+
+
+def conv2d_group_plan(calls) -> str:
+    arr = (L.ConvArgs * len(calls))()
+    for i, (x, w, kw) in enumerate(calls):
+        arr[i], _ = _conv_args(x, w, **kw)
+    return L.plan_dispatch(arr[0] if len(calls) == 1 else arr, len(calls))
 
 
 _WGRAD_WS = {}
diff --git a/include/aldi_hip.h b/include/aldi_hip.h
--- a/include/aldi_hip.h
+++ b/include/aldi_hip.h
@@ -42,6 +42,10 @@
     int ksplit;
     const void* mask_bits;
     void* bits_out;
+    const void* head_w;
+    const float* head_shift;
+    float* head_out;
+    int head_cout;
 } aldi_conv_args;
 
 int aldi_conv_igemm(const aldi_conv_args* a, aldi_stream_t stream);
```

After: 499.5, median of 2. Within noise of the previous version (-0.4%).
